# scheck-k/ste-gan

Measured on NVIDIA B200. Metric: GAN train samples/s, higher is better.
Workload: dtype bf16

## Files before the change

### include/stegan_b200.h

```cpp
#ifndef STEGAN_B200_H_
#define STEGAN_B200_H_

#include <stdint.h>

#ifdef __cplusplus
extern "C" {
#endif

typedef void* stg_stream_t;

enum { STG_F32 = 0, STG_BF16 = 1 };
enum { STG_ACT_NONE = 0, STG_ACT_RELU = 1, STG_ACT_LEAKY = 2, STG_ACT_TANH = 3 };
enum {
  STG_OK = 0,
  STG_EINVAL = -1,
  STG_ECUDA = -2,
  STG_EUNSUPPORTED = -3
};
enum { STG_ENGINE_AUTO = 0, STG_ENGINE_SIMT = 1, STG_ENGINE_TCGEN05 = 2, STG_ENGINE_MATVEC = 3  };

#define STG_MAX_TAPS 48

typedef struct StgConv {
  int32_t dtype;
  int32_t engine;
  int32_t n_samples;
  int32_t phases;
  int32_t t_src;
  int32_t t_dst;
  int32_t c_src;
  int32_t c_dst;
  int32_t groups;
  int32_t k, dilation, stride, pad;
  int32_t transposed;
  int32_t pair_sum;
  int32_t post_shift;
  int32_t mask_mode;
  int32_t act;
  int32_t dup_rows;
  int32_t out_f32;
  int32_t w_fwd_pack;
  const void* src;
  const void* w;
  const float* bias;
  const void* add_pre;
  const void* mask;
  const void* add_post;
  void* y_raw;
  void* y_act;
} StgConv;

int stg_conv(const StgConv* d, stg_stream_t stream);

int stg_conv_masked(const StgConv* d, const int32_t* valid_units, int32_t rows_per_unit, stg_stream_t stream);

typedef struct StgWgrad {
  int32_t dtype, engine;
  int32_t n_samples, phases, t_in, t_out, c_in, c_out, groups, k, dilation, stride, pad;
  const void* x;
  const void* dy;
  float* dw;
  float* dbias;
} StgWgrad;

int stg_conv_wgrad(const StgWgrad* d, stg_stream_t stream);
int stg_wgrad_layout(const StgWgrad* d, int* ld, int* span);

enum { STG_PACK_UNFOLD = 1 };
int stg_weightnorm_fold(const float* v, const float* g, int c_out, int cin_g, int k, int groups, int pack_groups,
                        int flags, int dtype, void* wf, void* wd, float* scale, stg_stream_t stream);
int stg_weightnorm_fold_bwd(const float* dw, int dw_ld, int dw_span, const float* v, const float* g, int c_out, int cin_g,
                            int k, int groups, float* dv, float* dg, int accumulate, stg_stream_t stream);

int stg_spectralnorm_fold(const float* w_orig, float* u, float* v, int c_out, int cin_g, int k, int groups,
                          int pack_groups, int flags, int training, int dtype, void* wf, void* wd, float* sigma_out,
                          float* scratch, float* u_used, float* v_used, stg_stream_t stream);
int stg_spectralnorm_fold_bwd(const float* dw, int dw_ld, int dw_span, const float* w_orig, const float* u, const float* v,
                              const float* sigma, int c_out, int cin_g, int k, int groups, float* dw_orig, int accumulate,
                              float* scratch, stg_stream_t stream);
typedef struct StgFoldItem {
  const float* v;
  const float* g;
  void* wf;
  void* wd;
  float* scale;
  const float* dw;
  float* dv;
  float* dg;
  int32_t c_out, cin_g, k, groups, pg, flags, dw_ld, dw_span;
  int32_t row0, tile0;
} StgFoldItem;
int stg_weightnorm_fold_multi(const StgFoldItem* items, int n_items, int total_rows, int total_tiles, int dtype,
                              stg_stream_t stream);
int stg_weightnorm_fold_bwd_multi(const StgFoldItem* items, int n_items, int total_rows, int accumulate,
                                  stg_stream_t stream);
int stg_weightnorm_fold_bwd_range(const StgFoldItem* items, int n_items, int row_base, int n_rows, int accumulate,
                                  stg_stream_t stream);

int stg_tc_pack_groups(int c_in, int c_out, int groups);

int stg_unfold(const void* src, int dtype, int B, int phases, int t_src, int t_dst, int C, int k, int dilation, int stride,
               int pad, void* out, stg_stream_t stream);
int stg_unfold_bwd(const void* dout, int dtype, int B, int phases, int t_src, int t_dst, int C, int k, int dilation,
                   int stride, int pad, float* dsrc, stg_stream_t stream);

int stg_period_first_layer(const float* x, const void* wf, const float* bias, int B, int T, int C, int period, int c_out,
                           int k, int stride, int pad, float slope, void* y, stg_stream_t stream);

int stg_embed_concat(const float* units, const float* emb, const int64_t* ids, int B, int T, int d_units, int d_emb,
                     int dtype, void* x0, stg_stream_t stream);
int stg_embed_concat_bwd(const void* dx0, const int64_t* ids, int B, int T, int d_units, int d_emb, int dtype,
                         float* demb, stg_stream_t stream);

int stg_reflect_pad_right(const float* x, int B, int T, int C, int T_pad, int dtype, void* out, stg_stream_t stream);
int stg_reflect_pad_right_bwd(const void* dout, int B, int T, int C, int T_pad, int dtype, float* dx, stg_stream_t stream);
int stg_avgpool4(const float* x, int B, int T, int C, float* out, stg_stream_t stream);
int stg_avgpool4_bwd(const float* dout, int B, int T, int C, float* dx, stg_stream_t stream);
int stg_cast(const void* src, int src_dtype, void* dst, int dst_dtype, int64_t n, stg_stream_t stream);
int stg_act_bwd(const float* dy, const float* y, int mode, int64_t n, int dtype, void* out, stg_stream_t stream);
int stg_relu_rows(const void* src, int dtype, int64_t rows, int C, int dup, void* out, stg_stream_t stream);
int stg_pair_sum_rows(const void* in, int64_t rows_out, int C, int dtype, void* out, stg_stream_t stream);
int stg_axpy_f32(float* y, const void* x, int x_dtype, float alpha, int64_t n, stg_stream_t stream);

int stg_td_loss(const float* x_real, const float* x_gen, int B, int T, int C, float* losses, const float* grad_scale,
                float* dx_gen, float* scratch, stg_stream_t stream);
int stg_td_loss_ex(const float* x_real, const float* x_gen, int B, int T, int C, int n_res, const int* wins,
                   const int* shifts, int pad_windows, int avg_window, float* losses, const float* grad_scale,
                   const float* grad_scale_dev, float* dx_gen, float* scratch, stg_stream_t stream);
int stg_td_features(const float* x, int B, int T, int C, int win, int shift, int pad_windows, int avg_window,
                    float* feats, float* scratch, stg_stream_t stream);
int stg_frame_stats(const float* x, int B, int T, int C, int win, int shift, int pad_windows, float* mean, float* power,
                    stg_stream_t stream);
int stg_window_signal(const float* x, int B, int T, int C, int win, int shift, int pad_windows, float* out,
                      stg_stream_t stream);
int stg_average_filter(const float* x, int64_t rows, int T, int window, int pad, float* out, stg_stream_t stream);

int stg_mse_const(const void* x, int dtype, int64_t n, float target, float* out_slot, float grad_scale, void* dx,
                  int dx_dtype, stg_stream_t stream);
int stg_l1_mean(const void* a, const void* b, int dtype, int64_t n, float* out_slot, float grad_scale, void* da,
                stg_stream_t stream);

#define STG_MAX_LOSS_ITEMS 32
typedef struct StgL1Item { const void* a; const void* b; void* da; int64_t n; } StgL1Item;
typedef struct StgMseItem { const void* x; void* dx; int64_t n; float target; int32_t slot; } StgMseItem;
int stg_l1_mean_multi(const StgL1Item* items, int n_items, int dtype, float* out_slot, float grad_scale, stg_stream_t stream);
int stg_mse_const_multi(const StgMseItem* items, int n_items, int x_dtype, int dx_dtype, float* slots, float grad_scale,
                        stg_stream_t stream);

int stg_layernorm_fwd(const void* x, int dtype, const float* gamma, const float* beta, int rows, int D, float eps, void* y,
                      float* stats, stg_stream_t stream);
int stg_layernorm_bwd(const void* dy, const void* x, int dtype, const float* stats, const float* gamma, int rows, int D,
                      void* dx, stg_stream_t stream);
int stg_relattn_fwd(const void* qkv, int dtype, const float* emb, int B, int L, int H, int d, int max_rel, float scale, void* o,
                    float* probs, stg_stream_t stream);
int stg_relattn_bwd(const void* qkv, int dtype, const float* emb, const float* probs, const void* dout, int B, int L, int H,
                    int d, int max_rel, float scale, void* dqkv, stg_stream_t stream);
int stg_relattn_dense_supported(int L, int d, int need_bwd);
int stg_relattn_band_fwd(const void* qkv, int dtype, const float* emb, int B, int L, int H, int d, int max_rel, float scale,
                         void* o, float* probs_band, stg_stream_t stream);
int stg_relattn_band_bwd(const void* qkv, int dtype, const float* emb, const float* probs_band, const void* dout, int B, int L,
                         int H, int d, int max_rel, float scale, void* dqkv, float* scratch, stg_stream_t stream);
int stg_relattn_fwd_masked(const void* qkv, int dtype, const float* emb, int B, int L, int H, int d, int max_rel, float scale,
                           void* o, float* probs, const int32_t* lengths, stg_stream_t stream);
int stg_relattn_band_fwd_masked(const void* qkv, int dtype, const float* emb, int B, int L, int H, int d, int max_rel, float scale,
                                void* o, float* probs_band, const int32_t* lengths, stg_stream_t stream);
int stg_encoder_losses(const float* unit_pred, const float* unit_target, const float* phoneme_logits,
                       const int64_t* phoneme_target, int N, int Du, int P, float* slots, float gs_units, float gs_phonemes,
                       void* d_units, void* d_logits, int grad_dtype, stg_stream_t stream);
int stg_encoder_scores(const float* unit_pred, const float* unit_target, const float* phoneme_logits,
                       const int64_t* phoneme_target, const int32_t* lengths, int B, int T, int Du, int P, int silence_index,
                       float* sums, int32_t* counts, stg_stream_t stream);

enum { STG_ADAMW_KEEP_STEP = 1 };
int stg_adamw(float* p, const float* g, float* m, float* v, int64_t n, float lr, const float* lr_dev, float beta1,
              float beta2, float eps, float weight_decay, int64_t* step_count, float grad_scale, int32_t* enable,
              int flags, stg_stream_t stream);

const char* stg_strerror(int code);
const char* stg_last_cuda_error(void);
int stg_version(void);
unsigned long long stg_launch_count(void);
void stg_set_sm_limit(int n_sms);
int stg_conv_tc_supported(const StgConv* d);
int stg_wgrad_tc_supported(const StgWgrad* d);
int stg_conv_route(const StgConv* d);
int stg_wgrad_route(const StgWgrad* d);
int stg_debug_set_trace(void* buf);
int stg_debug_rowshift(const void* x, const void* w, int rows_a, int shift, int base_off, float* out, stg_stream_t stream);
int stg_debug_group_mma(const void* x, const void* w, int cin_g, int cout_g, float* out, stg_stream_t stream);
int stg_debug_row_classes(int t_dst, int* out);
int stg_debug_tma_bw(const void* buf, long long n_rows, int box_rows, int n_iters, int mode, int stages, int grid, long long* clk,
                     stg_stream_t stream);
int stg_debug_conv_plan(const StgConv* d, int* out);
double stg_debug_ingest_bytes(int reset);

#ifdef __cplusplus
}
#endif
#endif
```

### ste_gan_b200/_lib.py

```python
from __future__ import annotations

import ctypes as C
import os

_HERE = os.path.dirname(os.path.abspath(__file__))
LIB_PATH = os.path.join(_HERE, "libstegan_b200.so")

F32, BF16 = 0, 1
ACT_NONE, ACT_RELU, ACT_LEAKY, ACT_TANH = 0, 1, 2, 3
ENGINE_AUTO, ENGINE_SIMT, ENGINE_TCGEN05 = 0, 1, 2
PACK_UNFOLD = 1
MAX_TAPS = 48


class StgConv(C.Structure):
    _fields_ = [(n, C.c_int32) for n in (
        "dtype", "engine", "n_samples", "phases", "t_src", "t_dst", "c_src", "c_dst", "groups", "k", "dilation",
        "stride", "pad", "transposed", "pair_sum", "post_shift", "mask_mode", "act", "dup_rows", "out_f32", "w_fwd_pack")] + [
        (n, C.c_void_p) for n in ("src", "w", "bias", "add_pre", "mask", "add_post", "y_raw", "y_act")]


class StgWgrad(C.Structure):
    _fields_ = [(n, C.c_int32) for n in (
        "dtype", "engine", "n_samples", "phases", "t_in", "t_out", "c_in", "c_out", "groups", "k", "dilation",
        "stride", "pad")] + [(n, C.c_void_p) for n in ("x", "dy", "dw", "dbias")]


class StgFoldItem(C.Structure):
    _fields_ = [(n, C.c_void_p) for n in ("v", "g", "wf", "wd", "scale", "dw", "dv", "dg")] + [
        (n, C.c_int32) for n in ("c_out", "cin_g", "k", "groups", "pg", "flags", "dw_ld", "dw_span", "row0", "tile0")]


class StgL1Item(C.Structure):
    _fields_ = [("a", C.c_void_p), ("b", C.c_void_p), ("da", C.c_void_p), ("n", C.c_int64)]


class StgMseItem(C.Structure):
    _fields_ = [("x", C.c_void_p), ("dx", C.c_void_p), ("n", C.c_int64), ("target", C.c_float), ("slot", C.c_int32)]


MAX_LOSS_ITEMS = 32
_P, _I, _L, _F = C.c_void_p, C.c_int, C.c_int64, C.c_float
_SIGS = {
    "stg_conv": [C.POINTER(StgConv), _P],
    "stg_conv_masked": [C.POINTER(StgConv), _P, C.c_int32, _P],
    "stg_conv_wgrad": [C.POINTER(StgWgrad), _P],
    "stg_conv_tc_supported": [C.POINTER(StgConv)],
    "stg_conv_route": [C.POINTER(StgConv)],
    "stg_wgrad_route": [C.POINTER(StgWgrad)],
    "stg_wgrad_tc_supported": [C.POINTER(StgWgrad)],
    "stg_weightnorm_fold": [_P, _P, _I, _I, _I, _I, _I, _I, _I, _P, _P, _P, _P],
    "stg_weightnorm_fold_bwd": [_P, _I, _I, _P, _P, _I, _I, _I, _I, _P, _P, _I, _P],
    "stg_wgrad_layout": [C.POINTER(StgWgrad), C.POINTER(C.c_int), C.POINTER(C.c_int)],
    "stg_spectralnorm_fold": [_P, _P, _P, _I, _I, _I, _I, _I, _I, _I, _I, _P, _P, _P, _P, _P, _P, _P],
    "stg_spectralnorm_fold_bwd": [_P, _I, _I, _P, _P, _P, _P, _I, _I, _I, _I, _P, _I, _P, _P],
    "stg_tc_pack_groups": [_I, _I, _I],
    "stg_l1_mean_multi": [_P, _I, _I, _P, _F, _P],
    "stg_mse_const_multi": [_P, _I, _I, _I, _P, _F, _P],
    "stg_weightnorm_fold_multi": [_P, _I, _I, _I, _I, _P],
    "stg_weightnorm_fold_bwd_multi": [_P, _I, _I, _I, _P],
    "stg_weightnorm_fold_bwd_range": [_P, _I, _I, _I, _I, _P],
    "stg_debug_set_trace": [_P],
    "stg_debug_rowshift": [_P, _P, _I, _I, _I, _P, _P],
    "stg_debug_row_classes": [_I, _P],
    "stg_debug_group_mma": [_P, _P, _I, _I, _P, _P],
    "stg_debug_conv_plan": [_P, _P],
    "stg_debug_tma_bw": [_P, C.c_longlong, _I, _I, _I, _I, _I, _P, _P],
    "stg_unfold": [_P, _I, _I, _I, _I, _I, _I, _I, _I, _I, _I, _P, _P],
    "stg_unfold_bwd": [_P, _I, _I, _I, _I, _I, _I, _I, _I, _I, _I, _P, _P],
    "stg_period_first_layer": [_P, _P, _P, _I, _I, _I, _I, _I, _I, _I, _I, C.c_float, _P, _P],
    "stg_embed_concat": [_P, _P, _P, _I, _I, _I, _I, _I, _P, _P],
    "stg_embed_concat_bwd": [_P, _P, _I, _I, _I, _I, _I, _P, _P],
    "stg_reflect_pad_right": [_P, _I, _I, _I, _I, _I, _P, _P],
    "stg_reflect_pad_right_bwd": [_P, _I, _I, _I, _I, _I, _P, _P],
    "stg_avgpool4": [_P, _I, _I, _I, _P, _P],
    "stg_avgpool4_bwd": [_P, _I, _I, _I, _P, _P],
    "stg_cast": [_P, _I, _P, _I, _L, _P],
    "stg_act_bwd": [_P, _P, _I, _L, _I, _P, _P],
    "stg_pair_sum_rows": [_P, _L, _I, _I, _P, _P],
    "stg_relu_rows": [_P, _I, _L, _I, _I, _P, _P],
    "stg_axpy_f32": [_P, _P, _I, _F, _L, _P],
    "stg_td_loss": [_P, _P, _I, _I, _I, _P, C.POINTER(C.c_float), _P, _P, _P],
    "stg_td_loss_ex": [_P, _P, _I, _I, _I, _I, C.POINTER(C.c_int), C.POINTER(C.c_int), _I, _I, _P, C.POINTER(C.c_float), _P, _P, _P, _P],
    "stg_td_features": [_P, _I, _I, _I, _I, _I, _I, _I, _P, _P, _P],
    "stg_frame_stats": [_P, _I, _I, _I, _I, _I, _I, _P, _P, _P],
    "stg_window_signal": [_P, _I, _I, _I, _I, _I, _I, _P, _P],
    "stg_average_filter": [_P, _L, _I, _I, _I, _P, _P],
    "stg_mse_const": [_P, _I, _L, _F, _P, _F, _P, _I, _P],
    "stg_l1_mean": [_P, _P, _I, _L, _P, _F, _P, _P],
    "stg_layernorm_fwd": [_P, _I, _P, _P, _I, _I, _F, _P, _P, _P],
    "stg_layernorm_bwd": [_P, _P, _I, _P, _P, _I, _I, _P, _P],
    "stg_relattn_fwd": [_P, _I, _P, _I, _I, _I, _I, _I, _F, _P, _P, _P],
    "stg_relattn_bwd": [_P, _I, _P, _P, _P, _I, _I, _I, _I, _I, _F, _P, _P],
    "stg_relattn_dense_supported": [_I, _I, _I],
    "stg_relattn_band_fwd": [_P, _I, _P, _I, _I, _I, _I, _I, _F, _P, _P, _P],
    "stg_relattn_band_bwd": [_P, _I, _P, _P, _P, _I, _I, _I, _I, _I, _F, _P, _P, _P],
    "stg_relattn_fwd_masked": [_P, _I, _P, _I, _I, _I, _I, _I, _F, _P, _P, _P, _P],
    "stg_relattn_band_fwd_masked": [_P, _I, _P, _I, _I, _I, _I, _I, _F, _P, _P, _P, _P],
    "stg_encoder_losses": [_P, _P, _P, _P, _I, _I, _I, _P, _F, _F, _P, _P, _I, _P],
    "stg_encoder_scores": [_P, _P, _P, _P, _P, _I, _I, _I, _I, _I, _P, _P, _P],
    "stg_adamw": [_P, _P, _P, _P, _L, _F, _P, _F, _F, _F, _F, _P, _F, _P, _I, _P],
}
EXPORTS = sorted(list(_SIGS) + ["stg_strerror", "stg_last_cuda_error", "stg_version", "stg_launch_count", "stg_set_sm_limit",
                                   "stg_debug_ingest_bytes"])

_lib = None


class StgError(RuntimeError):
    pass


def load(build_if_missing: bool = True):
    global _lib
    if _lib is not None:
        return _lib
    if not os.path.exists(LIB_PATH):
        if not build_if_missing:
            raise StgError(f"{LIB_PATH} is missing; run `python -m ste_gan_b200.build`")
        from . import build as _b
        _b.build()
    import torch
    lib = C.CDLL(LIB_PATH, mode=C.RTLD_GLOBAL)
    for name, argtypes in _SIGS.items():
        fn = getattr(lib, name)
        fn.argtypes = argtypes
        fn.restype = C.c_int
    lib.stg_strerror.argtypes = [C.c_int]
    lib.stg_strerror.restype = C.c_char_p
    lib.stg_last_cuda_error.argtypes = []
    lib.stg_last_cuda_error.restype = C.c_char_p
    lib.stg_version.argtypes = []
    lib.stg_version.restype = C.c_int
    lib.stg_set_sm_limit.argtypes = [C.c_int]
    lib.stg_set_sm_limit.restype = None
    lib.stg_debug_ingest_bytes.argtypes = [C.c_int]
    lib.stg_debug_ingest_bytes.restype = C.c_double
    lib.stg_launch_count.argtypes = []
    lib.stg_launch_count.restype = C.c_ulonglong
    _lib = lib
    return lib


def check(code: int, what: str = "") -> None:
    if code != 0:
        lib = load()
        msg = lib.stg_strerror(code).decode()
        if code == -2:
            msg += ": " + lib.stg_last_cuda_error().decode()
        raise StgError(f"{what}: {msg} (code {code})")
```

### ste_gan_b200/csrc/common.cuh

```cuda
#pragma once
#include <cuda_bf16.h>
#include <cuda_runtime.h>
#include <stdint.h>

#include "../../include/stegan_b200.h"

namespace stg {

void set_cuda_error(cudaError_t e, const char* where);

#define STG_CUDA_CHECK(expr)                                   \
  do {                                                         \
    cudaError_t _e = (expr);                                   \
    if (_e != cudaSuccess) {                                   \
      ::stg::set_cuda_error(_e, #expr);                        \
      return STG_ECUDA;                                        \
    }                                                          \
  } while (0)

extern unsigned long long g_launch_count;
extern double g_ingest_bytes;
extern int g_sm_limit;
#define STG_LAUNCH_CHECK()                 \
  do {                                     \
    ++::stg::g_launch_count;               \
    STG_CUDA_CHECK(cudaGetLastError());    \
  } while (0)

using bf16 = __nv_bfloat16;

__device__ __forceinline__ float to_f(float v) { return v; }
__device__ __forceinline__ float to_f(bf16 v) { return __bfloat162float(v); }
template <typename T> __device__ __forceinline__ T from_f(float v);
template <> __device__ __forceinline__ float from_f<float>(float v) { return v; }
template <> __device__ __forceinline__ bf16 from_f<bf16>(float v) { return __float2bfloat16_rn(v); }

__device__ __forceinline__ void ld4(const float* p, float (&o)[4]) {
  float4 v = *reinterpret_cast<const float4*>(p);
  o[0] = v.x; o[1] = v.y; o[2] = v.z; o[3] = v.w;
}
__device__ __forceinline__ void ld4(const bf16* p, float (&o)[4]) {
  uint2 v = *reinterpret_cast<const uint2*>(p);
  __nv_bfloat162 a = *reinterpret_cast<__nv_bfloat162*>(&v.x);
  __nv_bfloat162 b = *reinterpret_cast<__nv_bfloat162*>(&v.y);
  o[0] = __low2float(a); o[1] = __high2float(a); o[2] = __low2float(b); o[3] = __high2float(b);
}
__device__ __forceinline__ void st4(float* p, const float (&v)[4]) {
  *reinterpret_cast<float4*>(p) = make_float4(v[0], v[1], v[2], v[3]);
}
__device__ __forceinline__ void st4(bf16* p, const float (&v)[4]) {
  __nv_bfloat162 a = __floats2bfloat162_rn(v[0], v[1]);
  __nv_bfloat162 b = __floats2bfloat162_rn(v[2], v[3]);
  uint2 u;
  u.x = *reinterpret_cast<uint32_t*>(&a);
  u.y = *reinterpret_cast<uint32_t*>(&b);
  *reinterpret_cast<uint2*>(p) = u;
}

__device__ __forceinline__ float act_apply(int act, float v) {
  switch (act) {
    case STG_ACT_RELU: return v > 0.f ? v : 0.f;
    case STG_ACT_LEAKY: return v > 0.f ? v : 0.1f * v;
    case STG_ACT_TANH: return tanhf(v);
    default: return v;
  }
}
__device__ __forceinline__ float act_grad_from_output(int mode, float m) {
  switch (mode) {
    case STG_ACT_RELU: return m > 0.f ? 1.f : 0.f;
    case STG_ACT_LEAKY: return m > 0.f ? 1.f : 0.1f;
    case STG_ACT_TANH: return 1.f - m * m;
    default: return 1.f;
  }
}

__device__ __forceinline__ float warp_sum(float v) {
#pragma unroll
  for (int o = 16; o > 0; o >>= 1) v += __shfl_xor_sync(0xffffffffu, v, o);
  return v;
}
__device__ __forceinline__ float block_sum(float v, float* red) {
  const int lane = threadIdx.x & 31, warp = threadIdx.x >> 5, nw = (blockDim.x + 31) >> 5;
  v = warp_sum(v);
  __syncthreads();
  if (lane == 0) red[warp] = v;
  __syncthreads();
  float r = (lane < nw) ? red[lane] : 0.f;
  r = warp_sum(r);
  return r;
}

static inline int64_t ceil_div64(int64_t a, int64_t b) { return (a + b - 1) / b; }
static inline int ceil_div(int a, int b) { return (a + b - 1) / b; }

int conv_simt(const StgConv* d, cudaStream_t s, const int32_t* valid_units = nullptr, int rows_per_unit = 1);
int conv_tc(const StgConv* d, cudaStream_t s, const int32_t* valid_units = nullptr, int rows_per_unit = 1);
int conv_tc_plan(const StgConv* d, int* out);
bool conv_tc_supported(const StgConv* d);
int wgrad_simt(const StgWgrad* d, cudaStream_t s);
int wgrad_tc(const StgWgrad* d, cudaStream_t s);
bool wgrad_tc_supported(const StgWgrad* d);
int tc_pack_groups(int c_in, int c_out, int groups);
bool conv_c1_supported(const StgConv* d);
int conv_c1(const StgConv* d, cudaStream_t s);
bool wgrad_c1_supported(const StgWgrad* d);
int wgrad_c1(const StgWgrad* d, cudaStream_t s);
void conv_tc_set_trace(long long* buf);
void wgrad_tc_layout(const StgWgrad* d, int* ld, int* span);

}
```

### ste_gan_b200/csrc/misc.cu

```cuda
#include "common.cuh"

namespace stg {
namespace {

template <typename T>
__global__ void embed_concat_kernel(const float* __restrict__ units, const float* __restrict__ emb,
                                    const int64_t* __restrict__ ids, int T_, int du, int de, int64_t total,
                                    T* __restrict__ x0) {
  const int C = du + de;
  for (int64_t i = (int64_t)blockIdx.x * blockDim.x + threadIdx.x; i < total; i += (int64_t)gridDim.x * blockDim.x) {
    const int c = (int)(i % C);
    const int64_t bt = i / C;
    const int b = (int)(bt / T_);
    const float v = c < du ? units[bt * du + c] : emb[ids[b] * de + (c - du)];
    x0[i] = from_f<T>(v);
  }
}

template <typename T>
__global__ void embed_bwd_kernel(const T* __restrict__ dx0, const int64_t* __restrict__ ids, int T_, int du, int de,
                                 float* __restrict__ demb) {
  const int b = blockIdx.x, e = threadIdx.x;
  if (e >= de) return;
  const int C = du + de;
  float s = 0.f;
  for (int t = 0; t < T_; ++t) s += to_f(dx0[((int64_t)b * T_ + t) * C + du + e]);
  atomicAdd(demb + ids[b] * de + e, s);
}

__device__ __forceinline__ int reflect_right(int t, int T_) { return t < T_ ? t : 2 * (T_ - 1) - t; }

template <typename T>
__global__ void reflect_pad_kernel(const float* __restrict__ x, int T_, int C, int Tp, int64_t total, T* __restrict__ out) {
  for (int64_t i = (int64_t)blockIdx.x * blockDim.x + threadIdx.x; i < total; i += (int64_t)gridDim.x * blockDim.x) {
    const int c = (int)(i % C);
    const int64_t bt = i / C;
    const int t = (int)(bt % Tp), b = (int)(bt / Tp);
    out[i] = from_f<T>(x[((int64_t)b * T_ + reflect_right(t, T_)) * C + c]);
  }
}
template <typename T>
__global__ void reflect_pad_bwd_kernel(const T* __restrict__ dout, int T_, int C, int Tp, int64_t total_in,
                                       float* __restrict__ dx) {
  for (int64_t i = (int64_t)blockIdx.x * blockDim.x + threadIdx.x; i < total_in; i += (int64_t)gridDim.x * blockDim.x) {
    const int c = (int)(i % C);
    const int64_t bt = i / C;
    const int t = (int)(bt % T_), b = (int)(bt / T_);
    float g = to_f(dout[((int64_t)b * Tp + t) * C + c]);
    const int m = 2 * (T_ - 1) - t;
    if (m >= T_ && m < Tp) g += to_f(dout[((int64_t)b * Tp + m) * C + c]);
    atomicAdd(dx + i, g);
  }
}

__global__ void avgpool4_kernel(const float* __restrict__ x, int T_, int C, int To, int64_t total, float* __restrict__ out) {
  for (int64_t i = (int64_t)blockIdx.x * blockDim.x + threadIdx.x; i < total; i += (int64_t)gridDim.x * blockDim.x) {
    const int c = (int)(i % C);
    const int64_t bo = i / C;
    const int o = (int)(bo % To), b = (int)(bo / To);
    float s = 0.f;
#pragma unroll
    for (int j = -1; j <= 2; ++j) {
      const int t = 2 * o + j;
      if (t >= 0 && t < T_) s += x[((int64_t)b * T_ + t) * C + c];
    }
    out[i] = 0.25f * s;
  }
}
__global__ void avgpool4_bwd_kernel(const float* __restrict__ dout, int T_, int C, int To, int64_t total_in,
                                    float* __restrict__ dx) {
  for (int64_t i = (int64_t)blockIdx.x * blockDim.x + threadIdx.x; i < total_in; i += (int64_t)gridDim.x * blockDim.x) {
    const int c = (int)(i % C);
    const int64_t bt = i / C;
    const int t = (int)(bt % T_), b = (int)(bt / T_);
    float s = 0.f;
    const int lo = (t - 2 + 1) >> 1;
    for (int o = lo; o <= (t + 1) / 2; ++o)
      if (o >= 0 && o < To && 2 * o - 1 <= t && t <= 2 * o + 2) s += dout[((int64_t)b * To + o) * C + c];
    dx[i] += 0.25f * s;
  }
}

template <typename S, typename D>
__global__ void cast_kernel(const S* __restrict__ src, D* __restrict__ dst, int64_t n) {
  for (int64_t i = (int64_t)blockIdx.x * blockDim.x + threadIdx.x; i < n; i += (int64_t)gridDim.x * blockDim.x)
    dst[i] = from_f<D>(to_f(src[i]));
}

template <typename T>
__global__ void relu_rows_kernel(const T* __restrict__ src, int64_t rows, int C, int dup, T* __restrict__ out) {
  const int64_t total = rows * C;
  for (int64_t i = (int64_t)blockIdx.x * blockDim.x + threadIdx.x; i < total; i += (int64_t)gridDim.x * blockDim.x) {
    const int64_t r = i / C;
    const int c = (int)(i - r * C);
    const T v = from_f<T>(fmaxf(to_f(src[i]), 0.f));
    if (dup) { out[(2 * r) * C + c] = v; out[(2 * r + 1) * C + c] = v; }
    else out[i] = v;
  }
}

template <typename T>
__global__ void act_bwd_kernel(const float* __restrict__ dy, const float* __restrict__ y, int mode, int64_t n,
                               T* __restrict__ out) {
  for (int64_t i = (int64_t)blockIdx.x * blockDim.x + threadIdx.x; i < n; i += (int64_t)gridDim.x * blockDim.x)
    out[i] = from_f<T>(dy[i] * act_grad_from_output(mode, y[i]));
}

template <typename T>
__global__ void pair_sum_kernel(const T* __restrict__ in, int64_t rows_out, int C, T* __restrict__ out) {
  const int64_t total = rows_out * C;
  for (int64_t i = (int64_t)blockIdx.x * blockDim.x + threadIdx.x; i < total; i += (int64_t)gridDim.x * blockDim.x) {
    const int c = (int)(i % C);
    const int64_t r = i / C;
    out[i] = from_f<T>(to_f(in[(2 * r) * C + c]) + to_f(in[(2 * r + 1) * C + c]));
  }
}

template <typename T>
__global__ void axpy_kernel(float* __restrict__ y, const T* __restrict__ x, float alpha, int64_t n) {
  for (int64_t i = (int64_t)blockIdx.x * blockDim.x + threadIdx.x; i < n; i += (int64_t)gridDim.x * blockDim.x)
    y[i] = fmaf(alpha, to_f(x[i]), y[i]);
}

__global__ void step_inc_kernel(int64_t* step, const int32_t* __restrict__ enable) {
  if (enable == nullptr || *enable != 0) *step += 1;
}
__global__ void flag_clear_kernel(int32_t* flag) { *flag = 0; }

__global__ void __launch_bounds__(256) adamw_kernel(float* __restrict__ p, const float* __restrict__ g, float* __restrict__ m,
                                                    float* __restrict__ v, int64_t n, float lr_host,
                                                    const float* __restrict__ lr_dev, float b1, float b2, float eps,
                                                    float wd, const int64_t* __restrict__ step, float gscale,
                                                    const int32_t* __restrict__ enable) {
  if (enable != nullptr && *enable == 0) return;
  const float lr = lr_dev ? *lr_dev : lr_host;
  const float t = (float)(*step);
  const float bc1 = 1.f - powf(b1, t), bc2 = 1.f - powf(b2, t);
  const float step_size = lr / bc1, inv_sqrt_bc2 = rsqrtf(bc2), decay = 1.f - lr * wd;
  for (int64_t i = (int64_t)blockIdx.x * blockDim.x + threadIdx.x; i < n; i += (int64_t)gridDim.x * blockDim.x) {
    const float gi = g[i] * gscale;
    const float mi = b1 * m[i] + (1.f - b1) * gi;
    const float vi = b2 * v[i] + (1.f - b2) * gi * gi;
    m[i] = mi;
    v[i] = vi;
    const float denom = sqrtf(vi) * inv_sqrt_bc2 + eps;
    p[i] = p[i] * decay - step_size * (mi / denom);
  }
}

inline int grid_for(int64_t n) {
  int64_t b = ceil_div64(n, 256);
  const int64_t cap = 148 * 16;
  return (int)(b < 1 ? 1 : (b > cap ? cap : b));
}

template <typename T>
__global__ void unfold_kernel(const T* __restrict__ src, int phases, int t_src, int t_dst, int C, int k, int dil, int stride,
                              int pad, int Kp, int64_t total, T* __restrict__ out) {
  const int slots = Kp / C + ((Kp % C) ? 1 : 0);
  for (int64_t i = (int64_t)blockIdx.x * blockDim.x + threadIdx.x; i < total; i += (int64_t)gridDim.x * blockDim.x) {
    const int j = (int)(i % slots);
    const int64_t row = i / slots;
    const int ph = (int)(row % phases);
    const int64_t bt = row / phases;
    const int t = (int)(bt % t_dst);
    const int64_t b = bt / t_dst;
    const int ts = t * stride + j * dil - pad;
    const bool ok = j < k && ts >= 0 && ts < t_src;
    const T* s = src + ((b * t_src + ts) * phases + ph) * C;
    T* o = out + row * Kp + (int64_t)j * C;
    const int n = min(C, Kp - j * C);
    for (int c = 0; c < n; ++c) o[c] = ok ? s[c] : from_f<T>(0.f);
  }
}
template <typename T>
__global__ void unfold_bwd_kernel(const T* __restrict__ dout, int phases, int t_src, int t_dst, int C, int k, int dil,
                                  int stride, int pad, int Kp, int64_t total, float* __restrict__ dsrc) {
  for (int64_t i = (int64_t)blockIdx.x * blockDim.x + threadIdx.x; i < total; i += (int64_t)gridDim.x * blockDim.x) {
    const int c = (int)(i % C);
    const int64_t row = i / C;
    const int ph = (int)(row % phases);
    const int64_t bt = row / phases;
    const int ts = (int)(bt % t_src);
    const int64_t b = bt / t_src;
    float g = 0.f;
    for (int j = 0; j < k; ++j) {
      const int num = ts + pad - j * dil;
      if (num < 0) break;
      const int t = num / stride;
      if (t * stride == num && t < t_dst) g += to_f(dout[((b * t_dst + t) * phases + ph) * Kp + j * C + c]);
    }
    dsrc[i] += g;
  }
}

}
}

using namespace stg;
#define S_ static_cast<cudaStream_t>(stream)

extern "C" int stg_embed_concat(const float* units, const float* emb, const int64_t* ids, int B, int T, int d_units,
                                int d_emb, int dtype, void* x0, stg_stream_t stream) {
  if (!units || !x0 || (d_emb > 0 && (!emb || !ids))) return STG_EINVAL;
  const int64_t total = (int64_t)B * T * (d_units + d_emb);
  if (dtype == STG_F32) embed_concat_kernel<float><<<grid_for(total), 256, 0, S_>>>(units, emb, ids, T, d_units, d_emb, total, (float*)x0);
  else embed_concat_kernel<bf16><<<grid_for(total), 256, 0, S_>>>(units, emb, ids, T, d_units, d_emb, total, (bf16*)x0);
  STG_LAUNCH_CHECK();
  return STG_OK;
}

extern "C" int stg_embed_concat_bwd(const void* dx0, const int64_t* ids, int B, int T, int d_units, int d_emb, int dtype,
                                    float* demb, stg_stream_t stream) {
  if (!dx0 || !ids || !demb || d_emb > 1024) return STG_EINVAL;
  if (dtype == STG_F32) embed_bwd_kernel<float><<<B, d_emb, 0, S_>>>((const float*)dx0, ids, T, d_units, d_emb, demb);
  else embed_bwd_kernel<bf16><<<B, d_emb, 0, S_>>>((const bf16*)dx0, ids, T, d_units, d_emb, demb);
  STG_LAUNCH_CHECK();
  return STG_OK;
}

extern "C" int stg_reflect_pad_right(const float* x, int B, int T, int C, int T_pad, int dtype, void* out, stg_stream_t stream) {
  if (!x || !out || T_pad < T || T_pad - T > T - 1) return STG_EINVAL;
  const int64_t total = (int64_t)B * T_pad * C;
  if (dtype == STG_F32) reflect_pad_kernel<float><<<grid_for(total), 256, 0, S_>>>(x, T, C, T_pad, total, (float*)out);
  else reflect_pad_kernel<bf16><<<grid_for(total), 256, 0, S_>>>(x, T, C, T_pad, total, (bf16*)out);
  STG_LAUNCH_CHECK();
  return STG_OK;
}

extern "C" int stg_reflect_pad_right_bwd(const void* dout, int B, int T, int C, int T_pad, int dtype, float* dx, stg_stream_t stream) {
  if (!dout || !dx) return STG_EINVAL;
  const int64_t total = (int64_t)B * T * C;
  if (dtype == STG_F32) reflect_pad_bwd_kernel<float><<<grid_for(total), 256, 0, S_>>>((const float*)dout, T, C, T_pad, total, dx);
  else reflect_pad_bwd_kernel<bf16><<<grid_for(total), 256, 0, S_>>>((const bf16*)dout, T, C, T_pad, total, dx);
  STG_LAUNCH_CHECK();
  return STG_OK;
}

extern "C" int stg_avgpool4(const float* x, int B, int T, int C, float* out, stg_stream_t stream) {
  if (!x || !out) return STG_EINVAL;
  const int To = (T + 2 - 4) / 2 + 1;
  const int64_t total = (int64_t)B * To * C;
  avgpool4_kernel<<<grid_for(total), 256, 0, S_>>>(x, T, C, To, total, out);
  STG_LAUNCH_CHECK();
  return STG_OK;
}

extern "C" int stg_avgpool4_bwd(const float* dout, int B, int T, int C, float* dx, stg_stream_t stream) {
  if (!dout || !dx) return STG_EINVAL;
  const int To = (T + 2 - 4) / 2 + 1;
  const int64_t total = (int64_t)B * T * C;
  avgpool4_bwd_kernel<<<grid_for(total), 256, 0, S_>>>(dout, T, C, To, total, dx);
  STG_LAUNCH_CHECK();
  return STG_OK;
}

extern "C" int stg_cast(const void* src, int sd, void* dst, int dd, int64_t n, stg_stream_t stream) {
  if (!src || !dst) return STG_EINVAL;
  const int g = grid_for(n);
  if (sd == STG_F32 && dd == STG_BF16) cast_kernel<float, bf16><<<g, 256, 0, S_>>>((const float*)src, (bf16*)dst, n);
  else if (sd == STG_BF16 && dd == STG_F32) cast_kernel<bf16, float><<<g, 256, 0, S_>>>((const bf16*)src, (float*)dst, n);
  else if (sd == STG_F32 && dd == STG_F32) cast_kernel<float, float><<<g, 256, 0, S_>>>((const float*)src, (float*)dst, n);
  else if (sd == STG_BF16 && dd == STG_BF16) cast_kernel<bf16, bf16><<<g, 256, 0, S_>>>((const bf16*)src, (bf16*)dst, n);
  else return STG_EINVAL;
  STG_LAUNCH_CHECK();
  return STG_OK;
}

extern "C" int stg_relu_rows(const void* src, int dtype, int64_t rows, int C, int dup, void* out, stg_stream_t stream) {
  if (!src || !out || rows < 1 || C < 1) return STG_EINVAL;
  if (dtype == STG_F32) relu_rows_kernel<float><<<grid_for(rows * C), 256, 0, S_>>>((const float*)src, rows, C, dup, (float*)out);
  else if (dtype == STG_BF16) relu_rows_kernel<bf16><<<grid_for(rows * C), 256, 0, S_>>>((const bf16*)src, rows, C, dup, (bf16*)out);
  else return STG_EINVAL;
  STG_LAUNCH_CHECK();
  return STG_OK;
}

extern "C" int stg_act_bwd(const float* dy, const float* y, int mode, int64_t n, int dtype, void* out, stg_stream_t stream) {
  if (!dy || !y || !out) return STG_EINVAL;
  if (dtype == STG_F32) act_bwd_kernel<float><<<grid_for(n), 256, 0, S_>>>(dy, y, mode, n, (float*)out);
  else act_bwd_kernel<bf16><<<grid_for(n), 256, 0, S_>>>(dy, y, mode, n, (bf16*)out);
  STG_LAUNCH_CHECK();
  return STG_OK;
}

extern "C" int stg_pair_sum_rows(const void* in, int64_t rows_out, int C, int dtype, void* out, stg_stream_t stream) {
  if (!in || !out) return STG_EINVAL;
  const int g = grid_for(rows_out * C);
  if (dtype == STG_F32) pair_sum_kernel<float><<<g, 256, 0, S_>>>((const float*)in, rows_out, C, (float*)out);
  else pair_sum_kernel<bf16><<<g, 256, 0, S_>>>((const bf16*)in, rows_out, C, (bf16*)out);
  STG_LAUNCH_CHECK();
  return STG_OK;
}

extern "C" int stg_axpy_f32(float* y, const void* x, int x_dtype, float alpha, int64_t n, stg_stream_t stream) {
  if (!y || !x) return STG_EINVAL;
  if (x_dtype == STG_F32) axpy_kernel<float><<<grid_for(n), 256, 0, S_>>>(y, (const float*)x, alpha, n);
  else axpy_kernel<bf16><<<grid_for(n), 256, 0, S_>>>(y, (const bf16*)x, alpha, n);
  STG_LAUNCH_CHECK();
  return STG_OK;
}

extern "C" int stg_adamw(float* p, const float* g, float* m, float* v, int64_t n, float lr, const float* lr_dev, float beta1,
                         float beta2, float eps, float weight_decay, int64_t* step_count, float grad_scale, int32_t* enable,
                         int flags, stg_stream_t stream) {
  if (!p || !g || !m || !v || !step_count) return STG_EINVAL;
  if (!(flags & STG_ADAMW_KEEP_STEP)) {
    step_inc_kernel<<<1, 1, 0, S_>>>(step_count, enable);
    STG_LAUNCH_CHECK();
  }
  adamw_kernel<<<grid_for(n), 256, 0, S_>>>(p, g, m, v, n, lr, lr_dev, beta1, beta2, eps, weight_decay, step_count, grad_scale, enable);
  STG_LAUNCH_CHECK();
  if (enable) {
    flag_clear_kernel<<<1, 1, 0, S_>>>(enable);
    STG_LAUNCH_CHECK();
  }
  return STG_OK;
}

extern "C" int stg_unfold(const void* src, int dtype, int B, int phases, int t_src, int t_dst, int C, int k, int dilation,
                          int stride, int pad, void* out, stg_stream_t stream) {
  cudaStream_t s = static_cast<cudaStream_t>(stream);
  if (!src || !out || B < 1 || phases < 1 || C < 1 || k < 1 || stride < 1 || dilation < 1) return STG_EINVAL;
  const int Kp = (k * C + 7) / 8 * 8;
  const int slots = Kp / C + ((Kp % C) ? 1 : 0);
  const int64_t total = (int64_t)B * t_dst * phases * slots;
  const int64_t nb = ceil_div64(total, 256);
  const int blocks = (int)(nb < 148 * 16 ? nb : 148 * 16);
  if (dtype == STG_F32) unfold_kernel<float><<<blocks, 256, 0, s>>>(static_cast<const float*>(src), phases, t_src, t_dst, C, k, dilation, stride, pad, Kp, total, static_cast<float*>(out));
  else if (dtype == STG_BF16) unfold_kernel<bf16><<<blocks, 256, 0, s>>>(static_cast<const bf16*>(src), phases, t_src, t_dst, C, k, dilation, stride, pad, Kp, total, static_cast<bf16*>(out));
  else return STG_EINVAL;
  STG_LAUNCH_CHECK();
  return STG_OK;
}

extern "C" int stg_unfold_bwd(const void* dout, int dtype, int B, int phases, int t_src, int t_dst, int C, int k,
                              int dilation, int stride, int pad, float* dsrc, stg_stream_t stream) {
  cudaStream_t s = static_cast<cudaStream_t>(stream);
  if (!dout || !dsrc || B < 1 || phases < 1 || C < 1 || k < 1 || stride < 1 || dilation < 1) return STG_EINVAL;
  const int Kp = (k * C + 7) / 8 * 8;
  const int64_t total = (int64_t)B * t_src * phases * C;
  const int64_t nb = ceil_div64(total, 256);
  const int blocks = (int)(nb < 148 * 16 ? nb : 148 * 16);
  if (dtype == STG_F32) unfold_bwd_kernel<float><<<blocks, 256, 0, s>>>(static_cast<const float*>(dout), phases, t_src, t_dst, C, k, dilation, stride, pad, Kp, total, dsrc);
  else if (dtype == STG_BF16) unfold_bwd_kernel<bf16><<<blocks, 256, 0, s>>>(static_cast<const bf16*>(dout), phases, t_src, t_dst, C, k, dilation, stride, pad, Kp, total, dsrc);
  else return STG_EINVAL;
  STG_LAUNCH_CHECK();
  return STG_OK;
}
```

### ste_gan_b200/csrc/norm_fold.cu

```cuda
#include "common.cuh"

namespace stg {
namespace {

__global__ void __launch_bounds__(256) wn_scale_kernel(const float* __restrict__ v, const float* __restrict__ g, int n,
                                                       float* __restrict__ scale) {
  __shared__ float red[32];
  const int co = blockIdx.x;
  const float* row = v + (int64_t)co * n;
  float s = 0.f;
  for (int i = threadIdx.x; i < n; i += blockDim.x) { const float x = row[i]; s = fmaf(x, x, s); }
  s = block_sum(s, red);
  if (threadIdx.x == 0) scale[co] = g[co] / sqrtf(s);
}

template <typename T>
__global__ void __launch_bounds__(256) pack_fwd_kernel(const float* __restrict__ v, const float* __restrict__ scale,
                                                       int c_out, int cin_g, int k, int groups, int pg,
                                                       T* __restrict__ wf) {
  const int co = blockIdx.y;
  const int c_in = cin_g * groups, cin_gp = c_in / pg, cout_gp = c_out / pg, cout_g = c_out / groups;
  const int idx = blockIdx.x * 256 + threadIdx.x;
  if (idx >= cin_gp * k) return;
  const int j = idx / cin_gp, cip = idx - j * cin_gp;
// ... 24 lines not shown
    tile[r][tx] = w;
  }
  __syncthreads();
  for (int r = ty; r < 32; r += 8) {
    const int cip = ci0 + r, cop = co0 + tx;
    if (cip < cin_gp && cop < cout_gp)
      wd[((int64_t)j * c_in + gp * cin_gp + cip) * cout_gp + cop] = from_f<T>(tile[tx][r]);
  }
}

template <typename T>
__global__ void __launch_bounds__(256) pack_unfold_kernel(const float* __restrict__ v, const float* __restrict__ scale,
                                                          int c_out, int c_in, int k, int Kp, T* __restrict__ wf,
                                                          T* __restrict__ wd) {
  const int idx = blockIdx.x * 256 + threadIdx.x;
  if (idx >= c_out * Kp) return;
  const int co = idx / Kp, q = idx - co * Kp;
  float w = 0.f;
  if (q < k * c_in) {
    const int j = q / c_in, c = q - j * c_in;
    w = v[((int64_t)co * c_in + c) * k + j] * scale[co];
  }
  if (wf) wf[(int64_t)co * Kp + q] = from_f<T>(w);
  if (wd) wd[(int64_t)q * c_out + co] = from_f<T>(w);
}

__device__ __forceinline__ int span_goff(int co, int cin_g, int cout_g, int span) {
  if (span == cin_g || cout_g >= 128) return 0;
  return ((co / cout_g) % (128 / cout_g)) * cin_g;
}

__global__ void __launch_bounds__(256) wn_bwd_kernel(const float* __restrict__ dw, const float* __restrict__ v,
                                                     const float* __restrict__ g, int cin_g, int k, int dw_ld, int span,
                                                     int cout_g, float* __restrict__ dv, float* __restrict__ dg,
                                                     int accumulate) {
  __shared__ float red[32];
  const int co = blockIdx.x, n = cin_g * k;
  const float* vr = v + (int64_t)co * n;
  const float* dr = dw + (int64_t)co * dw_ld + span_goff(co, cin_g, cout_g, span);
  float ss = 0.f, dot = 0.f;
  for (int i = threadIdx.x; i < n; i += blockDim.x) {
    const int ci = i / k, j = i - ci * k;
    const float x = vr[i];
    ss = fmaf(x, x, ss);
    dot = fmaf(x, dr[j * span + ci], dot);
  }
  ss = block_sum(ss, red);
  dot = block_sum(dot, red);
  const float norm = sqrtf(ss), gg = g[co];
  const float a = gg / norm, bcoef = gg * dot / (norm * ss);
  for (int i = threadIdx.x; i < n; i += blockDim.x) {
    const int ci = i / k, j = i - ci * k;
    const float val = a * dr[j * span + ci] - bcoef * vr[i];
    float* o = dv + (int64_t)co * n + i;
    *o = accumulate ? (*o + val) : val;
  }
  if (threadIdx.x == 0) dg[co] = accumulate ? (dg[co] + dot / norm) : dot / norm;
}

__global__ void __launch_bounds__(256) sn_wt_u_kernel(const float* __restrict__ W, const float* __restrict__ u, int rows,
                                                      int n, float* __restrict__ out) {
  const int col = blockIdx.x * 256 + threadIdx.x;
  if (col >= n) return;
  const int r0 = blockIdx.y * 32, r1 = min(rows, r0 + 32);
  float s = 0.f;
  for (int r = r0; r < r1; ++r) s = fmaf(W[(int64_t)r * n + col], u[r], s);
  atomicAdd(out + col, s);
}
__global__ void __launch_bounds__(1024) sn_normalize_kernel(const float* __restrict__ raw, int n, float eps,
                                                            float* __restrict__ dst, float* __restrict__ sigma) {
  __shared__ float red[32];
  float s = 0.f;
  for (int i = threadIdx.x; i < n; i += blockDim.x) s = fmaf(raw[i], raw[i], s);
  s = block_sum(s, red);
  const float nrm = fmaxf(sqrtf(s), eps);
  for (int i = threadIdx.x; i < n; i += blockDim.x) dst[i] = raw[i] / nrm;
  if (sigma && threadIdx.x == 0) *sigma = s / nrm;
}
__global__ void __launch_bounds__(256) sn_w_v_kernel(const float* __restrict__ W, const float* __restrict__ v, int n,
                                                     float* __restrict__ out) {
  __shared__ float red[32];
  const int row = blockIdx.x;
  float s = 0.f;
  for (int i = threadIdx.x; i < n; i += blockDim.x) s = fmaf(W[(int64_t)row * n + i], v[i], s);
  s = block_sum(s, red);
  if (threadIdx.x == 0) out[row] = s;
}
__global__ void __launch_bounds__(256) sn_w_v_norm_kernel(const float* __restrict__ W, const float* __restrict__ raw_v, int n,
                                                          float eps, float* __restrict__ out, float* __restrict__ v_dst,
                                                          float* __restrict__ v_copy) {
  __shared__ float red[32];
  const int row = blockIdx.x;
  float ss = 0.f;
  for (int i = threadIdx.x; i < n; i += blockDim.x) ss = fmaf(raw_v[i], raw_v[i], ss);
  ss = block_sum(ss, red);
  const float nrm = fmaxf(sqrtf(ss), eps);
  __syncthreads();
  float s = 0.f;
  for (int i = threadIdx.x; i < n; i += blockDim.x) {
    const float vi = raw_v[i] / nrm;
    s = fmaf(W[(int64_t)row * n + i], vi, s);
    if (row == 0) { v_dst[i] = vi; if (v_copy) v_copy[i] = vi; }
  }
  s = block_sum(s, red);
  if (threadIdx.x == 0) out[row] = s;
}
__global__ void __launch_bounds__(1024) sn_finish_u_kernel(const float* __restrict__ raw, int n, float eps, float* __restrict__ u,
                                                           float* __restrict__ u_copy, float* __restrict__ sigma,
                                                           float* __restrict__ scale) {
  __shared__ float red[32];
  float s = 0.f;
  for (int i = threadIdx.x; i < n; i += blockDim.x) s = fmaf(raw[i], raw[i], s);
  s = block_sum(s, red);
  const float nrm = fmaxf(sqrtf(s), eps), sg = s / nrm;
  __syncthreads();
  for (int i = threadIdx.x; i < n; i += blockDim.x) {
    const float ui = raw[i] / nrm;
    u[i] = ui;
    if (u_copy) u_copy[i] = ui;
  }
  __syncthreads();
  for (int i = threadIdx.x; i < n; i += blockDim.x) scale[i] = 1.f / sg;
  if (threadIdx.x == 0) *sigma = sg;
}
__global__ void __launch_bounds__(1024) sn_dot_kernel(const float* __restrict__ a, const float* __restrict__ b, int n,
                                                      float* __restrict__ out) {
  __shared__ float red[32];
  float s = 0.f;
  for (int i = threadIdx.x; i < n; i += blockDim.x) s = fmaf(a[i], b[i], s);
  s = block_sum(s, red);
  if (threadIdx.x == 0) *out = s;
}
__global__ void sn_fill_scale_kernel(const float* __restrict__ sigma, int c_out, float* __restrict__ scale) {
  const int i = blockIdx.x * blockDim.x + threadIdx.x;
  if (i < c_out) scale[i] = 1.f / sigma[0];
}
__global__ void __launch_bounds__(256) sn_bwd_dot_kernel(const float* __restrict__ dw, const float* __restrict__ W,
                                                         int cin_g, int k, int dw_ld, int span, int cout_g,
                                                         float* __restrict__ acc) {
  __shared__ float red[32];
  const int co = blockIdx.x, n = cin_g * k;
  float s = 0.f;
  for (int i = threadIdx.x; i < n; i += blockDim.x) {
    const int ci = i / k, j = i - ci * k;
    s = fmaf(W[(int64_t)co * n + i], dw[(int64_t)co * dw_ld + span_goff(co, cin_g, cout_g, span) + j * span + ci], s);
  }
  s = block_sum(s, red);
  if (threadIdx.x == 0) atomicAdd(acc, s);
}
__global__ void __launch_bounds__(256) sn_bwd_kernel(const float* __restrict__ dw, const float* __restrict__ u,
                                                     const float* __restrict__ v, const float* __restrict__ sigma,
                                                     const float* __restrict__ dot, int cin_g, int k, int dw_ld,
                                                     int span, int cout_g, float* __restrict__ dW, int accumulate) {
  const int co = blockIdx.x, n = cin_g * k;
  const float sg = sigma[0], coef = dot[0] / (sg * sg) * u[co], inv = 1.f / sg;
  for (int i = threadIdx.x; i < n; i += blockDim.x) {
    const int ci = i / k, j = i - ci * k;
    const float val = dw[(int64_t)co * dw_ld + span_goff(co, cin_g, cout_g, span) + j * span + ci] * inv - coef * v[i];
    float* o = dW + (int64_t)co * n + i;
    if (accumulate) atomicAdd(o, val);
    else *o = val;
  }
}

__device__ __forceinline__ int find_item(const StgFoldItem* __restrict__ items, int n, int idx, bool by_tile) {
  int lo = 0, hi = n - 1;
  while (lo < hi) {
    const int mid = (lo + hi + 1) >> 1;
    const int first = by_tile ? items[mid].tile0 : items[mid].row0;
    if (first <= idx) lo = mid; else hi = mid - 1;
  }
  return lo;
}

__global__ void __launch_bounds__(256) wn_scale_multi_kernel(const StgFoldItem* __restrict__ items, int n) {
  __shared__ float red[32];
  const int it = find_item(items, n, blockIdx.x, false);
  const StgFoldItem d = items[it];
  const int co = blockIdx.x - d.row0, len = d.cin_g * d.k;
  const float* row = d.v + (int64_t)co * len;
  float s = 0.f;
  for (int i = threadIdx.x; i < len; i += blockDim.x) { const float x = row[i]; s = fmaf(x, x, s); }
  s = block_sum(s, red);
  if (threadIdx.x == 0) d.scale[co] = d.g[co] / sqrtf(s);
}

template <typename T>
__global__ void __launch_bounds__(256) pack_multi_kernel(const StgFoldItem* __restrict__ items, int n) {
  __shared__ float tile[32][33];
  const int it = find_item(items, n, blockIdx.x, true);
  const StgFoldItem d = items[it];
  int t = blockIdx.x - d.tile0;
  const int tx = threadIdx.x & 31, ty = threadIdx.x >> 5;
  T* wf = static_cast<T*>(d.wf);
  T* wd = static_cast<T*>(d.wd);
  if (d.flags & STG_PACK_UNFOLD) {
    const int Kp = (d.k * d.cin_g + 7) / 8 * 8, tq = (Kp + 31) / 32;
    const int co0 = (t / tq) * 32, q0 = (t % tq) * 32;
    for (int r = ty; r < 32; r += 8) {
      const int co = co0 + r, q = q0 + tx;
      float w = 0.f;
      if (co < d.c_out && q < d.k * d.cin_g) {
        const int j = q / d.cin_g, c = q - j * d.cin_g;
        w = d.v[((int64_t)co * d.cin_g + c) * d.k + j] * d.scale[co];
      }
      tile[r][tx] = w;
      if (wf && co < d.c_out && q < Kp) wf[(int64_t)co * Kp + q] = from_f<T>(w);
    }
    __syncthreads();
    if (wd) {
      for (int r = ty; r < 32; r += 8) {
        const int q = q0 + r, co = co0 + tx;
        if (q < Kp && co < d.c_out) wd[(int64_t)q * d.c_out + co] = from_f<T>(tile[tx][r]);
      }
    }
    return;
  }
  const int pg = d.pg, c_in = d.cin_g * d.groups, cin_gp = c_in / pg, cout_gp = d.c_out / pg, cout_g = d.c_out / d.groups;
  const int tco = (cout_gp + 31) / 32, tci = (cin_gp + 31) / 32;
  const int ci0 = (t % tci) * 32; t /= tci;
  const int co0 = (t % tco) * 32; t /= tco;
  const int j = t % d.k, gp = t / d.k;
  for (int r = ty; r < 32; r += 8) {
    const int cop = co0 + r, cip = ci0 + tx;
    float w = 0.f;
    if (cop < cout_gp && cip < cin_gp) {
      const int co = gp * cout_gp + cop, c = gp * cin_gp + cip;
      const int gc = c / d.cin_g;
      if (gc == co / cout_g) w = d.v[((int64_t)co * d.cin_g + (c - gc * d.cin_g)) * d.k + j] * d.scale[co];
      if (wf) wf[((int64_t)j * d.c_out + co) * cin_gp + cip] = from_f<T>(w);
    }
    tile[r][tx] = w;
  }
  __syncthreads();
  if (wd) {
    for (int r = ty; r < 32; r += 8) {
      const int cip = ci0 + r, cop = co0 + tx;
      if (cip < cin_gp && cop < cout_gp)
        wd[((int64_t)j * c_in + gp * cin_gp + cip) * cout_gp + cop] = from_f<T>(tile[tx][r]);
    }
  }
}

#ifndef STG_FOLD_RPW
#define STG_FOLD_RPW 1
#endif
constexpr int FOLD_RPW = STG_FOLD_RPW;
constexpr int FOLD_RPB = 8 * FOLD_RPW;
__device__ __forceinline__ bool al16(const void* p) { return (reinterpret_cast<uintptr_t>(p) & 15u) == 0; }
static inline bool al16_host(const void* p) { return (reinterpret_cast<uintptr_t>(p) & 15u) == 0; }

template <typename T> __device__ __forceinline__ void store4(T* dst, float a, float b, float c, float d);
template <> __device__ __forceinline__ void store4<float>(float* dst, float a, float b, float c, float d) {
  *reinterpret_cast<float4*>(dst) = make_float4(a, b, c, d);
}
template <> __device__ __forceinline__ void store4<bf16>(bf16* dst, float a, float b, float c, float d) {
  __nv_bfloat162 lo = __floats2bfloat162_rn(a, b), hi = __floats2bfloat162_rn(c, d);
  *reinterpret_cast<uint2*>(dst) = make_uint2(*reinterpret_cast<uint32_t*>(&lo), *reinterpret_cast<uint32_t*>(&hi));
}
__device__ __forceinline__ bool fold_fast(const StgFoldItem& d) {
  return d.flags == 0 && d.groups == 1 && d.pg == 1 && (d.k == 1 || d.k == 3 || d.k == 5) && (d.cin_g & 3) == 0 &&
         al16(d.v) && al16(d.wf);
}
__device__ __forceinline__ bool fold_bwd_fast(const StgFoldItem& d) {
  const int span = d.dw_span > 0 ? d.dw_span : d.cin_g, ld = d.dw_ld > 0 ? d.dw_ld : span * d.k;
  return d.flags == 0 && d.groups == 1 && (d.k == 1 || d.k == 3 || d.k == 5) && (d.cin_g & 3) == 0 && (span & 3) == 0 &&
         (ld & 3) == 0 && al16(d.v) && al16(d.dv) && al16(d.dw);
}

template <typename T, int K>
__device__ __forceinline__ void fold_row_warp(const StgFoldItem& d, int co, int lane) {
  const int cin = d.cin_g, ng = cin >> 2;
  const float4* v4 = reinterpret_cast<const float4*>(d.v + (int64_t)co * cin * K);
  float ss = 0.f;
  for (int g = lane; g < ng; g += 64) {
    float4 a[K], b[K];
    const bool two = g + 32 < ng;
#pragma unroll
    for (int q = 0; q < K; ++q) a[q] = v4[g * K + q];
#pragma unroll
    for (int q = 0; q < K; ++q) b[q] = two ? v4[(g + 32) * K + q] : make_float4(0.f, 0.f, 0.f, 0.f);
#pragma unroll
    for (int q = 0; q < K; ++q)
      ss += a[q].x * a[q].x + a[q].y * a[q].y + a[q].z * a[q].z + a[q].w * a[q].w +
            b[q].x * b[q].x + b[q].y * b[q].y + b[q].z * b[q].z + b[q].w * b[q].w;
  }
  ss = warp_sum(ss);
  const float sc = d.g[co] / sqrtf(ss);
  if (lane == 0) d.scale[co] = sc;
  T* wf = static_cast<T*>(d.wf);
  for (int g = lane; g < ng; g += 32) {
    float f[4 * K];
#pragma unroll
    for (int q = 0; q < K; ++q) {
      const float4 x = v4[g * K + q];
      f[4 * q] = x.x; f[4 * q + 1] = x.y; f[4 * q + 2] = x.z; f[4 * q + 3] = x.w;
    }
#pragma unroll
    for (int j = 0; j < K; ++j)
      store4<T>(wf + ((int64_t)j * d.c_out + co) * cin + 4 * g, f[j] * sc, f[K + j] * sc, f[2 * K + j] * sc, f[3 * K + j] * sc);
  }
}

template <int K>
__device__ __forceinline__ void fold_bwd_row_warp(const StgFoldItem& d, int co, int lane, int accumulate) {
  const int cin = d.cin_g, ng = cin >> 2;
  const int span = d.dw_span > 0 ? d.dw_span : cin, ld = d.dw_ld > 0 ? d.dw_ld : span * K;
  const float4* v4 = reinterpret_cast<const float4*>(d.v + (int64_t)co * cin * K);
  const float* dr = d.dw + (int64_t)co * ld;
  float4* o4 = reinterpret_cast<float4*>(d.dv + (int64_t)co * cin * K);
  float ss = 0.f, dot = 0.f;
  for (int g = lane; g < ng; g += 32) {
    float f[4 * K], w[K][4];
#pragma unroll
    for (int q = 0; q < K; ++q) {
      const float4 x = v4[g * K + q];
      f[4 * q] = x.x; f[4 * q + 1] = x.y; f[4 * q + 2] = x.z; f[4 * q + 3] = x.w;
    }
#pragma unroll
    for (int j = 0; j < K; ++j) {
      const float4 x = *reinterpret_cast<const float4*>(dr + j * span + 4 * g);
      w[j][0] = x.x; w[j][1] = x.y; w[j][2] = x.z; w[j][3] = x.w;
    }
#pragma unroll
    for (int c = 0; c < 4; ++c)
#pragma unroll
      for (int j = 0; j < K; ++j) { ss = fmaf(f[c * K + j], f[c * K + j], ss); dot = fmaf(f[c * K + j], w[j][c], dot); }
  }
  ss = warp_sum(ss);
  dot = warp_sum(dot);
  const float norm = sqrtf(ss), gg = d.g[co];
  const float a = gg / norm, bcoef = gg * dot / (norm * ss);
  for (int g = lane; g < ng; g += 32) {
    float f[4 * K], w[K][4], o[4 * K];
#pragma unroll
    for (int q = 0; q < K; ++q) {
      const float4 x = v4[g * K + q];
      f[4 * q] = x.x; f[4 * q + 1] = x.y; f[4 * q + 2] = x.z; f[4 * q + 3] = x.w;
    }
#pragma unroll
    for (int j = 0; j < K; ++j) {
      const float4 x = *reinterpret_cast<const float4*>(dr + j * span + 4 * g);
      w[j][0] = x.x; w[j][1] = x.y; w[j][2] = x.z; w[j][3] = x.w;
    }
#pragma unroll
    for (int c = 0; c < 4; ++c)
#pragma unroll
      for (int j = 0; j < K; ++j) o[c * K + j] = a * w[j][c] - bcoef * f[c * K + j];
#pragma unroll
    for (int q = 0; q < K; ++q) {
      float4 r = make_float4(o[4 * q], o[4 * q + 1], o[4 * q + 2], o[4 * q + 3]);
      if (accumulate) { const float4 p = o4[g * K + q]; r.x += p.x; r.y += p.y; r.z += p.z; r.w += p.w; }
      o4[g * K + q] = r;
    }
  }
  if (lane == 0) d.dg[co] = accumulate ? (d.dg[co] + dot / norm) : dot / norm;
}

template <typename T>
__device__ __forceinline__ void fold_row_warp_generic(const StgFoldItem& d, int co, int lane) {
  const int n = d.cin_g * d.k, k = d.k, cin_g = d.cin_g;
  const float* vr = d.v + (int64_t)co * n;
  float ss = 0.f;
  for (int i = lane; i < n; i += 32) { const float x = vr[i]; ss = fmaf(x, x, ss); }
  ss = warp_sum(ss);
  const float sc = d.g[co] / sqrtf(ss);
  if (lane == 0) d.scale[co] = sc;
  T* wf = static_cast<T*>(d.wf);
  if (d.flags & STG_PACK_UNFOLD) {
    const int Kp = (k * cin_g + 7) / 8 * 8;
    for (int q = lane; q < Kp; q += 32) {
      float w = 0.f;
      if (q < k * cin_g) { const int j = q / cin_g, c = q - j * cin_g; w = vr[c * k + j] * sc; }
      wf[(int64_t)co * Kp + q] = from_f<T>(w);
    }
    return;
  }
  const int pg = d.pg, c_in = cin_g * d.groups, cin_gp = c_in / pg, cout_gp = d.c_out / pg, cout_g = d.c_out / d.groups;
  const int off = ((co / cout_g) - (co / cout_gp) * (d.groups / pg)) * cin_g;
  for (int j = 0; j < k; ++j) {
    T* dst = wf + ((int64_t)j * d.c_out + co) * cin_gp;
    for (int cip = lane; cip < cin_gp; cip += 32) {
      const int c = cip - off;
      dst[cip] = from_f<T>((c >= 0 && c < cin_g) ? vr[c * k + j] * sc : 0.f);
    }
  }
}

template <typename T>
__global__ void __launch_bounds__(256) wd_from_wf_kernel(const StgFoldItem* __restrict__ items, int n_items) {
  __shared__ T slab[8192];
  const int it = find_item(items, n_items, blockIdx.x, true);
  const StgFoldItem d = items[it];
  const int local = blockIdx.x - d.tile0, j = local / d.pg, u = local - j * d.pg;
  const int c_in = d.cin_g * d.groups, cin_gp = c_in / d.pg, cout_gp = d.c_out / d.pg, n = cin_gp * cout_gp;
  const T* src = static_cast<const T*>(d.wf) + ((int64_t)j * d.c_out + (int64_t)u * cout_gp) * cin_gp;
  T* dst = static_cast<T*>(d.wd) + ((int64_t)j * c_in + (int64_t)u * cin_gp) * cout_gp;
  if (n <= 8192) {
    for (int i = threadIdx.x; i < n; i += 256) slab[i] = src[i];
    __syncthreads();
    for (int i = threadIdx.x; i < n; i += 256) { const int c = i / cout_gp, r = i - c * cout_gp; dst[i] = slab[r * cin_gp + c]; }
  } else {
    for (int i = threadIdx.x; i < n; i += 256) { const int c = i / cout_gp, r = i - c * cout_gp; dst[i] = src[(int64_t)r * cin_gp + c]; }
  }
}

template <typename T>
__global__ void __launch_bounds__(256, 4) wn_fold_rows_kernel(const StgFoldItem* __restrict__ items, int n_items, int total_rows) {
  const int warp = threadIdx.x >> 5, lane = threadIdx.x & 31;
  const int w_begin = blockIdx.x * FOLD_RPB + warp * FOLD_RPW, w_end = min(total_rows, w_begin + FOLD_RPW);
  if (w_begin >= w_end) return;
  int it = find_item(items, n_items, w_begin, false);
  StgFoldItem d = items[it];
  for (int r = w_begin; r < w_end; ++r) {
    while (r >= d.row0 + d.c_out) d = items[++it];
    const int co = r - d.row0;
    if (!fold_fast(d)) fold_row_warp_generic<T>(d, co, lane);
    else if (d.k == 3) fold_row_warp<T, 3>(d, co, lane);
    else if (d.k == 1) fold_row_warp<T, 1>(d, co, lane);
    else fold_row_warp<T, 5>(d, co, lane);
  }
}

__device__ __forceinline__ void fold_bwd_row_warp_generic(const StgFoldItem& d, int co, int lane, int accumulate) {
  const int n = d.cin_g * d.k, k = d.k, cin_g = d.cin_g;
  const int span = d.dw_span > 0 ? d.dw_span : cin_g, ld = d.dw_ld > 0 ? d.dw_ld : span * k;
  const float* vr = d.v + (int64_t)co * n;
  const float* dr = d.dw + (int64_t)co * ld + span_goff(co, cin_g, d.c_out / d.groups, span);
  float* orow = d.dv + (int64_t)co * n;
  float ss = 0.f, dot = 0.f;
  const int total = k * cin_g;
  for (int i = lane; i < total; i += 32) {
    const int j = i / cin_g, ci = i - j * cin_g;
    const float x = vr[ci * k + j];
    ss = fmaf(x, x, ss);
    dot = fmaf(x, dr[j * span + ci], dot);
  }
  ss = warp_sum(ss);
  dot = warp_sum(dot);
  const float norm = sqrtf(ss), gg = d.g[co];
  const float a = gg / norm, bcoef = gg * dot / (norm * ss);
  for (int i = lane; i < n; i += 32) {
    const int ci = i / k, j = i - ci * k;
    const float val = a * dr[j * span + ci] - bcoef * vr[i];
    orow[i] = accumulate ? (orow[i] + val) : val;
  }
  if (lane == 0) d.dg[co] = accumulate ? (d.dg[co] + dot / norm) : dot / norm;
}

__global__ void __launch_bounds__(256, 4) wn_bwd_multi_kernel(const StgFoldItem* __restrict__ items, int n_items, int row_base,
                                                           int total_rows, int accumulate) {
  const int warp = threadIdx.x >> 5, lane = threadIdx.x & 31;
  const int w_begin = row_base + blockIdx.x * FOLD_RPB + warp * FOLD_RPW, w_end = min(row_base + total_rows, w_begin + FOLD_RPW);
  if (w_begin >= w_end) return;
  int it = find_item(items, n_items, w_begin, false);
  StgFoldItem d = items[it];
  for (int r = w_begin; r < w_end; ++r) {
    while (r >= d.row0 + d.c_out) d = items[++it];
    const int co = r - d.row0;
    if (!fold_bwd_fast(d)) fold_bwd_row_warp_generic(d, co, lane, accumulate);
    else if (d.k == 3) fold_bwd_row_warp<3>(d, co, lane, accumulate);
    else if (d.k == 1) fold_bwd_row_warp<1>(d, co, lane, accumulate);
    else fold_bwd_row_warp<5>(d, co, lane, accumulate);
  }
}

template <typename T, int K>
__global__ void __launch_bounds__(256) pack_rows_kernel(const float* __restrict__ v, const float* __restrict__ scale, int c_out,
                                                        int cin, T* __restrict__ wf) {
  const int co = blockIdx.x * 8 + (threadIdx.x >> 5), lane = threadIdx.x & 31;
  if (co >= c_out) return;
  const float sc = scale[co];
  const float4* v4 = reinterpret_cast<const float4*>(v + (int64_t)co * cin * K);
  for (int g = lane; g < (cin >> 2); g += 32) {
    float f[4 * K];
#pragma unroll
    for (int q = 0; q < K; ++q) {
      const float4 x = v4[g * K + q];
      f[4 * q] = x.x; f[4 * q + 1] = x.y; f[4 * q + 2] = x.z; f[4 * q + 3] = x.w;
    }
#pragma unroll
    for (int j = 0; j < K; ++j)
      store4<T>(wf + ((int64_t)j * c_out + co) * cin + 4 * g, f[j] * sc, f[K + j] * sc, f[2 * K + j] * sc, f[3 * K + j] * sc);
  }
}

template <typename T>
__global__ void __launch_bounds__(256) wd_from_wf_direct_kernel(const T* __restrict__ wf, T* __restrict__ wd, int c_out, int c_in,
                                                                int pg) {
  __shared__ T slab[8192];
  const int j = blockIdx.x / pg, u = blockIdx.x - j * pg;
  const int cin_gp = c_in / pg, cout_gp = c_out / pg, n = cin_gp * cout_gp;
  const T* src = wf + ((int64_t)j * c_out + (int64_t)u * cout_gp) * cin_gp;
  T* dst = wd + ((int64_t)j * c_in + (int64_t)u * cin_gp) * cout_gp;
  if (n <= 8192) {
    for (int i = threadIdx.x; i < n; i += 256) slab[i] = src[i];
    __syncthreads();
    for (int i = threadIdx.x; i < n; i += 256) { const int c = i / cout_gp, r = i - c * cout_gp; dst[i] = slab[r * cin_gp + c]; }
  } else {
    for (int i = threadIdx.x; i < n; i += 256) { const int c = i / cout_gp, r = i - c * cout_gp; dst[i] = src[(int64_t)r * cin_gp + c]; }
  }
}

template <typename T>
int launch_packs(const float* v, const float* scale, int c_out, int cin_g, int k, int groups, int pg, int flags, T* wf,
                 T* wd, cudaStream_t s) {
  if (flags & STG_PACK_UNFOLD) {
    if (groups != 1) return STG_EINVAL;
    const int Kp = (k * cin_g + 7) / 8 * 8;
    pack_unfold_kernel<T><<<ceil_div(c_out * Kp, 256), 256, 0, s>>>(v, scale, c_out, cin_g, k, Kp, wf, wd);
    STG_LAUNCH_CHECK();
    return STG_OK;
  }
  if (pg <= 0) pg = groups;
  if (groups % pg) return STG_EINVAL;
  const int c_in = cin_g * groups, cin_gp = c_in / pg, cout_gp = c_out / pg;
  if (wf && groups == 1 && (k == 1 || k == 3 || k == 5) && (cin_g & 3) == 0 && al16_host(v) && al16_host(wf)) {
    const int nb = ceil_div(c_out, 8);
    if (k == 1) pack_rows_kernel<T, 1><<<nb, 256, 0, s>>>(v, scale, c_out, cin_g, wf);
    else if (k == 3) pack_rows_kernel<T, 3><<<nb, 256, 0, s>>>(v, scale, c_out, cin_g, wf);
    else pack_rows_kernel<T, 5><<<nb, 256, 0, s>>>(v, scale, c_out, cin_g, wf);
    STG_LAUNCH_CHECK();
  } else if (wf) {
    dim3 g1(ceil_div(cin_gp * k, 256), c_out);
    pack_fwd_kernel<T><<<g1, 256, 0, s>>>(v, scale, c_out, cin_g, k, groups, pg, wf);
    STG_LAUNCH_CHECK();
  }
  if (wd && wf && sizeof(T) == 2 && groups > 1) {
    wd_from_wf_direct_kernel<T><<<k * pg, 256, 0, s>>>(wf, wd, c_out, c_in, pg);
    STG_LAUNCH_CHECK();
  } else if (wd) {
    dim3 g2(ceil_div(cout_gp, 32), ceil_div(cin_gp, 32), k * pg);
    pack_dgrad_kernel<T><<<g2, 256, 0, s>>>(v, scale, c_out, cin_g, k, groups, pg, wd);
    STG_LAUNCH_CHECK();
  }
  return STG_OK;
}

}
}

using namespace stg;

extern "C" int stg_weightnorm_fold(const float* v, const float* g, int c_out, int cin_g, int k, int groups,
                                   int pack_groups, int flags, int dtype, void* wf, void* wd, float* scale,
                                   stg_stream_t stream) {
  cudaStream_t s = static_cast<cudaStream_t>(stream);
  if (!v || !g || !scale || c_out < 1 || cin_g < 1 || k < 1 || groups < 1 || c_out % groups) return STG_EINVAL;
  wn_scale_kernel<<<c_out, 256, 0, s>>>(v, g, cin_g * k, scale);
  STG_LAUNCH_CHECK();
  if (dtype == STG_F32) return launch_packs<float>(v, scale, c_out, cin_g, k, groups, pack_groups, flags, (float*)wf, (float*)wd, s);
  if (dtype == STG_BF16) return launch_packs<bf16>(v, scale, c_out, cin_g, k, groups, pack_groups, flags, (bf16*)wf, (bf16*)wd, s);
  return STG_EINVAL;
}

extern "C" int stg_weightnorm_fold_bwd(const float* dw, int dw_ld, int dw_span, const float* v, const float* g, int c_out,
                                       int cin_g, int k, int groups, float* dv, float* dg, int accumulate,
                                       stg_stream_t stream) {
  cudaStream_t s = static_cast<cudaStream_t>(stream);
  if (!dw || !v || !g || !dv || !dg || groups < 1) return STG_EINVAL;
  if (dw_span <= 0) dw_span = cin_g;
  if (dw_ld <= 0) dw_ld = dw_span * k;
  wn_bwd_kernel<<<c_out, 256, 0, s>>>(dw, v, g, cin_g, k, dw_ld, dw_span, c_out / groups, dv, dg, accumulate);
  STG_LAUNCH_CHECK();
  return STG_OK;
}

extern "C" int stg_spectralnorm_fold(const float* w_orig, float* u, float* v, int c_out, int cin_g, int k, int groups,
                                     int pack_groups, int flags, int training, int dtype, void* wf, void* wd,
                                     float* sigma_out, float* scratch, float* u_used, float* v_used, stg_stream_t stream) {
  cudaStream_t s = static_cast<cudaStream_t>(stream);
  if (!w_orig || !u || !v || !sigma_out || !scratch) return STG_EINVAL;
  const int n = cin_g * k;
  float* raw_u = scratch;
  float* raw_v = scratch + c_out;
  float* scale = raw_u;
  const float eps = 1e-12f;
  if (training) {
    STG_CUDA_CHECK(cudaMemsetAsync(raw_v, 0, sizeof(float) * n, s));
    dim3 g1(ceil_div(n, 256), ceil_div(c_out, 32));
    sn_wt_u_kernel<<<g1, 256, 0, s>>>(w_orig, u, c_out, n, raw_v);
    STG_LAUNCH_CHECK();
    sn_w_v_norm_kernel<<<c_out, 256, 0, s>>>(w_orig, raw_v, n, eps, raw_u, v, v_used);
    STG_LAUNCH_CHECK();
    sn_finish_u_kernel<<<1, 1024, 0, s>>>(raw_u, c_out, eps, u, u_used, sigma_out, scale);
    STG_LAUNCH_CHECK();
  } else {
    sn_w_v_kernel<<<c_out, 256, 0, s>>>(w_orig, v, n, raw_u);
    STG_LAUNCH_CHECK();
    sn_dot_kernel<<<1, 1024, 0, s>>>(u, raw_u, c_out, sigma_out);
    STG_LAUNCH_CHECK();
    sn_fill_scale_kernel<<<ceil_div(c_out, 256), 256, 0, s>>>(sigma_out, c_out, scale);
    STG_LAUNCH_CHECK();
    if (u_used) STG_CUDA_CHECK(cudaMemcpyAsync(u_used, u, sizeof(float) * c_out, cudaMemcpyDeviceToDevice, s));
    if (v_used) STG_CUDA_CHECK(cudaMemcpyAsync(v_used, v, sizeof(float) * n, cudaMemcpyDeviceToDevice, s));
  }
  if (dtype == STG_F32) return launch_packs<float>(w_orig, scale, c_out, cin_g, k, groups, pack_groups, flags, (float*)wf, (float*)wd, s);
  if (dtype == STG_BF16) return launch_packs<bf16>(w_orig, scale, c_out, cin_g, k, groups, pack_groups, flags, (bf16*)wf, (bf16*)wd, s);
  return STG_EINVAL;
}

extern "C" int stg_spectralnorm_fold_bwd(const float* dw, int dw_ld, int dw_span, const float* w_orig, const float* u,
                                         const float* v, const float* sigma, int c_out, int cin_g, int k, int groups,
                                         float* dw_orig, int accumulate, float* scratch, stg_stream_t stream) {
  cudaStream_t s = static_cast<cudaStream_t>(stream);
  if (!dw || !w_orig || !u || !v || !sigma || !dw_orig || !scratch || groups < 1) return STG_EINVAL;
  if (dw_span <= 0) dw_span = cin_g;
  if (dw_ld <= 0) dw_ld = dw_span * k;
  STG_CUDA_CHECK(cudaMemsetAsync(scratch, 0, sizeof(float), s));
  sn_bwd_dot_kernel<<<c_out, 256, 0, s>>>(dw, w_orig, cin_g, k, dw_ld, dw_span, c_out / groups, scratch);
  STG_LAUNCH_CHECK();
  sn_bwd_kernel<<<c_out, 256, 0, s>>>(dw, u, v, sigma, scratch, cin_g, k, dw_ld, dw_span, c_out / groups, dw_orig, accumulate);
  STG_LAUNCH_CHECK();
  return STG_OK;
}

extern "C" int stg_weightnorm_fold_multi(const StgFoldItem* items, int n_items, int total_rows, int total_tiles, int dtype,
                                         stg_stream_t stream) {
  cudaStream_t s = static_cast<cudaStream_t>(stream);
  if (!items || n_items < 1 || total_rows < 1) return STG_EINVAL;
  if (total_tiles <= 0) {
    if (dtype == STG_F32) wn_fold_rows_kernel<float><<<ceil_div(total_rows, FOLD_RPB), 256, 0, s>>>(items, n_items, total_rows);
    else if (dtype == STG_BF16) wn_fold_rows_kernel<bf16><<<ceil_div(total_rows, FOLD_RPB), 256, 0, s>>>(items, n_items, total_rows);
    else return STG_EINVAL;
    STG_LAUNCH_CHECK();
    if (total_tiles < 0) {
      if (dtype == STG_F32) return STG_EINVAL;
      wd_from_wf_kernel<bf16><<<-total_tiles, 256, 0, s>>>(items, n_items);
      STG_LAUNCH_CHECK();
    }
    return STG_OK;
  }
  wn_scale_multi_kernel<<<total_rows, 256, 0, s>>>(items, n_items);
  STG_LAUNCH_CHECK();
  if (dtype == STG_F32) pack_multi_kernel<float><<<total_tiles, 256, 0, s>>>(items, n_items);
  else if (dtype == STG_BF16) pack_multi_kernel<bf16><<<total_tiles, 256, 0, s>>>(items, n_items);
  else return STG_EINVAL;
  STG_LAUNCH_CHECK();
  return STG_OK;
}

extern "C" int stg_weightnorm_fold_bwd_multi(const StgFoldItem* items, int n_items, int total_rows, int accumulate,
                                             stg_stream_t stream) {
  cudaStream_t s = static_cast<cudaStream_t>(stream);
  if (!items || n_items < 1 || total_rows < 1) return STG_EINVAL;
  wn_bwd_multi_kernel<<<ceil_div(total_rows, FOLD_RPB), 256, 0, s>>>(items, n_items, 0, total_rows, accumulate);
  STG_LAUNCH_CHECK();
  return STG_OK;
}

extern "C" int stg_weightnorm_fold_bwd_range(const StgFoldItem* items, int n_items, int row_base, int n_rows, int accumulate,
                                             stg_stream_t stream) {
  cudaStream_t s = static_cast<cudaStream_t>(stream);
  if (!items || n_items < 1 || row_base < 0 || n_rows < 1) return STG_EINVAL;
  wn_bwd_multi_kernel<<<ceil_div(n_rows, FOLD_RPB), 256, 0, s>>>(items, n_items, row_base, n_rows, accumulate);
  STG_LAUNCH_CHECK();
  return STG_OK;
}
```

### ste_gan_b200/ops.py

```python
from __future__ import annotations

import ctypes as C
from typing import Optional, Tuple

import torch

from . import _lib
from ._lib import (ACT_LEAKY, ACT_NONE, ACT_RELU, ACT_TANH, BF16, ENGINE_AUTO, ENGINE_SIMT, ENGINE_TCGEN05, F32,
                   StgConv, StgWgrad, check)

Tensor = torch.Tensor
_engine_override: Optional[int] = None
profile = None
flop_log = None


def set_engine(engine: Optional[int]) -> None:
    global _engine_override
    _engine_override = engine


def code_of(dtype: torch.dtype) -> int:
    if dtype == torch.float32:
        return F32
    if dtype == torch.bfloat16:
        return BF16
    raise TypeError(f"unsupported dtype {dtype}")


def _ptr(t: Optional[Tensor]) -> Optional[int]:
    return None if t is None else t.data_ptr()


def _stream() -> int:
    return torch.cuda.current_stream().cuda_stream


def _need(t: Optional[Tensor], numel: int, dtype: Optional[torch.dtype], name: str) -> None:
    if t is None:
        return
    if not t.is_cuda:
        raise _lib.StgError(f"{name}: expected a CUDA tensor (there is no CPU fallback)")
    if not t.is_contiguous():
        raise _lib.StgError(f"{name}: expected a contiguous tensor")
    if dtype is not None and t.dtype != dtype:
        raise _lib.StgError(f"{name}: expected {dtype}, got {t.dtype}")
    if t.numel() < numel:
        raise _lib.StgError(f"{name}: buffer too small ({t.numel()} < {numel})")


def conv(src: Tensor, w: Tensor, *, n_samples: int, t_src: int, t_dst: int, c_src: int, c_dst: int, k: int,
         phases: int = 1, groups: int = 1, dilation: int = 1, stride: int = 1, pad: int = 0, transposed: bool = False,
         pair_sum: bool = False, post_shift: int = 0, mask: Optional[Tensor] = None, mask_mode: int = ACT_NONE,
         act: int = ACT_NONE, dup_rows: bool = False, bias: Optional[Tensor] = None, add_pre: Optional[Tensor] = None,
         add_post: Optional[Tensor] = None, y_raw: Optional[Tensor] = None, y_act: Optional[Tensor] = None,
         engine: int = ENGINE_AUTO, w_fwd_pack: bool = False, acct_groups: Optional[int] = None,
         valid_units: Optional[Tensor] = None, rows_per_unit: int = 1) -> None:
    dt = src.dtype
    nv = n_samples * phases
    t_out = t_dst // 2 if pair_sum else t_dst
    _need(src, nv * t_src * c_src, None, "src")
    _need(w, k * c_dst * (c_src // groups), dt, "w")
    _need(bias, c_dst, torch.float32, "bias")
    _need(add_pre, nv * t_out * c_dst, dt, "add_pre")
    _need(mask, nv * t_out * c_dst, dt, "mask")
    _need(add_post, nv * (t_out >> post_shift) * c_dst, dt, "add_post")
    outs = [t for t in (y_raw, y_act) if t is not None]
    out_f32 = dt != torch.float32 and len(outs) > 0 and all(t.dtype == torch.float32 for t in outs)
    odt = torch.float32 if out_f32 else dt
    _need(y_raw, nv * t_out * c_dst, odt, "y_raw")
    _need(y_act, nv * t_out * c_dst * (2 if dup_rows else 1), odt, "y_act")
    _need(valid_units, n_samples, torch.int32, "valid_units")
    d = StgConv(dtype=code_of(dt), engine=_engine_override if _engine_override is not None else engine,
                n_samples=n_samples, phases=phases, t_src=t_src, t_dst=t_dst, c_src=c_src, c_dst=c_dst, groups=groups,
                k=k, dilation=dilation, stride=stride, pad=pad, transposed=int(transposed), pair_sum=int(pair_sum),
                post_shift=post_shift, mask_mode=mask_mode, act=act, dup_rows=int(dup_rows), out_f32=int(out_f32),
                w_fwd_pack=int(w_fwd_pack), src=_ptr(src), w=_ptr(w), bias=_ptr(bias), add_pre=_ptr(add_pre), mask=_ptr(mask),
                add_post=_ptr(add_post), y_raw=_ptr(y_raw), y_act=_ptr(y_act))
    lib = _lib.load()

    def launch():
        if valid_units is None:
            check(lib.stg_conv(C.byref(d), _stream()), "stg_conv")
        else:
            check(lib.stg_conv_masked(C.byref(d), _ptr(valid_units), rows_per_unit, _stream()), "stg_conv_masked")

    if profile is None and flop_log is None:
        launch()
        return
    if valid_units is None:
        route = {1: "simt", 2: "tcgen05", 3: "matvec"}[lib.stg_conv_route(C.byref(d))]
    else:
        eng = d.engine if d.engine != ENGINE_AUTO else (ENGINE_TCGEN05 if lib.stg_conv_tc_supported(C.byref(d)) else ENGINE_SIMT)
        route = "tcgen05" if eng == ENGINE_TCGEN05 else "simt"
    ag = acct_groups if acct_groups is not None else groups
    flops = 2.0 * nv * t_src * c_src * k * (c_dst // ag) if transposed else 2.0 * nv * t_dst * c_dst * k * (c_src // ag)
    esz = 2 if dt == torch.bfloat16 else 4
    nbytes = esz * (nv * t_src * c_src + k * c_dst * (c_src // ag)) + sum(
        t.numel() * t.element_size() for t in (add_pre, mask, add_post, y_raw, y_act) if t is not None)
    rec = dict(kind=("dgrad" if transposed else "fwd"), engine=route, flops=flops, bytes=nbytes,
               shape=(n_samples, phases, t_src, t_dst, c_src, c_dst, k, dilation, stride, ag))
    if flop_log is not None:
        flop_log.append(rec)
    if profile is None:
        launch()
        return
    e0, e1 = torch.cuda.Event(enable_timing=True), torch.cuda.Event(enable_timing=True)
    e0.record()
    launch()
    e1.record()
    rec["ingest"] = _ingest(lib)
    fn, args = ("stg_conv", ()) if valid_units is None else ("stg_conv_masked", (_ptr(valid_units), rows_per_unit))
    profile.append(dict(rec, events=(e0, e1), desc=d, fn=fn, args=args,
                        keep=(src, w, bias, add_pre, mask, add_post, y_raw, y_act, valid_units)))


def _ingest(lib) -> float:
    return float(lib.stg_debug_ingest_bytes(1))


def conv_tc_supported(**kw) -> bool:
    d = StgConv(**kw)
    return bool(_lib.load().stg_conv_tc_supported(C.byref(d)))


def wgrad_layout(dtype: torch.dtype, *, c_in: int, c_out: int, k: int, groups: int = 1, stride: int = 1,
                 engine: int = ENGINE_AUTO) -> tuple:
    d = StgWgrad(dtype=code_of(dtype), engine=_engine_override if _engine_override is not None else engine, n_samples=1,
                 phases=1, t_in=1, t_out=1, c_in=c_in, c_out=c_out, groups=groups, k=k, dilation=1, stride=stride, pad=0)
    ld, span = C.c_int(0), C.c_int(0)
    check(_lib.load().stg_wgrad_layout(C.byref(d), C.byref(ld), C.byref(span)), "stg_wgrad_layout")
    return ld.value, span.value


def wgrad(x: Tensor, dy: Tensor, dw: Optional[Tensor], dbias: Optional[Tensor], *, n_samples: int, t_in: int,
          t_out: int, c_in: int, c_out: int, k: int, phases: int = 1, groups: int = 1, dilation: int = 1,
          stride: int = 1, pad: int = 0, engine: int = ENGINE_AUTO) -> None:
    nv = n_samples * phases
    _need(x, nv * t_in * c_in, None, "x")
    _need(dy, nv * t_out * c_out, x.dtype, "dy")
    if dw is not None:
        ld, _ = wgrad_layout(x.dtype, c_in=c_in, c_out=c_out, k=k, groups=groups, stride=stride, engine=engine)
        _need(dw, c_out * ld, torch.float32, "dw")
    _need(dbias, c_out, torch.float32, "dbias")
    d = StgWgrad(dtype=code_of(x.dtype), engine=_engine_override if _engine_override is not None else engine,
                 n_samples=n_samples, phases=phases, t_in=t_in, t_out=t_out, c_in=c_in, c_out=c_out, groups=groups,
                 k=k, dilation=dilation, stride=stride, pad=pad, x=_ptr(x), dy=_ptr(dy), dw=_ptr(dw), dbias=_ptr(dbias))
    lib = _lib.load()
    if profile is None and flop_log is None:
        check(lib.stg_conv_wgrad(C.byref(d), _stream()), "stg_conv_wgrad")
        return
    route = {1: "simt", 2: "tcgen05", 3: "matvec"}[lib.stg_wgrad_route(C.byref(d))]
    esz = 2 if x.dtype == torch.bfloat16 else 4
    rec = dict(kind="wgrad", engine=route, flops=2.0 * nv * t_out * c_out * k * (c_in // groups),
               bytes=esz * nv * (t_in * c_in + t_out * c_out) + 4 * c_out * k * (c_in // groups),
               shape=(n_samples, phases, t_in, t_out, c_in, c_out, k, dilation, stride, groups))
    if flop_log is not None:
        flop_log.append(rec)
    if profile is None:
        check(lib.stg_conv_wgrad(C.byref(d), _stream()), "stg_conv_wgrad")
        return
    e0, e1 = torch.cuda.Event(enable_timing=True), torch.cuda.Event(enable_timing=True)
    e0.record()
    check(lib.stg_conv_wgrad(C.byref(d), _stream()), "stg_conv_wgrad")
    e1.record()
    rec["ingest"] = _ingest(lib)
    profile.append(dict(rec, events=(e0, e1), desc=d, fn="stg_conv_wgrad", keep=(x, dy, dw, dbias)))


def tc_pack_groups(c_in: int, c_out: int, groups: int) -> int:
    return int(_lib.load().stg_tc_pack_groups(c_in, c_out, groups))


def round_up8(n: int) -> int:
    return (n + 7) // 8 * 8


def _pack_shapes(c_out: int, cin_g: int, k: int, groups: int, pack_groups: int, unfold: bool):
    if unfold:
        kp = round_up8(k * cin_g)
        return (c_out, kp), (kp, c_out)
    c_in = cin_g * groups
    return (k, c_out, c_in // pack_groups), (k, c_in, c_out // pack_groups)


def weightnorm_fold(v: Tensor, g: Tensor, groups: int, dtype: torch.dtype, want_dgrad: bool = True, out=None,
                    pack_groups: Optional[int] = None, unfold: bool = False):
    c_out, cin_g, k = v.shape[0], v.shape[1], v.shape[2]
    pg = groups if pack_groups is None else pack_groups
    sf, sd = _pack_shapes(c_out, cin_g, k, groups, pg, unfold)
    nf = sf[0] * sf[1] * (sf[2] if len(sf) > 2 else 1)
    _need(v, c_out * cin_g * k, torch.float32, "v"); _need(g, c_out, torch.float32, "g")
    if out is not None:
        wf, wd, scale = out
        _need(wf, nf, dtype, "wf"); _need(wd, nf, dtype, "wd"); _need(scale, c_out, torch.float32, "scale")
    else:
        wf = torch.empty(sf, device=v.device, dtype=dtype)
        wd = torch.empty(sd, device=v.device, dtype=dtype) if want_dgrad else None
        scale = torch.empty((c_out,), device=v.device, dtype=torch.float32)
    check(_lib.load().stg_weightnorm_fold(_ptr(v), _ptr(g), c_out, cin_g, k, groups, pg, _lib.PACK_UNFOLD if unfold else 0,
                                          code_of(dtype), _ptr(wf), _ptr(wd), _ptr(scale), _stream()), "stg_weightnorm_fold")
    return wf, wd, scale


def weightnorm_fold_bwd(dw: Tensor, v: Tensor, g: Tensor, dv: Tensor, dg: Tensor, accumulate: bool, dw_ld: int = 0,
                        dw_span: int = 0, groups: int = 1) -> None:
    c_out, cin_g, k = v.shape[0], v.shape[1], v.shape[2]
    _need(dw, c_out * max(dw_ld, max(dw_span, cin_g) * k), torch.float32, "dw"); _need(dv, c_out * cin_g * k, torch.float32, "dv")
    _need(dg, c_out, torch.float32, "dg")
    check(_lib.load().stg_weightnorm_fold_bwd(_ptr(dw), dw_ld, dw_span, _ptr(v), _ptr(g), c_out, cin_g, k, groups, _ptr(dv),
                                              _ptr(dg), int(accumulate), _stream()), "stg_weightnorm_fold_bwd")


def spectralnorm_fold(w_orig: Tensor, u: Tensor, v: Tensor, groups: int, training: bool, dtype: torch.dtype,
                      want_dgrad: bool = True, pack_groups: Optional[int] = None, unfold: bool = False, keep_uv: bool = False):
    c_out, cin_g, k = w_orig.shape[0], w_orig.shape[1], w_orig.shape[2]
    n = cin_g * k
    pg = groups if pack_groups is None else pack_groups
    sf, sd = _pack_shapes(c_out, cin_g, k, groups, pg, unfold)
    _need(w_orig, c_out * n, torch.float32, "w_orig"); _need(u, c_out, torch.float32, "u"); _need(v, n, torch.float32, "v")
    wf = torch.empty(sf, device=u.device, dtype=dtype)
    wd = torch.empty(sd, device=u.device, dtype=dtype) if want_dgrad else None
    sigma = torch.empty((1,), device=u.device, dtype=torch.float32)
    scratch = torch.empty((c_out + n + 8,), device=u.device, dtype=torch.float32)
    u_used = torch.empty_like(u) if keep_uv else None
    v_used = torch.empty_like(v) if keep_uv else None
    check(_lib.load().stg_spectralnorm_fold(_ptr(w_orig), _ptr(u), _ptr(v), c_out, cin_g, k, groups, pg,
                                            _lib.PACK_UNFOLD if unfold else 0, int(training), code_of(dtype), _ptr(wf),
                                            _ptr(wd), _ptr(sigma), _ptr(scratch), _ptr(u_used), _ptr(v_used), _stream()),
          "stg_spectralnorm_fold")
    if keep_uv:
        return wf, wd, sigma, u_used, v_used
    return wf, wd, sigma


def spectralnorm_fold_bwd(dw: Tensor, w_orig: Tensor, u: Tensor, v: Tensor, sigma: Tensor, dw_orig: Tensor,
                          accumulate: bool, dw_ld: int = 0, dw_span: int = 0, groups: int = 1) -> None:
    c_out, cin_g, k = w_orig.shape[0], w_orig.shape[1], w_orig.shape[2]
    _need(dw, c_out * max(dw_ld, max(dw_span, cin_g) * k), torch.float32, "dw"); _need(dw_orig, c_out * cin_g * k, torch.float32, "dw_orig")
    scratch = torch.empty((8,), device=u.device, dtype=torch.float32)
    check(_lib.load().stg_spectralnorm_fold_bwd(_ptr(dw), dw_ld, dw_span, _ptr(w_orig), _ptr(u), _ptr(v), _ptr(sigma), c_out,
                                                cin_g, k, groups, _ptr(dw_orig), int(accumulate), _ptr(scratch), _stream()),
          "stg_spectralnorm_fold_bwd")


def fold_table(items: list, device) -> Tensor:
    arr = (_lib.StgFoldItem * len(items))(*items)
    return torch.frombuffer(bytearray(bytes(arr)), dtype=torch.uint8).to(device)


def weightnorm_fold_multi(table: Tensor, n_items: int, total_rows: int, total_tiles: int, dtype: torch.dtype) -> None:
    check(_lib.load().stg_weightnorm_fold_multi(_ptr(table), n_items, total_rows, total_tiles, code_of(dtype), _stream()),
          "stg_weightnorm_fold_multi")


def weightnorm_fold_bwd_multi(table: Tensor, n_items: int, total_rows: int, accumulate: bool = True) -> None:
    check(_lib.load().stg_weightnorm_fold_bwd_multi(_ptr(table), n_items, total_rows, int(accumulate), _stream()),
          "stg_weightnorm_fold_bwd_multi")


def weightnorm_fold_bwd_range(table: Tensor, n_items: int, row_base: int, n_rows: int, accumulate: bool = True) -> None:
    check(_lib.load().stg_weightnorm_fold_bwd_range(_ptr(table), n_items, row_base, n_rows, int(accumulate), _stream()),
          "stg_weightnorm_fold_bwd_range")


def unfold(src: Tensor, *, n_samples: int, phases: int, t_src: int, t_dst: int, channels: int, k: int, dilation: int,
           stride: int, pad: int) -> Tensor:
    _need(src, n_samples * phases * t_src * channels, None, "src")
    out = torch.empty((n_samples, t_dst * phases, round_up8(k * channels)), device=src.device, dtype=src.dtype)
    check(_lib.load().stg_unfold(_ptr(src), code_of(src.dtype), n_samples, phases, t_src, t_dst, channels, k, dilation,
                                 stride, pad, _ptr(out), _stream()), "stg_unfold")
    return out


def unfold_bwd(dout: Tensor, dsrc: Tensor, *, n_samples: int, phases: int, t_src: int, t_dst: int, channels: int, k: int,
               dilation: int, stride: int, pad: int) -> None:
    _need(dout, n_samples * phases * t_dst * round_up8(k * channels), None, "dout")
    _need(dsrc, n_samples * phases * t_src * channels, torch.float32, "dsrc")
    check(_lib.load().stg_unfold_bwd(_ptr(dout), code_of(dout.dtype), n_samples, phases, t_src, t_dst, channels, k,
                                     dilation, stride, pad, _ptr(dsrc), _stream()), "stg_unfold_bwd")


def period_first_layer(x: Tensor, wf: Tensor, bias: Optional[Tensor], *, period: int, c_out: int, k: int, stride: int, pad: int,
                       slope: float = 0.1) -> Tuple[Tensor, int]:
    B, T, Cc = x.shape
    _need(x, B * T * Cc, torch.float32, "x")
    t_pad = T + (period - T % period)
    h_out = (t_pad // period + 2 * pad - (k - 1) - 1) // stride + 1
    _need(wf, c_out * round_up8(k * Cc), torch.bfloat16, "wf")
    y = torch.empty((B, h_out * period, c_out), device=x.device, dtype=torch.bfloat16)
    check(_lib.load().stg_period_first_layer(_ptr(x), _ptr(wf), _ptr(bias), B, T, Cc, period, c_out, k, stride, pad, float(slope),
                                             _ptr(y), _stream()), "stg_period_first_layer")
    return y, h_out


def embed_concat(units: Tensor, emb: Optional[Tensor], ids: Optional[Tensor], dtype: torch.dtype) -> Tensor:
    B, T, du = units.shape
    de = 0 if emb is None else emb.shape[1]
    _need(units, B * T * du, torch.float32, "units")
    if emb is not None:
        _need(emb, emb.shape[0] * de, torch.float32, "emb"); _need(ids, B, torch.int64, "ids")
    x0 = torch.empty((B, T, du + de), device=units.device, dtype=dtype)
    check(_lib.load().stg_embed_concat(_ptr(units), _ptr(emb), _ptr(ids), B, T, du, de, code_of(dtype), _ptr(x0),
                                       _stream()), "stg_embed_concat")
    return x0


def embed_concat_bwd(dx0: Tensor, ids: Tensor, d_units: int, demb: Tensor) -> None:
    B, T, Cc = dx0.shape
    de = Cc - d_units
    _need(ids, B, torch.int64, "ids"); _need(demb, de, torch.float32, "demb")
    check(_lib.load().stg_embed_concat_bwd(_ptr(dx0), _ptr(ids), B, T, d_units, de, code_of(dx0.dtype), _ptr(demb),
                                           _stream()), "stg_embed_concat_bwd")


def reflect_pad_right(x: Tensor, t_pad: int, dtype: torch.dtype) -> Tensor:
    B, T, Cc = x.shape
    _need(x, B * T * Cc, torch.float32, "x")
    out = torch.empty((B, t_pad, Cc), device=x.device, dtype=dtype)
    check(_lib.load().stg_reflect_pad_right(_ptr(x), B, T, Cc, t_pad, code_of(dtype), _ptr(out), _stream()),
          "stg_reflect_pad_right")
    return out


def reflect_pad_right_bwd(dout: Tensor, T: int, dx: Tensor) -> None:
    B, t_pad, Cc = dout.shape
    _need(dx, B * T * Cc, torch.float32, "dx"); _need(dout, B * t_pad * Cc, None, "dout")
    check(_lib.load().stg_reflect_pad_right_bwd(_ptr(dout), B, T, Cc, t_pad, code_of(dout.dtype), _ptr(dx), _stream()),
          "stg_reflect_pad_right_bwd")


def avgpool4(x: Tensor) -> Tensor:
    B, T, Cc = x.shape
    _need(x, B * T * Cc, torch.float32, "x")
    out = torch.empty((B, (T + 2 - 4) // 2 + 1, Cc), device=x.device, dtype=torch.float32)
    check(_lib.load().stg_avgpool4(_ptr(x), B, T, Cc, _ptr(out), _stream()), "stg_avgpool4")
    return out


def avgpool4_bwd(dout: Tensor, T: int, dx: Tensor) -> None:
    B, To, Cc = dout.shape
    _need(dout, B * To * Cc, torch.float32, "dout"); _need(dx, B * T * Cc, torch.float32, "dx")
    check(_lib.load().stg_avgpool4_bwd(_ptr(dout), B, T, Cc, _ptr(dx), _stream()), "stg_avgpool4_bwd")


def cast(src: Tensor, dtype: torch.dtype) -> Tensor:
    _need(src, src.numel(), None, "src")
    dst = torch.empty(src.shape, device=src.device, dtype=dtype)
    check(_lib.load().stg_cast(_ptr(src), code_of(src.dtype), _ptr(dst), code_of(dtype), src.numel(), _stream()), "stg_cast")
    return dst


def act_bwd(dy: Tensor, y: Tensor, mode: int, dtype: torch.dtype) -> Tensor:
    _need(dy, y.numel(), torch.float32, "dy"); _need(y, y.numel(), torch.float32, "y")
    out = torch.empty(y.shape, device=y.device, dtype=dtype)
    check(_lib.load().stg_act_bwd(_ptr(dy), _ptr(y), mode, y.numel(), code_of(dtype), _ptr(out), _stream()), "stg_act_bwd")
    return out


def average_filter(x: Tensor, window: int, pad: bool) -> Tensor:
    xc = x.contiguous().float()
    rows, T = xc.numel() // xc.shape[-1], xc.shape[-1]
    t_out = T if pad else T - window + 1
    out = torch.empty(xc.shape[:-1] + (t_out,), device=x.device, dtype=torch.float32)
    check(_lib.load().stg_average_filter(_ptr(xc), rows, T, window, int(pad), _ptr(out), _stream()), "stg_average_filter")
    return out


def relu_rows(x: Tensor, dup: bool) -> Tensor:
    B, T, Cc = x.shape
    _need(x, B * T * Cc, None, "x")
    out = torch.empty((B, T * (2 if dup else 1), Cc), device=x.device, dtype=x.dtype)
    check(_lib.load().stg_relu_rows(_ptr(x), code_of(x.dtype), B * T, Cc, int(dup), _ptr(out), _stream()), "stg_relu_rows")
    return out


def pair_sum_rows(x: Tensor, rows_out: int, Cc: int) -> Tensor:
    _need(x, 2 * rows_out * Cc, None, "x")
    out = torch.empty((rows_out, Cc), device=x.device, dtype=x.dtype)
    check(_lib.load().stg_pair_sum_rows(_ptr(x), rows_out, Cc, code_of(x.dtype), _ptr(out), _stream()), "stg_pair_sum_rows")
    return out


def axpy_f32(y: Tensor, x: Tensor, alpha: float) -> None:
    _need(y, x.numel(), torch.float32, "y"); _need(x, x.numel(), None, "x")
    check(_lib.load().stg_axpy_f32(_ptr(y), _ptr(x), code_of(x.dtype), float(alpha), x.numel(), _stream()), "stg_axpy_f32")


def td_loss(x_real: Tensor, x_gen: Tensor, losses: Tensor, grad_scale=None, dx_gen: Optional[Tensor] = None) -> None:
    B, T, Cc = x_gen.shape
    n = B * T * Cc
    _need(x_real, n, torch.float32, "x_real"); _need(x_gen, n, torch.float32, "x_gen")
    _need(losses, 3, torch.float32, "losses"); _need(dx_gen, n, torch.float32, "dx_gen")
    scratch = torch.empty((6 * n + 8,), device=x_gen.device, dtype=torch.float32)
    gs = (C.c_float * 3)(*([0.0] * 3 if grad_scale is None else [float(g) for g in grad_scale]))
    check(_lib.load().stg_td_loss(_ptr(x_real), _ptr(x_gen), B, T, Cc, _ptr(losses), gs, _ptr(dx_gen),
                                  _ptr(scratch), _stream()), "stg_td_loss")


def n_frames(T: int, win: int, shift: int, pad: bool) -> int:
    return ((T + 2 * (win // 2) if pad else T) - win) // shift + 1


def td_loss_ex(x_real: Tensor, x_gen: Tensor, resolutions, losses: Tensor, *, pad_windows: bool = True, avg_window: int = 9,
               grad_scale=None, dx_gen: Optional[Tensor] = None) -> None:
    B, T, Cc = x_gen.shape
    n, nr = B * T * Cc, len(resolutions)
    _need(x_real, n, torch.float32, "x_real"); _need(x_gen, n, torch.float32, "x_gen")
    _need(losses, nr, torch.float32, "losses"); _need(dx_gen, n, torch.float32, "dx_gen")
    scratch = torch.empty((6 * n + 8,), device=x_gen.device, dtype=torch.float32)
    wins = (C.c_int * nr)(*[int(w) for w, _ in resolutions]); shifts = (C.c_int * nr)(*[int(s_) for _, s_ in resolutions])
    gs_host, gs_dev = None, None
    if isinstance(grad_scale, torch.Tensor):
        _need(grad_scale, nr, torch.float32, "grad_scale")
        gs_dev = grad_scale
    elif grad_scale is not None:
        gs_host = (C.c_float * nr)(*[float(g) for g in grad_scale])
    check(_lib.load().stg_td_loss_ex(_ptr(x_real), _ptr(x_gen), B, T, Cc, nr, wins, shifts, int(pad_windows), int(avg_window),
                                     _ptr(losses), gs_host, _ptr(gs_dev), _ptr(dx_gen), _ptr(scratch), _stream()), "stg_td_loss_ex")


def td_features(x: Tensor, win: int, shift: int, pad_windows: bool = True, avg_window: int = 9) -> Tensor:
    x = x.contiguous().float()
    B, T, Cc = x.shape
    _need(x, B * T * Cc, torch.float32, "x")
    out = torch.empty((B, n_frames(T, win, shift, pad_windows), Cc, 4), device=x.device, dtype=torch.float32)
    scratch = torch.empty((2 * B * T * Cc,), device=x.device, dtype=torch.float32)
    check(_lib.load().stg_td_features(_ptr(x), B, T, Cc, win, shift, int(pad_windows), avg_window, _ptr(out), _ptr(scratch),
                                      _stream()), "stg_td_features")
    return out


def frame_stats(x: Tensor, win: int, shift: int, pad_windows: bool, want_mean: bool, want_power: bool):
    x = x.contiguous().float()
    B, T, Cc = x.shape
    _need(x, B * T * Cc, torch.float32, "x")
    F_ = n_frames(T, win, shift, pad_windows)
    mean = torch.empty((B, F_, Cc), device=x.device, dtype=torch.float32) if want_mean else None
    power = torch.empty((B, F_, Cc), device=x.device, dtype=torch.float32) if want_power else None
    check(_lib.load().stg_frame_stats(_ptr(x), B, T, Cc, win, shift, int(pad_windows), _ptr(mean), _ptr(power), _stream()),
          "stg_frame_stats")
    return mean, power


def window_signal(x: Tensor, win: int, shift: int, pad_windows: bool) -> Tensor:
    x = x.contiguous().float()
    B, T, Cc = x.shape
    _need(x, B * T * Cc, torch.float32, "x")
    out = torch.empty((B, n_frames(T, win, shift, pad_windows), Cc, win), device=x.device, dtype=torch.float32)
    check(_lib.load().stg_window_signal(_ptr(x), B, T, Cc, win, shift, int(pad_windows), _ptr(out), _stream()), "stg_window_signal")
    return out


def mse_const(x: Tensor, target: float, out_slot: Optional[Tensor], grad_scale: float = 0.0, dx: Optional[Tensor] = None) -> None:
    _need(x, x.numel(), None, "x"); _need(dx, x.numel(), None, "dx"); _need(out_slot, 1, torch.float32, "out_slot")
    check(_lib.load().stg_mse_const(_ptr(x), code_of(x.dtype), x.numel(), float(target), _ptr(out_slot), float(grad_scale),
                                    _ptr(dx), code_of(dx.dtype) if dx is not None else 0, _stream()), "stg_mse_const")


def l1_mean(a: Tensor, b: Tensor, out_slot: Optional[Tensor], grad_scale: float = 0.0, da: Optional[Tensor] = None) -> None:
    _need(a, a.numel(), None, "a"); _need(b, a.numel(), a.dtype, "b"); _need(da, a.numel(), a.dtype, "da")
    _need(out_slot, 1, torch.float32, "out_slot")
    check(_lib.load().stg_l1_mean(_ptr(a), _ptr(b), code_of(a.dtype), a.numel(), _ptr(out_slot), float(grad_scale), _ptr(da),
                                  _stream()), "stg_l1_mean")


def l1_mean_multi(pairs, out_slot: Tensor, grad_scale: float, want_grad: bool = True):
    _need(out_slot, 1, torch.float32, "out_slot")
    das = []
    lib = _lib.load()
    for lo in range(0, len(pairs), _lib.MAX_LOSS_ITEMS):
        chunk = pairs[lo:lo + _lib.MAX_LOSS_ITEMS]
        items = (_lib.StgL1Item * len(chunk))()
        for i, (a, b) in enumerate(chunk):
            _need(a, a.numel(), None, "a"); _need(b, a.numel(), a.dtype, "b")
            if a.dtype != chunk[0][0].dtype:
                raise _lib.StgError("l1_mean_multi: mixed dtypes")
            da = torch.empty_like(a) if want_grad else None
            das.append(da)
            items[i] = _lib.StgL1Item(_ptr(a), _ptr(b), _ptr(da), a.numel())
        check(lib.stg_l1_mean_multi(items, len(chunk), code_of(chunk[0][0].dtype), _ptr(out_slot), float(grad_scale), _stream()),
              "stg_l1_mean_multi")
    return das if want_grad else None


def mse_const_multi(xs, targets, slots: Tensor, slot_idx, grad_scale: float, dx_dtype: torch.dtype, outs=None):
    n = len(xs)
    if n > _lib.MAX_LOSS_ITEMS:
        raise _lib.StgError("mse_const_multi: too many tensors")
    items = (_lib.StgMseItem * n)()
    dxs = []
    for i, x in enumerate(xs):
        _need(x, x.numel(), xs[0].dtype, "x")
        if outs is not None and outs[i] is not None:
            dx = outs[i]
            _need(dx, x.numel(), dx_dtype, "out")
        else:
            dx = torch.empty(x.shape, device=x.device, dtype=dx_dtype)
        dxs.append(dx)
        items[i] = _lib.StgMseItem(_ptr(x), _ptr(dx), x.numel(), float(targets[i]), int(slot_idx[i]))
    check(_lib.load().stg_mse_const_multi(items, n, code_of(xs[0].dtype), code_of(dx_dtype), _ptr(slots), float(grad_scale),
                                          _stream()), "stg_mse_const_multi")
    return dxs


def adamw(p: Tensor, g: Tensor, m: Tensor, v: Tensor, step: Tensor, lr, beta1: float = 0.8, beta2: float = 0.99,
          eps: float = 1e-8, weight_decay: float = 0.01, grad_scale: float = 1.0, enable: Optional[Tensor] = None,
          keep_step: bool = False) -> None:
    _need(enable, 1, torch.int32, "enable")
    n = p.numel()
    lr_dev = None
    if isinstance(lr, torch.Tensor):
        _need(lr, 1, torch.float32, "lr")
        lr_dev, lr = lr, 0.0
    for t, nm in ((p, "p"), (g, "g"), (m, "m"), (v, "v")):
        _need(t, n, torch.float32, nm)
    _need(step, 1, torch.int64, "step")
    check(_lib.load().stg_adamw(_ptr(p), _ptr(g), _ptr(m), _ptr(v), n, float(lr), _ptr(lr_dev), beta1, beta2, eps, weight_decay,
                                _ptr(step), grad_scale, _ptr(enable), int(keep_step), _stream()), "stg_adamw")


def layernorm(x: Tensor, gamma: Tensor, beta: Tensor, eps: float = 1e-5) -> Tuple[Tensor, Tensor]:
    D = x.shape[-1]
    rows = x.numel() // D
    _need(x, rows * D, None, "x"); _need(gamma, D, torch.float32, "gamma"); _need(beta, D, torch.float32, "beta")
    y = torch.empty_like(x)
    stats = torch.empty((rows, 2), device=x.device, dtype=torch.float32)
    check(_lib.load().stg_layernorm_fwd(_ptr(x), code_of(x.dtype), _ptr(gamma), _ptr(beta), rows, D, float(eps), _ptr(y), _ptr(stats),
                                        _stream()), "stg_layernorm_fwd")
    return y, stats


def layernorm_bwd(dy: Tensor, x: Tensor, stats: Tensor, gamma: Tensor) -> Tensor:
    D = x.shape[-1]
    rows = x.numel() // D
    _need(dy, rows * D, x.dtype, "dy"); _need(x, rows * D, None, "x"); _need(stats, rows * 2, torch.float32, "stats")
    dx = torch.empty_like(x)
    check(_lib.load().stg_layernorm_bwd(_ptr(dy), _ptr(x), code_of(x.dtype), _ptr(stats), _ptr(gamma), rows, D, _ptr(dx), _stream()),
          "stg_layernorm_bwd")
    return dx


def relattn_fwd(qkv: Tensor, emb: Tensor, n_head: int, max_rel: int, lengths: Optional[Tensor] = None) -> Tuple[Tensor, Tensor]:
    B, L, C3 = qkv.shape
    d = C3 // (3 * n_head)
    _need(qkv, B * L * C3, None, "qkv"); _need(emb, n_head * (2 * max_rel - 1) * d, torch.float32, "emb")
    _need(lengths, B, torch.int32, "lengths")
    o = torch.empty((B, L, n_head * d), device=qkv.device, dtype=qkv.dtype)
    probs = torch.empty((B, n_head, L, L), device=qkv.device, dtype=torch.float32)
    args = (_ptr(qkv), code_of(qkv.dtype), _ptr(emb), B, L, n_head, d, max_rel, float(d) ** -0.5, _ptr(o), _ptr(probs))
    if lengths is None:
        check(_lib.load().stg_relattn_fwd(*args, _stream()), "stg_relattn_fwd")
    else:
        check(_lib.load().stg_relattn_fwd_masked(*args, _ptr(lengths), _stream()), "stg_relattn_fwd_masked")
    return o, probs


def relattn_bwd(qkv: Tensor, emb: Tensor, probs: Tensor, dout: Tensor, n_head: int, max_rel: int) -> Tensor:
# ... 72 lines not shown
```

### ste_gan_b200/passes.py

```python
from __future__ import annotations

from dataclasses import dataclass, field
from typing import Dict, List, Optional, Sequence, Tuple

import torch

from . import ops
from .ops import ACT_LEAKY, ACT_NONE, ACT_RELU, ACT_TANH

Tensor = torch.Tensor


@dataclass
class Folded:
    mod: torch.nn.Module
    wf: Tensor
    wd: Optional[Tensor]
    dtype: torch.dtype
    scale: Optional[Tensor] = None
    u: Optional[Tensor] = None
    v: Optional[Tensor] = None
    sigma: Optional[Tensor] = None
    pg: int = 1
    unfold: bool = False
# ... 142 lines not shown
            scale = self._scales[so:so + m.out_channels]; so += (m.out_channels + 3) // 4 * 4
            kp = ops.round_up8(m.kernel * m.in_channels) if unf else 0
            self.folds[id(m)] = Folded(m, wf, wd, dtype, scale=scale, pg=pg, unfold=unf, kp=kp)
        self._dw_off = {}
        for m in self.wn:
            n = dw_layout(self.folds[id(m)])[0]
            self._dw_off[id(m)] = (n_dw, n); n_dw += (n + 3) // 4 * 4
        self.arena = torch.zeros(n_dw, device=dev, dtype=torch.float32)
        items, row0, tile0 = [], 0, 0
        for m in self.wn:
            f = self.folds[id(m)]
            cin_g = m.in_channels // m.groups
            _, ld, span = dw_layout(f)
            off, n = self._dw_off[id(m)]
            gv, gg = _grad_of(m.weight_v), _grad_of(m.weight_g)
            items.append(_lib.StgFoldItem(
                v=m.weight_v.data.data_ptr(), g=m.weight_g.data.data_ptr(), wf=f.wf.data_ptr(), wd=f.wd.data_ptr() if f.wd is not None else None,
                scale=f.scale.data_ptr(), dw=self.arena[off:off + n].data_ptr(), dv=gv.data_ptr(), dg=gg.data_ptr(),
                c_out=m.out_channels, cin_g=cin_g, k=m.kernel, groups=m.groups, pg=f.pg,
                flags=_lib.PACK_UNFOLD if f.unfold else 0, dw_ld=ld, dw_span=span, row0=row0, tile0=tile0))
            row0 += m.out_channels
            if not self.need_wd:
                tile0 += m.kernel * f.pg if f.wd is not None else 0
            elif f.unfold:
                tile0 += -(-m.out_channels // 32) * -(-f.kp // 32)
            else:
                tile0 += m.kernel * f.pg * -(-(m.out_channels // f.pg) // 32) * -(-(m.in_channels // f.pg) // 32)
        self.n_items, self.total_rows, self.total_tiles = len(items), row0, (tile0 if self.need_wd else -tile0)
        self.item_row0 = [it.row0 for it in items] + [row0]
        self.table = ops.fold_table(items, dev)
        self._ptrs = [(p.data_ptr(), p.grad.data_ptr()) for m in self.wn for p in (m.weight_v, m.weight_g)]

    def _check_ptrs(self) -> None:
        cur = [(p.data_ptr(), p.grad.data_ptr() if p.grad is not None else 0) for m in self.wn for p in (m.weight_v, m.weight_g)]
        if cur != self._ptrs:
            raise RuntimeError("FoldPlan: parameter / gradient storage moved after the plan was built")

    def fold(self) -> Dict[int, Folded]:
        self._check_ptrs()
        ops.weightnorm_fold_multi(self.table, self.n_items, self.total_rows, self.total_tiles, self.dtype)
        return self.folds

    def zero(self) -> None:
        self.arena.zero_()

    def take(self, f: Folded) -> Tensor:
        ent = self._dw_off.get(id(f.mod))
        if ent is None:
            return torch.zeros(dw_layout(f)[0], device=self.device, dtype=torch.float32)
        return self.arena[ent[0]:ent[0] + ent[1]]

    def backward(self, accumulate: bool = True) -> None:
        self._check_ptrs()
        ops.weightnorm_fold_bwd_multi(self.table, self.n_items, self.total_rows, accumulate)


    def backward_range(self, item_lo: int, item_hi: int, accumulate: bool = True) -> None:
        self._check_ptrs()
        r0, r1 = self.item_row0[item_lo], self.item_row0[item_hi]
        if r1 > r0:
            ops.weightnorm_fold_bwd_range(self.table, self.n_items, r0, r1 - r0, accumulate)


def unfold_input(f: Folded, src: Tensor, B: int, t_src: int, phases: int = 1) -> Tensor:
    m = f.mod
    return ops.unfold(src, n_samples=B, phases=phases, t_src=t_src, t_dst=m.t_out(t_src), channels=m.in_channels,
                      k=m.kernel, dilation=m.dilation, stride=m.stride, pad=m.pad)


def _fwd(f: Folded, src: Tensor, B: int, t_src: int, *, phases: int = 1, act: int = ACT_NONE, want_raw: bool = False,
         want_act: bool = False, dup: bool = False, add_post: Optional[Tensor] = None, post_shift: int = 0,
         out_f32: bool = False, lengths: Optional[Tensor] = None, rate: int = 1) -> Tuple[Optional[Tensor], Optional[Tensor], int]:
    m = f.mod
    t_dst = m.t_out(t_src)
    odt = torch.float32 if out_f32 else f.dtype
    y_raw = torch.empty((B, t_dst * phases, m.out_channels), device=src.device, dtype=odt) if want_raw else None
    y_act = torch.empty((B, t_dst * phases * (2 if dup else 1), m.out_channels), device=src.device, dtype=odt) if want_act else None
    if f.unfold:
        ops.conv(src, f.wf, n_samples=B, phases=phases, t_src=t_dst, t_dst=t_dst, c_src=f.kp, c_dst=m.out_channels, k=1,
                 bias=m.bias.data, act=act, dup_rows=dup, add_post=add_post, post_shift=post_shift, y_raw=y_raw, y_act=y_act,
                 valid_units=lengths, rows_per_unit=rate)
    else:
        ops.conv(src, f.wf, n_samples=B, phases=phases, t_src=t_src, t_dst=t_dst, c_src=m.in_channels, c_dst=m.out_channels,
                 groups=f.pg, k=m.kernel, dilation=m.dilation, stride=m.stride, pad=m.pad, bias=m.bias.data, act=act,
                 dup_rows=dup, add_post=add_post, post_shift=post_shift, y_raw=y_raw, y_act=y_act, acct_groups=m.groups,
                 valid_units=lengths, rows_per_unit=rate)
    return y_raw, y_act, t_dst


def _dgrad(f: Folded, dy: Tensor, B: int, t_dy: int, t_x: int, *, phases: int = 1, mask: Optional[Tensor] = None,
           mask_mode: int = ACT_NONE, add_pre: Optional[Tensor] = None, add_post: Optional[Tensor] = None,
           pair_sum: bool = False, out_f32: bool = False) -> Tensor:
    m = f.mod
    if f.unfold:
        assert mask is None and add_pre is None and add_post is None and not pair_sum
        du = torch.empty((B, t_dy * phases, f.kp), device=dy.device, dtype=f.dtype)
        fwd_pack = f.dtype == torch.bfloat16
        ops.conv(dy, f.wf if fwd_pack else f.wd, n_samples=B, phases=phases, t_src=t_dy, t_dst=t_dy, c_src=m.out_channels,
                 c_dst=f.kp, k=1, transposed=True, y_raw=du, w_fwd_pack=fwd_pack)
        dx = torch.zeros((B, t_x * phases, m.in_channels), device=dy.device, dtype=torch.float32)
        ops.unfold_bwd(du, dx, n_samples=B, phases=phases, t_src=t_x, t_dst=t_dy, channels=m.in_channels, k=m.kernel,
                       dilation=m.dilation, stride=m.stride, pad=m.pad)
        return dx if out_f32 else ops.cast(dx, f.dtype)
    rows = t_x // 2 if pair_sum else t_x
    dx = torch.empty((B, rows * phases, m.in_channels), device=dy.device, dtype=torch.float32 if out_f32 else f.dtype)
    fwd_pack = f.dtype == torch.bfloat16 and not (m.groups > 1 and f.wd is not None)
    ops.conv(dy, f.wf if fwd_pack else f.wd, n_samples=B, phases=phases, t_src=t_dy, t_dst=t_x, c_src=m.out_channels,
             c_dst=m.in_channels, groups=f.pg, k=m.kernel, dilation=m.dilation, stride=m.stride, pad=m.pad, transposed=True,
             pair_sum=pair_sum, mask=mask, mask_mode=mask_mode, add_pre=add_pre, add_post=add_post, y_raw=dx,
             w_fwd_pack=fwd_pack, acct_groups=m.groups)
    return dx


def _wgrad(f: Folded, x: Tensor, dy: Tensor, B: int, t_x: int, t_dy: int, ws: _Workspace, phases: int = 1) -> None:
    m = f.mod
    side = ws.side_for_current() if getattr(ws, "wgrad_stream", None) is not None else None
    if side is not None:
        ev = torch.cuda.Event()
        ev.record(torch.cuda.current_stream())
        side.wait_event(ev)
        ws._keep.append((x, dy))
        with torch.cuda.stream(side):
            _wgrad_here(f, x, dy, B, t_x, t_dy, ws, phases)
        return
    _wgrad_here(f, x, dy, B, t_x, t_dy, ws, phases)


def _wgrad_here(f: Folded, x: Tensor, dy: Tensor, B: int, t_x: int, t_dy: int, ws, phases: int) -> None:
    m = f.mod
    dw = ws.take(f)
    if f.unfold:
        ops.wgrad(x, dy, dw, _grad_of(m.bias), n_samples=B, phases=phases, t_in=t_dy, t_out=t_dy, c_in=f.kp,
                  c_out=m.out_channels, k=1)
    else:
        ops.wgrad(x, dy, dw, _grad_of(m.bias), n_samples=B, phases=phases, t_in=t_x, t_out=t_dy, c_in=m.in_channels,
                  c_out=m.out_channels, groups=m.groups, k=m.kernel, dilation=m.dilation, stride=m.stride, pad=m.pad)
    if not (ws.deferred and m.norm == "weight_norm"):
        fold_backward(f, dw)


def generator_convs(model) -> List:
    convs = [model.gblocks[0]]
    for blk in list(model.gblocks)[1:]:
        c = blk.convs()
        convs += [c["c1"], c["c2"], c["res"], c["c3"], c["c4"]]
    convs.append(model.last_conv[1])
    return convs


def gblock_fwd(blk, folds: Dict[int, Folded], x_raw: Tensor, x_act: Tensor, B: int, t: int, *, want_raw: bool,
               want_act: bool, dup_next: bool, side=None, lengths: Optional[Tensor] = None, rate: int = 1):
    c = blk.convs()
    up = blk.upsample
    t_hi = t * up
    lo = dict(lengths=lengths, rate=rate)
    hi = dict(lengths=lengths, rate=rate * up)
    (r, _, _), (_, a1, _) = fork_join(
        side, lambda: _fwd(folds[id(c["res"])], x_raw, B, t, want_raw=True, **lo),
        lambda: _fwd(folds[id(c["c1"])], x_act, B, t_hi, act=ACT_RELU, want_act=True, **hi))
    h_raw, h_act, _ = _fwd(folds[id(c["c2"])], a1, B, t_hi, act=ACT_RELU, want_raw=True, want_act=True,
                           add_post=r, post_shift=1 if up > 1 else 0, **hi)
    _, a3, _ = _fwd(folds[id(c["c3"])], h_act, B, t_hi, act=ACT_RELU, want_act=True, **hi)
    y_raw, y_act, _ = _fwd(folds[id(c["c4"])], a3, B, t_hi, act=ACT_RELU, want_raw=want_raw, want_act=want_act,
                           add_post=h_raw, dup=dup_next, **hi)
    saved = dict(x_raw=x_raw, x_act=x_act, a1=a1, h_act=h_act, a3=a3, t_lo=t, t_hi=t_hi, up=up)
    return y_raw, y_act, saved


def gblock_bwd(blk, folds: Dict[int, Folded], s: dict, dy: Tensor, B: int, ws: _Workspace, out_f32: bool = False,
               side=None) -> Tensor:
    c = blk.convs()
    t_lo, t_hi, up = s["t_lo"], s["t_hi"], s["up"]
    f1, f2, fr, f3, f4 = (folds[id(c[k])] for k in ("c1", "c2", "res", "c3", "c4"))
    _wgrad(f4, s["a3"], dy, B, t_hi, t_hi, ws)
    da3 = _dgrad(f4, dy, B, t_hi, t_hi, mask=s["a3"], mask_mode=ACT_RELU)
    _wgrad(f3, s["h_act"], da3, B, t_hi, t_hi, ws)
    dh = _dgrad(f3, da3, B, t_hi, t_hi, mask=s["h_act"], mask_mode=ACT_RELU, add_post=dy)
    _wgrad(f2, s["a1"], dh, B, t_hi, t_hi, ws)

    def res_branch():
        dr = dh if up == 1 else ops.pair_sum_rows(dh, B * t_lo, fr.mod.out_channels).view(B, t_lo, -1)
        _wgrad(fr, s["x_raw"], dr, B, t_lo, t_lo, ws)
        return _dgrad(fr, dr, B, t_lo, t_lo), dr

    (dx_res, dr), da1 = fork_join(side, res_branch, lambda: _dgrad(f2, dh, B, t_hi, t_hi, mask=s["a1"], mask_mode=ACT_RELU))
    _wgrad(f1, s["x_act"], da1, B, t_hi, t_hi, ws)
    return _dgrad(f1, da1, B, t_hi, t_hi, pair_sum=up > 1, mask=s["x_raw"], mask_mode=ACT_RELU, add_post=dx_res,
                  out_f32=out_f32)


def fold_generator(model, dtype: torch.dtype, want_dgrad: bool = True, plan: Optional[FoldPlan] = None) -> Dict[int, Folded]:
    if plan is not None:
        return plan.fold()
    return {id(c): fold(c, dtype, want_dgrad=want_dgrad) for c in generator_convs(model)}


@dataclass
class GenCtx:
    B: int = 0
    T: int = 0
    dtype: torch.dtype = torch.float32
    folds: Dict[int, Folded] = field(default_factory=dict)
    x0: Optional[Tensor] = None
    ids: List[Optional[Tensor]] = field(default_factory=list)
    emb_dims: List[int] = field(default_factory=list)
    blocks: List[dict] = field(default_factory=list)
    y_last_act: Optional[Tensor] = None
    x_pred: Optional[Tensor] = None


def generator_forward(model, speech_units: Tensor, session_ids: Optional[Tensor], speaking_mode_ids: Optional[Tensor],
                      dtype: torch.dtype, need_ctx: bool, folds: Optional[Dict[int, Folded]] = None, side=None,
                      lengths: Optional[Tensor] = None):
    if need_ctx and lengths is not None:
        raise ValueError("generator_forward: length masks are forward-only (need_ctx=True with lengths)")
    su = speech_units.contiguous().float()
    B, T, du = su.shape
    if folds is None:
        folds = fold_generator(model, dtype, want_dgrad=need_ctx)
    tables, ids = [], []
    if model.use_session_embeddings:
        tables.append(model.session_embeddings.weight); ids.append(session_ids.to(torch.int64).contiguous())
    if model.use_speaking_mode_embedding:
        tables.append(model.speaking_mode_embeddings.weight); ids.append(speaking_mode_ids.to(torch.int64).contiguous())
    if len(tables) == 0:
        x0 = ops.cast(su, dtype)
    elif len(tables) == 1:
        x0 = ops.embed_concat(su, tables[0].data, ids[0], dtype)
    else:
        tmp = ops.embed_concat(su, tables[0].data, ids[0], torch.float32)
        x0 = ops.embed_concat(tmp, tables[1].data, ids[1], dtype)
    blocks = list(model.gblocks)[1:]
    ups = [b.upsample for b in blocks]
    for u in ups:
        if u not in (1, 2):
            raise ValueError("GBlock upsample must be 1 or 2 on this path")
    f0 = folds[id(model.gblocks[0])]
    if f0.unfold:
        x0 = unfold_input(f0, x0, B, T)
    x_raw, x_act, t = _fwd(f0, x0, B, T, act=ACT_RELU, want_raw=True, want_act=True, dup=ups[0] > 1, lengths=lengths)
    saved = []
    rate = 1
    for i, blk in enumerate(blocks):
        last = i + 1 == len(blocks)
        nxt_dup = (not last) and ups[i + 1] > 1
        y_raw, y_act, s = gblock_fwd(blk, folds, x_raw, x_act, B, t, want_raw=not last, want_act=True, dup_next=nxt_dup,
                                     side=side, lengths=lengths, rate=rate)
        if need_ctx:
            saved.append(s)
        x_raw, x_act, t = y_raw, y_act, s["t_hi"]
        rate *= s["up"]
    _, x_pred, _ = _fwd(folds[id(model.last_conv[1])], x_act, B, t, act=ACT_TANH, want_act=True, out_f32=True,
                        lengths=lengths, rate=rate)
    if not need_ctx:
        return x_pred, None
    ctx = GenCtx(B=B, T=T, dtype=dtype, folds=folds, x0=x0, ids=ids, emb_dims=[tb.shape[1] for tb in tables],
                 blocks=saved, y_last_act=x_act, x_pred=x_pred)
    ctx.tables = tables
    ctx.d_units = du
    ctx.t_out = t
    return x_pred, ctx


class GenBackward:

    def __init__(self, model, ctx: GenCtx, dx_pred: Tensor, plan: Optional[FoldPlan] = None, side=None, res_side=None,
                 overwrite_grads: bool = False):
        self.model, self.ctx, self.plan, self.side, self.res_side = model, ctx, plan, side, res_side
        self.accumulate = not overwrite_grads
        B, dtype, folds = ctx.B, ctx.dtype, ctx.folds
        if plan is not None:
            plan.zero()
            self.ws = plan
            if side is not None:
                plan.async_wgrads(side)
        else:
            self.ws = _Workspace([folds[id(c)] for c in generator_convs(model)], dx_pred.device)
        self.gblocks = list(model.gblocks)[1:]
        t = ctx.t_out
        dpre = ops.act_bwd(dx_pred.contiguous(), ctx.x_pred, ACT_TANH, dtype)
        f = folds[id(model.last_conv[1])]
        _wgrad(f, ctx.y_last_act, dpre, B, t, t, self.ws)
        self.dy = _dgrad(f, dpre, B, t, t, mask=ctx.y_last_act, mask_mode=ACT_RELU)

    def blocks(self, lo: int, hi: int) -> None:
        for i in reversed(range(lo, hi)):
            self.dy = gblock_bwd(self.gblocks[i], self.ctx.folds, self.ctx.blocks[i], self.dy, self.ctx.B, self.ws, side=self.res_side)

    def finish(self) -> None:
        model, ctx, dy, B = self.model, self.ctx, self.dy, self.ctx.B
        f0 = ctx.folds[id(model.gblocks[0])]
        _wgrad(f0, ctx.x0, dy, B, ctx.T, ctx.T, self.ws)
        if ctx.tables:
            dx0 = _dgrad(f0, dy, B, ctx.T, ctx.T)
            off = ctx.d_units
            if len(ctx.tables) == 1:
                ops.embed_concat_bwd(dx0, ctx.ids[0], off, _grad_of(ctx.tables[0]))
            else:
                d0, d1 = ctx.emb_dims
                ops.embed_concat_bwd(dx0[:, :, :off + d0].contiguous(), ctx.ids[0], off, _grad_of(ctx.tables[0]))
                ops.embed_concat_bwd(dx0, ctx.ids[1], off + d0, _grad_of(ctx.tables[1]))
        self.dy = None

    def bucket(self, item_lo: int, item_hi: int, last: bool = False) -> None:
        plan = self.plan
        if plan is None:
            return
        plan.join_wgrads()
        plan.backward_range(item_lo, item_hi, accumulate=self.accumulate)
        if not last and self.side is not None:
            plan.async_wgrads(self.side)


def generator_backward(model, ctx: GenCtx, dx_pred: Tensor, plan: Optional[FoldPlan] = None, side=None,
                       res_side=None, overwrite_grads: bool = False) -> None:
    gb = GenBackward(model, ctx, dx_pred, plan, side, res_side, overwrite_grads)
    gb.blocks(0, len(gb.gblocks))
    gb.finish()
    if plan is not None:
        plan.join_wgrads()
        plan.backward(accumulate=not overwrite_grads)


def fork_many(streams: Sequence["torch.cuda.Stream"], fns: Sequence) -> None:
    cur = torch.cuda.current_stream()
    ev = torch.cuda.Event()
    ev.record(cur)
    for st, fn in zip(streams, fns[1:]):
        st.wait_event(ev)
        with torch.cuda.stream(st):
            fn()
    fns[0]()
    for st in streams[:len(fns) - 1]:
        e2 = torch.cuda.Event()
        e2.record(st)
        cur.wait_event(e2)


def fork_join(side: Optional["torch.cuda.Stream"], fn_side, fn_main):
    if side is None:
        return fn_side(), fn_main()
    ev = torch.cuda.Event()
    ev.record(torch.cuda.current_stream())
    side.wait_event(ev)
    with torch.cuda.stream(side):
        ra = fn_side()
    rb = fn_main()
    ev2 = torch.cuda.Event()
    ev2.record(side)
    torch.cuda.current_stream().wait_event(ev2)
    return ra, rb


def disc_subnets(model) -> List[Tuple[str, object]]:
    return [("P", d) for d in model.multi_pooled_disc] + [("S", d) for d in model.multi_scale_disc]


def discriminator_convs(model) -> List:
    out = []
    for _, d in disc_subnets(model):
        out += list(d.layers) + [d.output]
    return out


def fold_discriminator(model, dtype: torch.dtype, training: bool = True, want_dgrad: bool = True,
                       reuse: Optional[Dict[int, Folded]] = None,
                       persist: Optional[Dict[int, Folded]] = None,
                       plan: Optional[FoldPlan] = None, refold: bool = True, sn_streams=None) -> Dict[int, Folded]:
    if plan is not None:
        sn = [c for c in discriminator_convs(model) if c.norm != "weight_norm"]
        if sn_streams and sn:
            cur = torch.cuda.current_stream()
            ev = torch.cuda.Event()
            ev.record(cur)
            out = dict(plan.fold() if refold else plan.folds)
            used = []
            for i, c in enumerate(sn):
                st = sn_streams[i % len(sn_streams)]
                if st not in used:
                    st.wait_event(ev)
                    used.append(st)
                with torch.cuda.stream(st):
                    out[id(c)] = fold(c, dtype, training=training, want_dgrad=want_dgrad)
            for st in used:
                e2 = torch.cuda.Event()
                e2.record(st)
                cur.wait_event(e2)
            return out
        out = dict(plan.fold() if refold else plan.folds)
        for c in sn:
            out[id(c)] = fold(c, dtype, training=training, want_dgrad=want_dgrad)
        return out
    out = {}
    for c in discriminator_convs(model):
        if reuse is not None and c.norm == "weight_norm" and id(c) in reuse:
            out[id(c)] = reuse[id(c)]
        else:
            out[id(c)] = fold(c, dtype, training=training, want_dgrad=want_dgrad, persist=persist)
    return out


@dataclass
class DiscCtx:
    B: int = 0
    T: int = 0
    C: int = 0
    dtype: torch.dtype = torch.float32
    folds: Dict[int, Folded] = field(default_factory=dict)
    subs: List[dict] = field(default_factory=list)


def _heavy_split(subs: Sequence) -> Tuple[List[int], List[int]]:
    heavy = [i for i, (kind, _) in enumerate(subs) if kind == "S"][:1]
    return heavy, [i for i in range(len(subs)) if i not in heavy]


def discriminator_forward(model, x: Tensor, dtype: torch.dtype, folds: Dict[int, Folded], side=None,
                          subset: Optional[Sequence[int]] = None, spread: Optional[Sequence] = None):
    x = x.contiguous().float()
    B, T, Cc = x.shape
    ctx = DiscCtx(B=B, T=T, C=Cc, dtype=dtype, folds=folds)
    subs = disc_subnets(model)
    wanted = set(range(len(subs)) if subset is None else subset)
    last_scale = max([i for i in wanted if subs[i][0] == "S"], default=-1)
    scale_in, xs = {}, x
    for i, (kind, d) in enumerate(subs):
        if kind == "S":
            scale_in[i] = xs
            if subset is None or i < last_scale:
                xs = ops.avgpool4(xs)
    results: List = [None] * len(subs)
    sub_ctx: List = [None] * len(subs)

    def run(idx: List[int]) -> None:
        for i in idx:
            kind, d = subs[i]
            fused0 = False
            if kind == "P":
                p = d.period
                t_pad = T + (p - T % p)
                phases, t = p, t_pad // p
                l0, f0_ = d.layers[0], folds[id(d.layers[0])]
                fused0 = (f0_.unfold and dtype == torch.bfloat16 and l0.groups == 1 and l0.dilation == 1 and
                          l0.out_channels % 8 == 0 and t_pad - T < T)
                src = None if fused0 else ops.reflect_pad_right(x, t_pad, dtype)
            else:
                src = ops.cast(scale_in[i], dtype)
                phases, t = 1, scale_in[i].shape[1]
            f0 = folds[id(d.layers[0])]
            if f0.unfold and not fused0:
                src = unfold_input(f0, src, B, t, phases)
            sub = dict(kind=kind, phases=phases, inputs=[src], ts=[t], t_in0=scale_in[i].shape[1] if kind == "S" else T, mod=d)
            fmaps = []
            h = src
            layers = list(d.layers)
            if fused0:
                l0 = layers[0]
                h, t = ops.period_first_layer(x, f0.wf, l0.bias.data, period=phases, c_out=l0.out_channels, k=l0.kernel,
                                              stride=l0.stride, pad=l0.pad, slope=0.1)
                fmaps.append(h); sub["inputs"].append(h); sub["ts"].append(t)
                sub["x0"] = x
                layers = layers[1:]
            for layer in layers:
                _, h, t = _fwd(folds[id(layer)], h, B, t, phases=phases, act=ACT_LEAKY, want_act=True)
                fmaps.append(h); sub["inputs"].append(h); sub["ts"].append(t)
            logits, _, t = _fwd(folds[id(d.output)], h, B, t, phases=phases, want_raw=True, out_f32=True)
            sub["ts"].append(t)
            fmaps.append(logits)
            if kind == "S":
                sub["x_scale"] = scale_in[i]
            results[i], sub_ctx[i] = fmaps, sub

    heavy, rest = _heavy_split(subs)
    heavy, rest = [i for i in heavy if i in wanted], [i for i in rest if i in wanted]
    if spread:
        todo = heavy + rest
        lanes = [todo[j::len(spread) + 1] for j in range(len(spread) + 1)]
        fork_many(list(spread), [(lambda idx=idx: run(idx)) for idx in lanes if idx])
    elif side is not None and heavy and rest:
        fork_join(side, lambda: run(heavy), lambda: run(rest))
    else:
        run(heavy + rest)
    ctx.subs = sub_ctx
    ctx.keep = (scale_in, xs)
    return results, ctx


def first_layer_input(sub: dict, f: Folded, B: int, dtype: torch.dtype) -> Tensor:
    x, p, t = sub["x0"], sub["phases"], sub["ts"][0]
    src = ops.reflect_pad_right(x, t * p, dtype)
    return unfold_input(f, src, B, t, p)


def split_disc_batch(results: List, ctx: DiscCtx, idx: Sequence[int], n_first: int):
    res_a: List = [None] * len(results)
    res_b: List = [None] * len(results)
    sub_a: List = [None] * len(results)
    for i in idx:
        res_a[i] = [fm[:n_first] for fm in results[i]]
        res_b[i] = [fm[n_first:] for fm in results[i]]
        sub = dict(ctx.subs[i])
        sub["inputs"] = [t[:n_first] if t is not None else None for t in sub["inputs"]]
        if "x0" in sub:
            sub["x0"] = sub["x0"][:n_first]
        if "x_scale" in sub:
            sub["x_scale"] = sub["x_scale"][:n_first]
        sub_a[i] = sub
    return res_a, res_b, sub_a


def discriminator_backward(model, ctx: DiscCtx, dlogits: Sequence[Optional[Tensor]],
                           dfmaps: Optional[Sequence[Sequence[Optional[Tensor]]]] = None, want_input_grad: bool = False,
                           want_weight_grad: bool = True, plan: Optional[FoldPlan] = None, side=None,
                           spread: Optional[Sequence] = None) -> Optional[Tensor]:
    B, T, Cc, dtype, folds = ctx.B, ctx.T, ctx.C, ctx.dtype, ctx.folds
    dev = next(sub for sub in ctx.subs if sub is not None)["inputs"][1].device
    if plan is not None and want_weight_grad:
        ws = plan
    else:
        ws = _Workspace([folds[id(c)] for c in discriminator_convs(model)], dev) if want_weight_grad else None
        if ws is not None:
            side = None
    dx = torch.zeros((B, T, Cc), device=dev, dtype=torch.float32) if want_input_grad else None
    n_sub = len(ctx.subs)
    scale_grad: List = [None] * n_sub

    def run(idx: List[int]) -> None:
        for di in idx:
            sub = ctx.subs[di]
            if sub is None:
                continue
            d, phases, inputs, ts = sub["mod"], sub["phases"], sub["inputs"], sub["ts"]
            convs = list(d.layers) + [d.output]
            g = dlogits[di]
            fm_g = dfmaps[di] if dfmaps is not None else None
            if g is None and (fm_g is None or all(t is None for t in fm_g)):
                continue
            if g is None:
                g = torch.zeros((B, ts[-1] * phases, 1), device=dev, dtype=dtype)
            dxin = None
            for j in reversed(range(len(convs))):
                f = folds[id(convs[j])]
                if want_weight_grad:
                    xin = inputs[j] if inputs[j] is not None else first_layer_input(sub, f, B, dtype)
                    _wgrad(f, xin, g, B, ts[j], ts[j + 1], ws, phases=phases)
                if j == 0:
                    if want_input_grad:
                        dxin = _dgrad(f, g, B, ts[1], ts[0], phases=phases, out_f32=True)
                    break
                g = _dgrad(f, g, B, ts[j + 1], ts[j], phases=phases, mask=inputs[j], mask_mode=ACT_LEAKY,
                           add_pre=fm_g[j - 1] if fm_g is not None else None)
            if want_input_grad:
                if sub["kind"] == "P":
                    ops.reflect_pad_right_bwd(dxin, T, dx)
                else:
                    scale_grad[di] = dxin

    heavy, rest = _heavy_split([(sub["kind"] if sub is not None else "-", None) for sub in ctx.subs])
    if spread and (plan is not None or not want_weight_grad):
        h_here = [i for i in heavy if ctx.subs[i] is not None] if side is not None else []
        todo = [i for i in range(n_sub) if ctx.subs[i] is not None and i not in h_here]
        lanes = [l for l in (todo[j::len(spread) + 1] for j in range(len(spread) + 1)) if l]
        fns = [(lambda idx=idx: run(idx)) for idx in lanes] or [lambda: None]
        streams = list(spread)[:len(fns) - 1]
        if h_here:
            fns.append(lambda: run(h_here)); streams.append(side)
        fork_many(streams, fns)
    elif side is not None and heavy and any(ctx.subs[i] is not None for i in rest):
        fork_join(side, lambda: run(heavy), lambda: run(rest))
    else:
        run(list(range(n_sub)))
    if want_input_grad:
        carry = None
        for di in reversed([i for i, sub in enumerate(ctx.subs) if sub is not None and sub["kind"] == "S"]):
            t_in, cur = ctx.subs[di]["t_in0"], scale_grad[di]
            if carry is not None:
                if cur is None:
                    cur = torch.zeros((B, t_in, Cc), device=dev, dtype=torch.float32)
                ops.avgpool4_bwd(carry, t_in, cur)
            carry = cur
        if carry is not None:
            ops.axpy_f32(dx, carry, 1.0)
    return dx


def to_reference_layout(fm: Tensor, kind: str, phases: int) -> Tensor:
    B, HP, Cc = fm.shape
    if kind == "P":
        return fm.view(B, HP // phases, phases, Cc).permute(0, 3, 1, 2)
    return fm.transpose(1, 2)


def single_conv_forward(mod, x: Tensor) -> Tensor:
    from .autograd import SingleConvFn
    return SingleConvFn.apply(mod, x, *[p for p in mod.parameters()])


def gblock_forward_torch_layout(blk, x: Tensor) -> Tensor:
    from .autograd import GBlockFn
    return GBlockFn.apply(blk, x, *[p for p in blk.parameters()])
```

### ste_gan_b200/trainer.py

```python
from __future__ import annotations

from typing import Dict, List, Optional

import torch
from . import ops, passes
from .dist import GradReducer

Tensor = torch.Tensor

W_TD_DEFAULT, W_FM_DEFAULT = 15.0, 7.0
LOSS_NAMES = ["loss_d", "loss_adv", "loss_fm", "loss_td_20_8", "loss_td_51_13", "loss_td_80_16", "loss_speech_unit", "loss_phoneme"]
W_SU_DEFAULT, W_PH_DEFAULT = 1.0, 1.0


class FlatParams:

    def __init__(self, module: torch.nn.Module):
        self.params = [p for p in module.parameters()]
        dev = self.params[0].device
        if dev.type != "cuda":
            raise RuntimeError("FlatParams: move the module to a CUDA device first")
        al = lambda k: (k + 3) // 4 * 4
        n = sum(al(p.numel()) for p in self.params)
        self.flat = torch.zeros(n, device=dev, dtype=torch.float32)
        self.grad = torch.zeros(n, device=dev, dtype=torch.float32)
        off = 0
        self.offsets: Dict[str, int] = {}
        names = [nm for nm, _ in module.named_parameters()]
        for nm, p in zip(names, self.params):
            k = p.numel()
            self.flat[off:off + k].copy_(p.data.reshape(-1))
            p.data = self.flat[off:off + k].view(p.shape)
            p.grad = self.grad[off:off + k].view(p.shape)
            self.offsets[nm] = off
            off += al(k)
        self.m = torch.zeros_like(self.flat)
        self.v = torch.zeros_like(self.flat)
        self.step = torch.zeros(1, device=dev, dtype=torch.int64)
        self.numel = n

    def zero_grad(self) -> None:
        self.grad.zero_()

    def adamw(self, lr, betas=(0.8, 0.99), eps: float = 1e-8, weight_decay: float = 1e-2,
              grad_scale: float = 1.0, enable: Optional[Tensor] = None, lo: int = 0, hi: Optional[int] = None,
              keep_step: bool = False) -> None:
        hi = self.numel if hi is None else hi
        ops.adamw(self.flat[lo:hi], self.grad[lo:hi], self.m[lo:hi], self.v[lo:hi], self.step, lr, betas[0], betas[1], eps,
                  weight_decay, grad_scale, enable, keep_step)


def generator_grad_buckets(offsets: Dict[str, int], numel: int, nblk: int) -> list:
    first = [offsets[next(nm for nm in offsets if nm.startswith(f"gblocks.{i + 1}."))] for i in range(nblk)]
    last = offsets[next(nm for nm in offsets if nm.startswith("last_conv."))]
    near = lambda frac, lo: min(range(lo, nblk), key=lambda i: abs(first[i] - frac * numel), default=nblk)
    k1 = near(1.0 / 3.0, 1)
    k2 = near(2.0 / 3.0, k1)
    n_conv = 5 * nblk + 2
    cut = lambda i: first[i] if i < nblk else last
    return [(k2, nblk, 1 + 5 * k2, n_conv, (cut(k2), numel)),
            (k1, k2, 1 + 5 * k1, 1 + 5 * k2, (cut(k1), cut(k2))),
            (0, k1, 0, 1 + 5 * k1, (0, cut(k1)))]


class GanTrainer:
    def __init__(self, net_g, net_d, precision: str = "bf16", lr: float = 2e-4, w_td: float = W_TD_DEFAULT,
                 w_fm: float = W_FM_DEFAULT, loss_adversarial: bool = True, loss_multi_td: bool = True,
                 loss_feat_match: bool = True, group=None, grad_buckets: Optional[int] = None, data_parallel: bool = True,
                 emg_encoder=None, loss_speech_unit: Optional[bool] = None, loss_phoneme: Optional[bool] = None,
                 w_su: float = W_SU_DEFAULT, w_ph: float = W_PH_DEFAULT):
        self.net_g, self.net_d = net_g, net_d
        self.dtype = torch.bfloat16 if precision == "bf16" else torch.float32
        self.w_td, self.w_fm = w_td, w_fm
        self.use_adv, self.use_td, self.use_fm = loss_adversarial, loss_multi_td, loss_feat_match
        self.emg_encoder = emg_encoder
        self.use_su = (emg_encoder is not None) if loss_speech_unit is None else bool(loss_speech_unit)
        self.use_ph = (emg_encoder is not None) if loss_phoneme is None else bool(loss_phoneme)
        if (self.use_su or self.use_ph) and emg_encoder is None:
            raise ValueError("loss_speech_unit / loss_phoneme need an emg_encoder")
        self.w_su, self.w_ph = w_su, w_ph
        self._enc_plan = None
        if emg_encoder is not None:
            if emg_encoder.training:
                raise ValueError("the EMG encoder of the perceptual losses is frozen: call emg_encoder.eval() (emg_encoder_loss.py:61)")
            self._enc_plan = emg_encoder.plan(self.dtype)
        self._cur_su = self._cur_ph = None
        self.G, self.D = FlatParams(net_g), FlatParams(net_d)
        self.g_plan = passes.FoldPlan(passes.generator_convs(net_g), self.dtype)
        self.d_plan = passes.FoldPlan(passes.discriminator_convs(net_d), self.dtype)
        self._d_folded = False
        self.reducer = GradReducer(group, enabled=data_parallel)
        self._inline = self.reducer.comm is not None
        dev = self.G.flat.device
        self.device = dev
        self.base_lr = float(lr)
        self._lr = float(lr)
        self.lr_dev = torch.full((1,), float(lr), device=dev, dtype=torch.float32)
        self.slots = torch.zeros(8, device=dev, dtype=torch.float32)
        self.d_folds: Optional[Dict[int, passes.Folded]] = None
        self._d_persist: Dict[int, passes.Folded] = {}
        self._graphs = None
        self._d_graphs = None
        self._pending_g = None
        self._static = None
        self.x_pred: Optional[Tensor] = None
        self._side = torch.cuda.Stream(device=dev)
        self._side2 = [torch.cuda.Stream(device=dev), torch.cuda.Stream(device=dev)]
        self._wg = [torch.cuda.Stream(device=dev) for _ in range(7)]
        self._ps = [torch.cuda.Stream(device=dev) for _ in range(2)]
        self._ss = [torch.cuda.Stream(device=dev)]
        self._sn = [torch.cuda.Stream(device=dev) for _ in range(4)]
        self._aux = torch.cuda.Stream(device=dev)
        self._enc = torch.cuda.Stream(device=dev)
        self._comm = torch.cuda.Stream(device=dev)
        self._pend = torch.zeros(1, device=dev, dtype=torch.int32)
        self._fused = None
        self._pending_host = False
        self._sm_reserve, self._n_sm = 0, torch.cuda.get_device_properties(dev).multi_processor_count
        self.concurrent_d = True
        import os
        self._d_slices = self._disc_grad_slices() if os.environ.get("STG_D_BUCKETS", "1") != "0" else None
        self.g_buckets = generator_grad_buckets(self.G.offsets, self.G.numel, len(list(net_g.gblocks)) - 1)
        if grad_buckets is None and os.environ.get("STG_G_BUCKETS"):
            grad_buckets = int(os.environ["STG_G_BUCKETS"])
        if (grad_buckets if grad_buckets is not None else (3 if self.reducer.enabled else 1)) == 1:
            nblk = len(list(net_g.gblocks)) - 1
            self.g_buckets = [(0, nblk, 0, 5 * nblk + 2, (0, self.G.numel))]

    @property
    def lr(self) -> float:
        return self._lr

    @lr.setter
    def lr(self, value: float) -> None:
        self.flush()
        self._lr = float(value)
        self.lr_dev.fill_(self._lr)

    def scheduler_step(self, gamma: float = 0.999) -> float:
        self.lr = self._lr * gamma
        return self._lr

    def _disc_grad_slices(self):
        subs = passes.disc_subnets(self.net_d)
        heavy, rest = passes._heavy_split(subs)
        if len(heavy) != 1 or any(i > heavy[0] for i in rest if subs[i][0] == "P") or any(i < heavy[0] for i in rest if subs[i][0] == "S"):
            return None
        wn = self.d_plan.wn
        def item_range(mods):
            ids = [k for k, m in enumerate(wn) if any(m is c for d_ in mods for c in list(d_.layers) + [d_.output])]
            return (ids[0], ids[-1] + 1) if ids and ids == list(range(ids[0], ids[-1] + 1)) else None
        def grad_range(prefixes):
            offs = [o for nm, o in self.D.offsets.items() if nm.startswith(tuple(prefixes))]
            nxt = [o for nm, o in self.D.offsets.items() if o > max(offs) and not nm.startswith(tuple(prefixes))]
            return min(offs), (min(nxt) if nxt else self.D.numel)
        p_mods = [subs[i][1] for i in rest if subs[i][0] == "P"]
        s_mods = [subs[i][1] for i in rest if subs[i][0] == "S"]
        h_mods = [subs[heavy[0]][1]]
        names = {id(m): nm for nm, m in self.net_d.named_modules()}
        pre = lambda mods: [names[id(m)] + "." for m in mods]
        out = dict(early=[], late=None)
        for mods in (p_mods, s_mods):
            if mods:
                ir = item_range(mods)
                if ir is None:
                    return None
                out["early"].append((ir, grad_range(pre(mods))))
        ir = item_range(h_mods)
        if ir is None:
            return None
        out["late"] = (ir, grad_range(pre(h_mods)))
        cover = sorted([g for _, g in out["early"]] + [out["late"][1]])
        if cover[0][0] != 0 or cover[-1][1] != self.D.numel or any(a[1] != b[0] for a, b in zip(cover, cover[1:])):
            return None
        return out

    def _s2(self, i: int):
        return self._side2[i] if self.concurrent_d else None

    def _fold_d(self, refold: bool):
        return passes.fold_discriminator(self.net_d, self.dtype, training=True, plan=self.d_plan, refold=refold,
                                         sn_streams=self._sn if self.concurrent_d else None)

    def _reduce(self, flat_slice: Tensor):
        if not self.reducer.enabled or flat_slice.numel() == 0:
            return None
        ev = torch.cuda.Event()
        ev.record(torch.cuda.current_stream())
        self._comm.wait_event(ev)
        self.reducer.all_reduce_on(flat_slice, self._comm)
        done = torch.cuda.Event()
        done.record(self._comm)
        return done

    @staticmethod
    def _wait_events(evs) -> None:
        for e in evs:
            if e is not None:
                torch.cuda.current_stream().wait_event(e)

    def _sm_scope(self, on: bool) -> None:
        if self._sm_reserve > 0:
            from . import _lib as _l
            _l.load().stg_set_sm_limit(self._n_sm - self._sm_reserve if on else 0)

    def _fork(self) -> None:
        ev = torch.cuda.Event()
        ev.record(torch.cuda.current_stream())
        self._side.wait_event(ev)

    def _join(self) -> None:
        ev = torch.cuda.Event()
        ev.record(self._side)
        torch.cuda.current_stream().wait_event(ev)

    def _d_folds(self) -> None:
        refold_d = not self._d_folded
        self._d_folded = True
        self._f1 = self._fold_d(refold_d)
        self._ev_f1 = torch.cuda.Event()
        self._ev_f1.record(torch.cuda.current_stream())
        self._f2 = self._fold_d(False)

    def _split_subs(self):
        subs = passes.disc_subnets(self.net_d)
        heavy, rest = passes._heavy_split(subs)
        return subs, heavy, [i for i in rest if subs[i][0] == "P"], [i for i in rest if subs[i][0] == "S"]

    def _d_real(self, x_real: Tensor) -> None:
        self._x_real = x_real
        if self.concurrent_d:
            _, heavy, _, _ = self._split_subs()
            self._real = passes.discriminator_forward(self.net_d, x_real, self.dtype, self._f2, subset=heavy) if heavy else (None, None)
        else:
            self._real = passes.discriminator_forward(self.net_d, x_real, self.dtype, self._f2)

    def _g_forward(self, su: Tensor, sess: Tensor, mode: Optional[Tensor], x_pred: Optional[Tensor] = None) -> None:
        self.slots.zero_()
        self.G.zero_grad(); self.D.zero_grad()
        self._gctx = None
        self._cur_su = su
        if x_pred is not None:
            self.x_pred = x_pred
            return
        self.x_pred, self._gctx = passes.generator_forward(self.net_g, su, sess, mode, self.dtype, True, folds=self.g_plan.fold(),
                                                           side=self._s2(1) if self.use_adv else None)

    def _d_fake(self) -> None:
        dt = self.dtype
        if not self.concurrent_d:
            self._fake = passes.discriminator_forward(self.net_d, self.x_pred, dt, self._f1)
            return
        _, heavy, p_idx, s_idx = self._split_subs()
        fwd = lambda x, idx: passes.discriminator_forward(self.net_d, x, dt, self._f1, subset=idx,
                                                          spread=self._ps if idx is p_idx else (self._ss if idx is s_idx else None)) if idx else (None, None)
        x_cat = torch.cat([self.x_pred, self._x_real], 0)
        ((rs, cs), (rp, cp)), (rh, ch) = passes.fork_join(
            self._s2(1), lambda: passes.fork_join(self._s2(0), lambda: fwd(x_cat, p_idx), lambda: fwd(x_cat, s_idx))[::-1],
            lambda: fwd(self.x_pred, heavy))
        self._fake = (rh, ch)
        self._batched = (rp, cp, rs, cs, x_cat)

    def _d_update(self) -> None:
        dt = self.dtype
        if not self.concurrent_d:
            (res_f, ctx_f), (res_r, ctx_r) = self._fake, self._real
            self._fake = self._real = None
            self._last_d_fmaps = (res_f, res_r, ctx_f)
            nd = len(res_f)
            dl = ops.mse_const_multi([fm[-1] for fm in res_f] + [fm[-1] for fm in res_r], [0.0] * nd + [1.0] * nd, self.slots,
                                     [0] * (2 * nd), 1.0, dt)
            self.d_plan.zero()
            passes.discriminator_backward(self.net_d, ctx_f, dl[:nd], None, want_input_grad=False, want_weight_grad=True, plan=self.d_plan)
            passes.discriminator_backward(self.net_d, ctx_r, dl[nd:], None, want_input_grad=False, want_weight_grad=True, plan=self.d_plan)
            self.d_plan.backward(accumulate=False)
            self._reduce_d()
            return
        subs, heavy, p_idx, s_idx = self._split_subs()
        (rh_f, ch_f), (rh_r, ch_r) = self._fake, self._real
        rp, cp, rs, cs, x_cat = self._batched
        self._fake = self._real = self._batched = None
        Bq, nd = self.x_pred.shape[0], len(subs)
        res_f, res_r = [None] * nd, [None] * nd
        for r_b, c_b, idx in ((rp, cp, p_idx), (rs, cs, s_idx)):
            if idx:
                a, b, _ = passes.split_disc_batch(r_b, c_b, idx, Bq)
                for i in idx:
                    res_f[i], res_r[i] = a[i], b[i]
        for i in heavy:
            res_f[i], res_r[i] = rh_f[i], rh_r[i]
        self._last_d_fmaps = (res_f, res_r, ch_f)
        dcat = {i: torch.empty((2 * Bq,) + tuple(res_f[i][-1].shape[1:]), device=self.device, dtype=dt) for i in p_idx + s_idx}
        outs = [dcat[i][:Bq] if i in dcat else None for i in range(nd)] + [dcat[i][Bq:] if i in dcat else None for i in range(nd)]
        dl = ops.mse_const_multi([fm[-1] for fm in res_f] + [fm[-1] for fm in res_r], [0.0] * nd + [1.0] * nd, self.slots,
                                 [0] * (2 * nd), 1.0, dt, outs=outs)
        dl_f, dl_r = dl[:nd], dl[nd:]
        dl_b = [dcat.get(i) for i in range(nd)]
        self.d_plan.zero()
        cur = torch.cuda.current_stream()
        self.d_plan.async_wgrads({st.cuda_stream: w for st, w in zip((cur, self._side, self._side2[0], self._side2[1], *self._ps, *self._ss), self._wg)})
        bwd = lambda ctx, dlog: passes.discriminator_backward(self.net_d, ctx, dlog, None, want_input_grad=False,
                                                              want_weight_grad=True, plan=self.d_plan,
                                                              spread=self._ps if ctx is cp else (self._ss if ctx is cs else None)) if ctx is not None else None
        only = lambda dlog, idx: [dlog[i] if i in idx else None for i in range(nd)]
        self._fork()
        with torch.cuda.stream(self._side):
            passes.fork_join(self._s2(0), lambda: bwd(ch_r, only(dl_r, heavy)), lambda: bwd(ch_f, only(dl_f, heavy)))
        passes.fork_join(self._s2(1), lambda: bwd(cs, only(dl_b, s_idx)), lambda: bwd(cp, only(dl_b, p_idx)))
        early = []
        if self._inline and heavy and self._d_slices is not None:
            self.d_plan.join_wgrads_of([cur, self._side2[1], *self._ps, *self._ss])
            for (i_lo, i_hi), (g_lo, g_hi) in self._d_slices["early"]:
                self.d_plan.backward_range(i_lo, i_hi, accumulate=False)
                early.append(self._reduce(self.D.grad[g_lo:g_hi]))
        self._join()
        self.d_plan.join_wgrads()
        if early:
            (i_lo, i_hi), (g_lo, g_hi) = self._d_slices["late"]
            self.d_plan.backward_range(i_lo, i_hi, accumulate=False)
            self._wait_events(early + [self._reduce(self.D.grad[g_lo:g_hi])])
            return
        self.d_plan.backward(accumulate=False)
        self._reduce_d()

    def _reduce_d(self) -> None:
        if self._inline:
            self._wait_events([self._reduce(self.D.grad)])

    def _phase_d(self, su: Tensor, sess: Tensor, mode: Optional[Tensor], x_real: Tensor, x_pred: Optional[Tensor] = None,
                 head=None) -> None:
        head = head or (lambda: None)
        if not self.use_adv:
            head()
            self._g_forward(su, sess, mode, x_pred)
            return
        if self.concurrent_d:
            cur = torch.cuda.current_stream()
            self._fork()
            self._sm_scope(True)
            with torch.cuda.stream(self._side):
                self._d_folds()
                self._d_real(x_real)
            head()
            self._sm_scope(False)
            self._g_forward(su, sess, mode, x_pred)
            cur.wait_event(self._ev_f1)
            self._d_fake()
            self._join()
        else:
            self._d_folds()
            head()
            self._g_forward(su, sess, mode, x_pred)
            self._d_fake()
            self._d_real(x_real)
        self._sm_scope(True)
        self._d_update()
        self._sm_scope(False)

    def _phase_g_head(self, x_real: Tensor, update_d: bool = True) -> None:
        dx_pred = self._g_losses(x_real, update_d)
        self._last_gctx = self._gctx
        self._gb = passes.GenBackward(self.net_g, self._gctx, dx_pred, plan=self.g_plan, side=self._s2(1), res_side=self._s2(0),
                                      overwrite_grads=True)
        self._g_bucket(0)

    def _g_losses(self, x_real: Tensor, update_d: bool = True) -> Tensor:
        dt = self.dtype
        x_pred = self.x_pred
        dx_pred = torch.zeros_like(x_pred)
        td_ev = None
        enc_ev, dx_enc = None, None
        if self.use_su or self.use_ph:
            from . import passes_encoder as pe
            if self._cur_ph is None:
                raise ValueError("the phoneme loss needs phoneme_targets ([B, frames] int64) in step() / step_graph()")
            ev = torch.cuda.Event()
            ev.record(torch.cuda.current_stream())
            self._enc.wait_event(ev)
            with torch.cuda.stream(self._enc if self.concurrent_d else torch.cuda.current_stream()):
                dx_enc, self._enc_units, self._enc_logits = pe.encoder_losses(
                    self._enc_plan, x_pred, self._cur_su, self._cur_ph, self.slots[6:8], self.w_su, self.w_ph, True,
                    self.use_su, self.use_ph)
                enc_ev = torch.cuda.Event()
                enc_ev.record(torch.cuda.current_stream())
        if self.use_td and self.use_adv and self.concurrent_d:
            ev = torch.cuda.Event()
            ev.record(torch.cuda.current_stream())
            self._aux.wait_event(ev)
            with torch.cuda.stream(self._aux):
                ops.td_loss(x_real, x_pred, self.slots[3:6], [self.w_td] * 3, dx_pred)
                td_ev = torch.cuda.Event()
                td_ev.record(self._aux)
        if self.use_adv:
            if update_d:
                self.D.adamw(self.lr_dev, grad_scale=self.reducer.grad_scale)
            refold_d = update_d or not self._d_folded
            self._d_folded = True
            if self.concurrent_d:
                subs = passes.disc_subnets(self.net_d)
                heavy, rest = passes._heavy_split(subs)
                p_idx = [i for i in rest if subs[i][0] == "P"]
                s_idx = [i for i in rest if subs[i][0] == "S"]
                Bq = x_pred.shape[0]
                f3 = self._fold_d(refold_d)
                x_cat = torch.cat([x_pred, x_real], 0)
                fwd = lambda x, f, idx: passes.discriminator_forward(self.net_d, x, dt, f, subset=idx,
                                                                     spread=self._ps if idx is p_idx else (self._ss if idx is s_idx else None)) if idx else (None, None)
                self._fork()
                with torch.cuda.stream(self._side):
                    (rs, cs), (rh_f, ch_f) = passes.fork_join(self._s2(0), lambda: fwd(x_cat, f3, s_idx), lambda: fwd(x_pred, f3, heavy))
                f4 = self._fold_d(False)
                (rh_r, _), (rp, cp) = passes.fork_join(self._s2(1), lambda: fwd(x_real, f4, heavy), lambda: fwd(x_cat, f3, p_idx))
                self._join()
                res_f, res_r, sub_f = [None] * len(subs), [None] * len(subs), [None] * len(subs)
                for r_b, c_b, idx in ((rp, cp, p_idx), (rs, cs, s_idx)):
                    if idx:
                        a, b, sa = passes.split_disc_batch(r_b, c_b, idx, Bq)
                        for i in idx:
                            res_f[i], res_r[i], sub_f[i] = a[i], b[i], sa[i]
                for i in heavy:
                    res_f[i], res_r[i], sub_f[i] = rh_f[i], rh_r[i], ch_f.subs[i]
                assert all(r is not None for r in res_f)
                ctx_f = passes.DiscCtx(B=Bq, T=x_pred.shape[1], C=x_pred.shape[2], dtype=dt, folds=f3, subs=sub_f)
                ctx_f.keep = (ch_f, cp, cs, x_cat)
            else:
                f3 = self._fold_d(refold_d)
                f4 = self._fold_d(False)
                res_f, ctx_f = passes.discriminator_forward(self.net_d, x_pred, dt, f3)
                res_r, _ = passes.discriminator_forward(self.net_d, x_real, dt, f4)
            self.d_folds = f4
            self._last_g_fmaps = (res_f, res_r)
            nd = len(res_f)
            dlog = ops.mse_const_multi([fm[-1] for fm in res_f], [1.0] * nd, self.slots, [1] * nd, 1.0, dt)
            if self.use_fm:
                pairs = [(a, b) for fm_f, fm_r in zip(res_f, res_r) for a, b in zip(fm_f[:-1], fm_r[:-1])]
                grads = ops.l1_mean_multi(pairs, self.slots[2:3], self.w_fm)
                dfm, i = [], 0
                for fm_f in res_f:
                    dfm.append(grads[i:i + len(fm_f) - 1]); i += len(fm_f) - 1
            else:
                dfm = [[None] * (len(fm_f) - 1) for fm_f in res_f]
            dx_d = passes.discriminator_backward(self.net_d, ctx_f, dlog, dfm, want_input_grad=True, want_weight_grad=False,
                                                 side=self._s2(0), spread=self._ps if self.concurrent_d else None)
            if td_ev is not None:
                torch.cuda.current_stream().wait_event(td_ev)
            ops.axpy_f32(dx_pred, dx_d, 1.0)
        if self.use_td and td_ev is None:
            ops.td_loss(x_real, x_pred, self.slots[3:6], [self.w_td] * 3, dx_pred)
        if dx_enc is not None:
            torch.cuda.current_stream().wait_event(enc_ev)
            ops.axpy_f32(dx_pred, dx_enc, 1.0)
        return dx_pred

    def _g_bucket(self, i: int) -> None:
        lo, hi, c_lo, c_hi, _ = self.g_buckets[i]
        gb = self._gb
        gb.blocks(lo, hi)
        if i == len(self.g_buckets) - 1:
            gb.finish()
        gb.bucket(c_lo, c_hi, last=i == len(self.g_buckets) - 1)
        if i == len(self.g_buckets) - 1:
            self._gb = self._gctx = None

    def _phase_g(self, x_real: Tensor, update_d: bool = True, reduce: bool = False, defer_last: bool = False) -> list:
        handles = []
        self._phase_g_head(x_real, update_d)
        n = len(self.g_buckets)
        for i in range(n):
            if i > 0:
                self._g_bucket(i)
            if reduce and not (defer_last and i == n - 1):
                handles += self._reduce_g_bucket(i)
        return handles

    def _reduce_g_bucket(self, i: int) -> list:
        lo, hi = self.g_buckets[i][4]
        if self._inline:
            return [self._reduce(self.G.grad[lo:hi])]
        return self.reducer.all_reduce_async(self.G.grad[lo:hi]) if hi > lo else []

    def _wait_handles(self, handles) -> None:
        if self._inline:
            self._wait_events(handles)
        else:
            self.reducer.wait(handles)

    def _phase_opt_g(self) -> None:
        self.G.adamw(self.lr_dev, grad_scale=self.reducer.grad_scale)

    def _opt_g_head(self) -> None:
        n = len(self.g_buckets)
        lo, hi = self.g_buckets[n - 1][4]
        if self._inline:
            self._wait_events(self._reduce_g_bucket(n - 1))
        self.G.adamw(self.lr_dev, grad_scale=self.reducer.grad_scale, enable=self._pend, lo=lo, hi=hi, keep_step=n > 1)

    def _fused_step(self, s: dict) -> None:
        self._phase_d(s["su"], s["sess"], s["mode"], s["x_real"], head=self._opt_g_head)
        self._phase_g_head(s["x_real"])
        n, evs = len(self.g_buckets), []
        for i in range(n - 1):
            if i > 0:
                self._g_bucket(i)
            lo, hi = self.g_buckets[i][4]
            ev = self._reduce(self.G.grad[lo:hi])
            self._sm_scope(True)
            if ev is None:
                ev = torch.cuda.Event()
                ev.record(torch.cuda.current_stream())
                self._comm.wait_event(ev)
            with torch.cuda.stream(self._comm):
                self.G.adamw(self.lr_dev, grad_scale=self.reducer.grad_scale, lo=lo, hi=hi, keep_step=i > 0)
                done = torch.cuda.Event()
                done.record(self._comm)
            evs.append(done)
        if n > 1:
            self._g_bucket(n - 1)
        self._sm_scope(False)
        self._wait_events(evs)
        self._pend.fill_(1)

    def step(self, speech_units: Tensor, session_ids: Tensor, x_real: Tensor,
             speaking_mode_ids: Optional[Tensor] = None, phoneme_targets: Optional[Tensor] = None) -> Tensor:
        self.flush()
        su = speech_units.contiguous().float()
        xr = x_real.contiguous().float()
        self._cur_ph = phoneme_targets
        self._phase_d(su, session_ids, speaking_mode_ids, xr)
        if not self._inline:
            self.reducer.all_reduce(self.D.grad)
        self._wait_handles(self._phase_g(xr, reduce=True))
        self._phase_opt_g()
        return self.slots

    def disc_losses_step(self, x_pred: Tensor, x_real: Tensor) -> Tensor:
        self._phase_d(None, None, None, x_real, x_pred=x_pred)
        return self._g_losses(x_real, update_d=True)

    def capture(self, batch: int, frames: int, unit_dim: int = 256, hop: int = 16, channels: int = 8,
                pipelined: Optional[bool] = None, fused: Optional[bool] = None) -> None:
        dev = self.device
        import os
        if fused is None:
            fused = pipelined is None and os.environ.get("STG_FUSED_GRAPH", "1") != "0"
        if pipelined is None:
            pipelined = self.concurrent_d and self.use_adv and os.environ.get("STG_PIPELINE", "1") != "0"
        self.flush()
        self._fused = None
        self._static = dict(
            su=torch.zeros(batch, frames, unit_dim, device=dev), sess=torch.zeros(batch, device=dev, dtype=torch.int64),
            x_real=torch.zeros(batch, frames * hop, channels, device=dev),
            mode=torch.zeros(batch, device=dev, dtype=torch.int64) if self.net_g.use_speaking_mode_embedding else None,
            ph=torch.zeros(batch, frames, device=dev, dtype=torch.int64) if (self.use_su or self.use_ph) else None)
        s = self._static
        self._cur_ph = s["ph"]
        snap = self._snapshot_state()
        side = torch.cuda.Stream()
        side.wait_stream(torch.cuda.current_stream())
        with torch.cuda.stream(side):
            for _ in range(2):
                self.step(s["su"], s["sess"], s["x_real"], s["mode"], s["ph"])
        torch.cuda.current_stream().wait_stream(side)
        torch.cuda.synchronize()
        self._restore_state(snap)
        torch.cuda.synchronize()
        pool = torch.cuda.graph_pool_handle()
        G = torch.cuda.CUDAGraph
        gkw = dict(capture_error_mode="thread_local") if self.reducer.enabled else {}
        if fused:
            from . import _lib as _l
            reserve = int(os.environ.get("STG_NCCL_SMS", "16")) if self.reducer.enabled else 0
            n_sm = torch.cuda.get_device_properties(dev).multi_processor_count
            step_g, flush_g = G(), G()
            self._pend.zero_()
            scoped = os.environ.get("STG_NCCL_SCOPE", "0") == "1"
            if reserve > 0:
                if scoped:
                    self._sm_reserve = reserve
                else:
                    _l.load().stg_set_sm_limit(n_sm - reserve)
            try:
                with torch.cuda.graph(step_g, pool=pool, **gkw):
                    self._fused_step(s)
            finally:
                self._sm_reserve = 0
                if reserve > 0:
                    _l.load().stg_set_sm_limit(0)
            with torch.cuda.graph(flush_g, pool=pool, **gkw):
                self._opt_g_head()
            self._pend.zero_()
            self._fused, self._graphs, self._d_graphs, self._pending_host = (step_g, flush_g), None, None, False
            return
        import contextlib, os
        from . import _lib
        reserve = int(os.environ.get("STG_NCCL_SMS", "0")) if self.reducer.enabled else 0
        n_sm = torch.cuda.get_device_properties(dev).multi_processor_count

        @contextlib.contextmanager
        def beside_allreduce():
            if reserve > 0:
                _lib.load().stg_set_sm_limit(n_sm - reserve)
            try:
                yield
            finally:
                if reserve > 0:
                    _lib.load().stg_set_sm_limit(0)
        if pipelined:
            pool_a = torch.cuda.graph_pool_handle()
            a1, a2, b1, b2, b3 = G(), G(), G(), G(), G()
            with beside_allreduce():
                with torch.cuda.graph(a1, pool=pool_a, **gkw):
                    self._d_folds()
                with torch.cuda.graph(a2, pool=pool_a, **gkw):
                    self._d_real(s["x_real"])
            with torch.cuda.graph(b1, pool=pool, **gkw):
                self._g_forward(s["su"], s["sess"], s["mode"])
            with torch.cuda.graph(b2, pool=pool, **gkw):
                self._d_fake()
            with torch.cuda.graph(b3, pool=pool, **gkw):
                self._d_update()
            self._d_graphs = (a1, a2, b1, b2, b3)
            self._pipe = torch.cuda.Stream(device=dev)
            self._pipe_ev = [torch.cuda.Event() for _ in range(3)]
            g1 = None
        else:
            self._d_graphs = None
            g1 = G()
            with torch.cuda.graph(g1, pool=pool, **gkw):
                self._phase_d(s["su"], s["sess"], s["mode"], s["x_real"])
        g2 = [G() for _ in self.g_buckets]
        with torch.cuda.graph(g2[0], pool=pool, **gkw):
            self._phase_g_head(s["x_real"])
        for i in range(1, len(g2)):
            with beside_allreduce(), torch.cuda.graph(g2[i], pool=pool, **gkw):
                self._g_bucket(i)
        g3 = G()
        with torch.cuda.graph(g3, pool=pool, **gkw):
            self._phase_opt_g()
        self._graphs = (g1, g2, g3)

    def _sn_buffers(self) -> list:
        return [b for c in passes.discriminator_convs(self.net_d) if c.norm != "weight_norm" for b in (c.weight_u, c.weight_v)]

    def _snapshot_state(self) -> dict:
        return dict(flat=[(fp, fp.flat.clone(), fp.m.clone(), fp.v.clone(), fp.step.clone()) for fp in (self.G, self.D)],
                    sn=[(b, b.clone()) for b in self._sn_buffers()], slots=self.slots.clone())

    def _restore_state(self, snap: dict) -> None:
        for fp, flat, m, v, step in snap["flat"]:
            fp.flat.copy_(flat); fp.m.copy_(m); fp.v.copy_(v); fp.step.copy_(step)
            fp.grad.zero_()
        for b, val in snap["sn"]:
            b.copy_(val)
        self.slots.copy_(snap["slots"])
        self._pend.zero_()
        self._pending_host = False
        self.refold()

    def refold(self) -> None:
        self.d_plan.fold()
        self._d_folded = True

    def flush(self) -> None:
        if self._pending_host and self._fused is not None:
            self._pending_host = False
            self._fused[1].replay()
        if self._pending_g is not None:
            self._wait_handles(self._pending_g)
            self._pending_g = None
            self._graphs[2].replay()

    def step_graph(self, speech_units: Tensor, session_ids: Tensor, x_real: Tensor,
                   speaking_mode_ids: Optional[Tensor] = None, phoneme_targets: Optional[Tensor] = None) -> Tensor:
        s = self._static
        s["su"].copy_(speech_units, non_blocking=True)
        s["sess"].copy_(session_ids, non_blocking=True)
        s["x_real"].copy_(x_real, non_blocking=True)
        if s["mode"] is not None:
            if speaking_mode_ids is None:
                raise ValueError("step_graph: this generator uses speaking-mode embeddings - pass speaking_mode_ids")
            s["mode"].copy_(speaking_mode_ids, non_blocking=True)
        if s["ph"] is not None:
            if phoneme_targets is None:
                raise ValueError("step_graph: the EMG-encoder losses are on - pass phoneme_targets")
            s["ph"].copy_(phoneme_targets, non_blocking=True)
        if self._fused is not None:
            self._fused[0].replay()
            self._pending_host = True
            return self.slots
        g1, g2, g3 = self._graphs
        def phase_g() -> list:
            handles = []
            for i, gr in enumerate(g2):
                gr.replay()
                handles += self._reduce_g_bucket(i)
            return handles
        if self._d_graphs is None:
            g1.replay()
            if not self._inline:
                self.reducer.all_reduce(self.D.grad)
            self._wait_handles(phase_g())
            g3.replay()
            return self.slots
        a1, a2, b1, b2, b3 = self._d_graphs
        ev0, ev_f, ev_r = self._pipe_ev
        cur = torch.cuda.current_stream()
        ev0.record(cur)
        self._pipe.wait_event(ev0)
        with torch.cuda.stream(self._pipe):
            a1.replay(); ev_f.record(self._pipe)
            a2.replay(); ev_r.record(self._pipe)
        self.flush()
        b1.replay()
        cur.wait_event(ev_f)
        b2.replay()
        cur.wait_event(ev_r)
        b3.replay()
        if not self._inline:
            self.reducer.all_reduce(self.D.grad)
        self._pending_g = phase_g()
        return self.slots

    def save_checkpoint(self, directory, steps: int, epoch: int, final: bool = False) -> None:
        from . import checkpoint
        checkpoint.save_checkpoint(self, directory, steps, epoch, final)

    def load_latest_checkpoint(self, directory):
        from . import checkpoint
        return checkpoint.load_latest_checkpoint(self, directory)

    def losses(self) -> Dict[str, float]:
        v = self.slots.tolist()
        out = dict(zip(LOSS_NAMES, v[:8]))
        out["loss_td"] = v[3] + v[4] + v[5]
        out["loss_g"] = v[1] + self.w_td * out["loss_td"] + self.w_fm * v[2] + \
            (self.w_su * v[6] if self.use_su else 0.0) + (self.w_ph * v[7] if self.use_ph else 0.0)
        return out
```

Before: 4034.

## Fuse weight-norm backward, AdamW update and refold into one row kernel

Adds a kernel that, per weight-norm conv row, computes the fold backward (dv/dg), applies AdamW directly to v, g and their moments, then refolds the effective weight. A second block range in the same launch updates the plain parameters in flat chunks. This replaces the separate fold-backward, full-flat AdamW and refold launches and skips their round trips through the dv/dg grad buffer. It applies only to the single-bucket, non-data-parallel bf16 path. Zeroing of grads is narrowed to the plain ranges, and a later forward reuses the already refolded weights. The cost is more complex bookkeeping of fold state, plus fused-path numerics that use explicit fma rounding.

```diff
diff --git a/include/stegan_b200.h b/include/stegan_b200.h
--- a/include/stegan_b200.h
+++ b/include/stegan_b200.h
@@ -97,6 +97,16 @@
 int stg_weightnorm_fold_bwd_range(const StgFoldItem* items, int n_items, int row_base, int n_rows, int accumulate,
                                   stg_stream_t stream);
 
+#define STG_UPDATE_CHUNK 2048
+typedef struct StgFlatRange {
+  int64_t lo, n;
+  int32_t blk0, pad;
+} StgFlatRange;
+int stg_weightnorm_update_multi(const StgFoldItem* items, int n_items, int total_rows, int wd_blocks, const StgFlatRange* ranges,
+                                int n_ranges, int range_blocks, int dtype, float* p, const float* g, float* m, float* v,
+                                float lr, const float* lr_dev, float beta1, float beta2, float eps, float weight_decay,
+                                int64_t* step_count, float grad_scale, int32_t* enable, stg_stream_t stream);
+
 int stg_tc_pack_groups(int c_in, int c_out, int groups);
 
 int stg_unfold(const void* src, int dtype, int B, int phases, int t_src, int t_dst, int C, int k, int dilation, int stride,
diff --git a/ste_gan_b200/_lib.py b/ste_gan_b200/_lib.py
--- a/ste_gan_b200/_lib.py
+++ b/ste_gan_b200/_lib.py
@@ -11,6 +11,7 @@
 ENGINE_AUTO, ENGINE_SIMT, ENGINE_TCGEN05 = 0, 1, 2
 PACK_UNFOLD = 1
 MAX_TAPS = 48
+UPDATE_CHUNK = 2048
 
 
 class StgConv(C.Structure):
@@ -29,6 +30,10 @@
 class StgFoldItem(C.Structure):
     _fields_ = [(n, C.c_void_p) for n in ("v", "g", "wf", "wd", "scale", "dw", "dv", "dg")] + [
         (n, C.c_int32) for n in ("c_out", "cin_g", "k", "groups", "pg", "flags", "dw_ld", "dw_span", "row0", "tile0")]
+
+
+class StgFlatRange(C.Structure):
+    _fields_ = [("lo", C.c_int64), ("n", C.c_int64), ("blk0", C.c_int32), ("pad", C.c_int32)]
 
 
 class StgL1Item(C.Structure):
@@ -60,6 +65,7 @@
     "stg_weightnorm_fold_multi": [_P, _I, _I, _I, _I, _P],
     "stg_weightnorm_fold_bwd_multi": [_P, _I, _I, _I, _P],
     "stg_weightnorm_fold_bwd_range": [_P, _I, _I, _I, _I, _P],
+    "stg_weightnorm_update_multi": [_P, _I, _I, _I, _P, _I, _I, _I, _P, _P, _P, _P, _F, _P, _F, _F, _F, _F, _P, _F, _P, _P],
     "stg_debug_set_trace": [_P],
     "stg_debug_rowshift": [_P, _P, _I, _I, _I, _P, _P],
     "stg_debug_row_classes": [_I, _P],
diff --git a/ste_gan_b200/csrc/common.cuh b/ste_gan_b200/csrc/common.cuh
--- a/ste_gan_b200/csrc/common.cuh
+++ b/ste_gan_b200/csrc/common.cuh
@@ -90,6 +90,26 @@
   return r;
 }
 
+struct AdamwCoef {
+  float b1, b2, eps, gscale, step_size, inv_sqrt_bc2, decay;
+};
+static __device__ __noinline__ AdamwCoef adamw_coef(float lr_host, const float* lr_dev, float b1, float b2, float eps, float wd,
+                                                    const int64_t* step, float gscale) {
+  const float lr = lr_dev ? *lr_dev : lr_host;
+  const float t = (float)(*step);
+  const float bc1 = 1.f - powf(b1, t), bc2 = 1.f - powf(b2, t);
+  return AdamwCoef{b1, b2, eps, gscale, lr / bc1, rsqrtf(bc2), 1.f - lr * wd};
+}
+__device__ __forceinline__ void adamw_elem(const AdamwCoef& c, float grad, float& p, float& m, float& v) {
+  const float gi = __fmul_rn(grad, c.gscale);
+  const float mi = __fmaf_rn(c.b1, m, __fmul_rn(1.f - c.b1, gi));
+  const float vi = __fmaf_rn(c.b2, v, __fmul_rn(__fmul_rn(1.f - c.b2, gi), gi));
+  m = mi;
+  v = vi;
+  const float denom = __fmaf_rn(sqrtf(vi), c.inv_sqrt_bc2, c.eps);
+  p = __fmaf_rn(-c.step_size, mi / denom, __fmul_rn(p, c.decay));
+}
+
 static inline int64_t ceil_div64(int64_t a, int64_t b) { return (a + b - 1) / b; }
 static inline int ceil_div(int a, int b) { return (a + b - 1) / b; }
 
@@ -106,6 +126,8 @@
 bool wgrad_c1_supported(const StgWgrad* d);
 int wgrad_c1(const StgWgrad* d, cudaStream_t s);
 void conv_tc_set_trace(long long* buf);
+int adamw_step_inc(int64_t* step, const int32_t* enable, cudaStream_t s);
+int adamw_flag_clear(int32_t* enable, cudaStream_t s);
 void wgrad_tc_layout(const StgWgrad* d, int* ld, int* span);
 
 }
diff --git a/ste_gan_b200/csrc/misc.cu b/ste_gan_b200/csrc/misc.cu
--- a/ste_gan_b200/csrc/misc.cu
+++ b/ste_gan_b200/csrc/misc.cu
@@ -133,18 +133,13 @@
                                                     float wd, const int64_t* __restrict__ step, float gscale,
                                                     const int32_t* __restrict__ enable) {
   if (enable != nullptr && *enable == 0) return;
-  const float lr = lr_dev ? *lr_dev : lr_host;
-  const float t = (float)(*step);
-  const float bc1 = 1.f - powf(b1, t), bc2 = 1.f - powf(b2, t);
-  const float step_size = lr / bc1, inv_sqrt_bc2 = rsqrtf(bc2), decay = 1.f - lr * wd;
+  const AdamwCoef c = adamw_coef(lr_host, lr_dev, b1, b2, eps, wd, step, gscale);
   for (int64_t i = (int64_t)blockIdx.x * blockDim.x + threadIdx.x; i < n; i += (int64_t)gridDim.x * blockDim.x) {
-    const float gi = g[i] * gscale;
-    const float mi = b1 * m[i] + (1.f - b1) * gi;
-    const float vi = b2 * v[i] + (1.f - b2) * gi * gi;
+    float pi = p[i], mi = m[i], vi = v[i];
+    adamw_elem(c, g[i], pi, mi, vi);
     m[i] = mi;
     v[i] = vi;
-    const float denom = sqrtf(vi) * inv_sqrt_bc2 + eps;
-    p[i] = p[i] * decay - step_size * (mi / denom);
+    p[i] = pi;
   }
 }
 
@@ -195,6 +190,18 @@
 }
 
 }
+
+int adamw_step_inc(int64_t* step, const int32_t* enable, cudaStream_t s) {
+  step_inc_kernel<<<1, 1, 0, s>>>(step, enable);
+  STG_LAUNCH_CHECK();
+  return STG_OK;
+}
+int adamw_flag_clear(int32_t* enable, cudaStream_t s) {
+  flag_clear_kernel<<<1, 1, 0, s>>>(enable);
+  STG_LAUNCH_CHECK();
+  return STG_OK;
+}
+
 }
 
 using namespace stg;
@@ -306,15 +313,12 @@
                          int flags, stg_stream_t stream) {
   if (!p || !g || !m || !v || !step_count) return STG_EINVAL;
   if (!(flags & STG_ADAMW_KEEP_STEP)) {
-    step_inc_kernel<<<1, 1, 0, S_>>>(step_count, enable);
-    STG_LAUNCH_CHECK();
+    const int rc = adamw_step_inc(step_count, enable, S_);
+    if (rc != STG_OK) return rc;
   }
   adamw_kernel<<<grid_for(n), 256, 0, S_>>>(p, g, m, v, n, lr, lr_dev, beta1, beta2, eps, weight_decay, step_count, grad_scale, enable);
   STG_LAUNCH_CHECK();
-  if (enable) {
-    flag_clear_kernel<<<1, 1, 0, S_>>>(enable);
-    STG_LAUNCH_CHECK();
-  }
+  if (enable) return adamw_flag_clear(enable, S_);
   return STG_OK;
 }
 
diff --git a/ste_gan_b200/csrc/norm_fold.cu b/ste_gan_b200/csrc/norm_fold.cu
--- a/ste_gan_b200/csrc/norm_fold.cu
+++ b/ste_gan_b200/csrc/norm_fold.cu
@@ -350,13 +350,61 @@
   }
 }
 
-template <int K>
-__device__ __forceinline__ void fold_bwd_row_warp(const StgFoldItem& d, int co, int lane, int accumulate) {
+struct GradOut {
+  int accumulate;
+  __device__ __forceinline__ void put4(const StgFoldItem& d, int co, int i, float4 r, float4) const {
+    float4* o = reinterpret_cast<float4*>(d.dv + (int64_t)co * d.cin_g * d.k + i);
+    if (accumulate) { const float4 p = *o; r.x += p.x; r.y += p.y; r.z += p.z; r.w += p.w; }
+    *o = r;
+  }
+  __device__ __forceinline__ void put(const StgFoldItem& d, int co, int i, float val, float) const {
+    float* o = d.dv + (int64_t)co * d.cin_g * d.k + i;
+    *o = accumulate ? (*o + val) : val;
+  }
+  __device__ __forceinline__ void put_g(const StgFoldItem& d, int co, float val, float) const {
+    d.dg[co] = accumulate ? (d.dg[co] + val) : val;
+  }
+};
+struct AdamwOut {
+  const float* p;
+  float* m;
+  float* s;
+  AdamwCoef c;
+  __device__ __forceinline__ void put4(const StgFoldItem& d, int co, int i, float4 r, float4 x) const {
+    const int64_t off = (d.v - p) + (int64_t)co * d.cin_g * d.k + i;
+    float4 mm = *reinterpret_cast<const float4*>(m + off), ss = *reinterpret_cast<const float4*>(s + off);
+    adamw_elem(c, r.x, x.x, mm.x, ss.x);
+    adamw_elem(c, r.y, x.y, mm.y, ss.y);
+    adamw_elem(c, r.z, x.z, mm.z, ss.z);
+    adamw_elem(c, r.w, x.w, mm.w, ss.w);
+    *reinterpret_cast<float4*>(m + off) = mm;
+    *reinterpret_cast<float4*>(s + off) = ss;
+    *reinterpret_cast<float4*>(const_cast<float*>(d.v) + (int64_t)co * d.cin_g * d.k + i) = x;
+  }
+  __device__ __forceinline__ void put(const StgFoldItem& d, int co, int i, float val, float x) const {
+    const int64_t off = (d.v - p) + (int64_t)co * d.cin_g * d.k + i;
+    float mm = m[off], ss = s[off];
+    adamw_elem(c, val, x, mm, ss);
+    m[off] = mm;
+    s[off] = ss;
+    const_cast<float*>(d.v)[(int64_t)co * d.cin_g * d.k + i] = x;
+  }
+  __device__ __forceinline__ void put_g(const StgFoldItem& d, int co, float val, float x) const {
+    const int64_t off = (d.g - p) + co;
+    float mm = m[off], ss = s[off];
+    adamw_elem(c, val, x, mm, ss);
+    m[off] = mm;
+    s[off] = ss;
+    const_cast<float*>(d.g)[co] = x;
+  }
+};
+
+template <int K, typename Out>
+__device__ __forceinline__ void fold_bwd_row_warp(const StgFoldItem& d, int co, int lane, const Out& out) {
   const int cin = d.cin_g, ng = cin >> 2;
   const int span = d.dw_span > 0 ? d.dw_span : cin, ld = d.dw_ld > 0 ? d.dw_ld : span * K;
   const float4* v4 = reinterpret_cast<const float4*>(d.v + (int64_t)co * cin * K);
   const float* dr = d.dw + (int64_t)co * ld;
-  float4* o4 = reinterpret_cast<float4*>(d.dv + (int64_t)co * cin * K);
   float ss = 0.f, dot = 0.f;
   for (int g = lane; g < ng; g += 32) {
     float f[4 * K], w[K][4];
@@ -380,29 +428,20 @@
   const float norm = sqrtf(ss), gg = d.g[co];
   const float a = gg / norm, bcoef = gg * dot / (norm * ss);
   for (int g = lane; g < ng; g += 32) {
-    float f[4 * K], w[K][4], o[4 * K];
 #pragma unroll
     for (int q = 0; q < K; ++q) {
       const float4 x = v4[g * K + q];
-      f[4 * q] = x.x; f[4 * q + 1] = x.y; f[4 * q + 2] = x.z; f[4 * q + 3] = x.w;
-    }
-#pragma unroll
-    for (int j = 0; j < K; ++j) {
-      const float4 x = *reinterpret_cast<const float4*>(dr + j * span + 4 * g);
-      w[j][0] = x.x; w[j][1] = x.y; w[j][2] = x.z; w[j][3] = x.w;
-    }
-#pragma unroll
-    for (int c = 0; c < 4; ++c)
-#pragma unroll
-      for (int j = 0; j < K; ++j) o[c * K + j] = a * w[j][c] - bcoef * f[c * K + j];
-#pragma unroll
-    for (int q = 0; q < K; ++q) {
-      float4 r = make_float4(o[4 * q], o[4 * q + 1], o[4 * q + 2], o[4 * q + 3]);
-      if (accumulate) { const float4 p = o4[g * K + q]; r.x += p.x; r.y += p.y; r.z += p.z; r.w += p.w; }
-      o4[g * K + q] = r;
-    }
-  }
-  if (lane == 0) d.dg[co] = accumulate ? (d.dg[co] + dot / norm) : dot / norm;
+      const float f[4] = {x.x, x.y, x.z, x.w};
+      float o[4];
+#pragma unroll
+      for (int e = 0; e < 4; ++e) {
+        const int j = (4 * q + e) % K, c = (4 * q + e) / K;
+        o[e] = __fmaf_rn(a, dr[j * span + 4 * g + c], -__fmul_rn(bcoef, f[e]));
+      }
+      out.put4(d, co, 4 * (g * K + q), make_float4(o[0], o[1], o[2], o[3]), x);
+    }
+  }
+  if (lane == 0) out.put_g(d, co, dot / norm, gg);
 }
 
 template <typename T>
@@ -470,12 +509,12 @@
   }
 }
 
-__device__ __forceinline__ void fold_bwd_row_warp_generic(const StgFoldItem& d, int co, int lane, int accumulate) {
+template <typename Out>
+__device__ __forceinline__ void fold_bwd_row_warp_generic(const StgFoldItem& d, int co, int lane, const Out& out) {
   const int n = d.cin_g * d.k, k = d.k, cin_g = d.cin_g;
   const int span = d.dw_span > 0 ? d.dw_span : cin_g, ld = d.dw_ld > 0 ? d.dw_ld : span * k;
   const float* vr = d.v + (int64_t)co * n;
   const float* dr = d.dw + (int64_t)co * ld + span_goff(co, cin_g, d.c_out / d.groups, span);
-  float* orow = d.dv + (int64_t)co * n;
   float ss = 0.f, dot = 0.f;
   const int total = k * cin_g;
   for (int i = lane; i < total; i += 32) {
@@ -490,10 +529,10 @@
   const float a = gg / norm, bcoef = gg * dot / (norm * ss);
   for (int i = lane; i < n; i += 32) {
     const int ci = i / k, j = i - ci * k;
-    const float val = a * dr[j * span + ci] - bcoef * vr[i];
-    orow[i] = accumulate ? (orow[i] + val) : val;
-  }
-  if (lane == 0) d.dg[co] = accumulate ? (d.dg[co] + dot / norm) : dot / norm;
+    const float x = vr[i];
+    out.put(d, co, i, __fmaf_rn(a, dr[j * span + ci], -__fmul_rn(bcoef, x)), x);
+  }
+  if (lane == 0) out.put_g(d, co, dot / norm, gg);
 }
 
 __global__ void __launch_bounds__(256, 4) wn_bwd_multi_kernel(const StgFoldItem* __restrict__ items, int n_items, int row_base,
@@ -506,10 +545,60 @@
   for (int r = w_begin; r < w_end; ++r) {
     while (r >= d.row0 + d.c_out) d = items[++it];
     const int co = r - d.row0;
-    if (!fold_bwd_fast(d)) fold_bwd_row_warp_generic(d, co, lane, accumulate);
-    else if (d.k == 3) fold_bwd_row_warp<3>(d, co, lane, accumulate);
-    else if (d.k == 1) fold_bwd_row_warp<1>(d, co, lane, accumulate);
-    else fold_bwd_row_warp<5>(d, co, lane, accumulate);
+    const GradOut out{accumulate};
+    if (!fold_bwd_fast(d)) fold_bwd_row_warp_generic(d, co, lane, out);
+    else if (d.k == 3) fold_bwd_row_warp<3>(d, co, lane, out);
+    else if (d.k == 1) fold_bwd_row_warp<1>(d, co, lane, out);
+    else fold_bwd_row_warp<5>(d, co, lane, out);
+  }
+}
+
+template <typename T>
+__global__ void __launch_bounds__(256, 4) wn_update_rows_kernel(const StgFoldItem* __restrict__ items, int n_items, int total_rows,
+                                                              const StgFlatRange* __restrict__ ranges, int n_ranges, float* p,
+                                                              const float* __restrict__ grad, float* m, float* s, float lr_host,
+                                                              const float* __restrict__ lr_dev, float b1, float b2, float eps,
+                                                              float wd, const int64_t* __restrict__ step, float gscale,
+                                                              const int32_t* __restrict__ enable) {
+  if (enable != nullptr && *enable == 0) return;
+  const AdamwOut out{p, m, s, adamw_coef(lr_host, lr_dev, b1, b2, eps, wd, step, gscale)};
+  const int row_blocks = (total_rows + FOLD_RPB - 1) / FOLD_RPB;
+  if ((int)blockIdx.x >= row_blocks) {
+    const int b = blockIdx.x - row_blocks;
+    int lo = 0, hi = n_ranges - 1;
+    while (lo < hi) {
+      const int mid = (lo + hi + 1) >> 1;
+      if (ranges[mid].blk0 <= b) lo = mid; else hi = mid - 1;
+    }
+    const StgFlatRange r = ranges[lo];
+    const int64_t i0 = r.lo + (int64_t)(b - r.blk0) * STG_UPDATE_CHUNK;
+    const int64_t i1 = min(r.lo + r.n, i0 + STG_UPDATE_CHUNK);
+    for (int64_t i = i0 + threadIdx.x; i < i1; i += 256) {
+      float pi = p[i], mi = m[i], si = s[i];
+      adamw_elem(out.c, grad[i], pi, mi, si);
+      m[i] = mi;
+      s[i] = si;
+      p[i] = pi;
+    }
+    return;
+  }
+  const int warp = threadIdx.x >> 5, lane = threadIdx.x & 31;
+  const int w_begin = blockIdx.x * FOLD_RPB + warp * FOLD_RPW, w_end = min(total_rows, w_begin + FOLD_RPW);
+  if (w_begin >= w_end) return;
+  int it = find_item(items, n_items, w_begin, false);
+  for (int r = w_begin; r < w_end; ++r) {
+    while (r >= items[it].row0 + items[it].c_out) ++it;
+    const StgFoldItem& d = items[it];
+    const int co = r - d.row0;
+    if (!fold_bwd_fast(d)) fold_bwd_row_warp_generic(d, co, lane, out);
+    else if (d.k == 3) fold_bwd_row_warp<3>(d, co, lane, out);
+    else if (d.k == 1) fold_bwd_row_warp<1>(d, co, lane, out);
+    else fold_bwd_row_warp<5>(d, co, lane, out);
+    __syncwarp();
+    if (!fold_fast(d)) fold_row_warp_generic<T>(d, co, lane);
+    else if (d.k == 3) fold_row_warp<T, 3>(d, co, lane);
+    else if (d.k == 1) fold_row_warp<T, 1>(d, co, lane);
+    else fold_row_warp<T, 5>(d, co, lane);
   }
 }
 
@@ -705,3 +794,32 @@
   STG_LAUNCH_CHECK();
   return STG_OK;
 }
+
+extern "C" int stg_weightnorm_update_multi(const StgFoldItem* items, int n_items, int total_rows, int wd_blocks,
+                                           const StgFlatRange* ranges, int n_ranges, int range_blocks, int dtype, float* p,
+                                           const float* g, float* m, float* v, float lr, const float* lr_dev, float beta1,
+                                           float beta2, float eps, float weight_decay, int64_t* step_count, float grad_scale,
+                                           int32_t* enable, stg_stream_t stream) {
+  cudaStream_t s = static_cast<cudaStream_t>(stream);
+  if (!items || n_items < 1 || total_rows < 1 || wd_blocks < 0 || n_ranges < 0 || range_blocks < 0 ||
+      (n_ranges > 0) != (range_blocks > 0) || (n_ranges > 0 && !ranges) || !p || !g || !m || !v || !step_count)
+    return STG_EINVAL;
+  if (dtype != STG_F32 && dtype != STG_BF16) return STG_EINVAL;
+  if (dtype == STG_F32 && wd_blocks > 0) return STG_EINVAL;
+  int rc = adamw_step_inc(step_count, enable, s);
+  if (rc != STG_OK) return rc;
+  const int blocks = ceil_div(total_rows, FOLD_RPB) + range_blocks;
+  if (dtype == STG_F32)
+    wn_update_rows_kernel<float><<<blocks, 256, 0, s>>>(items, n_items, total_rows, ranges, n_ranges, p, g, m, v, lr, lr_dev,
+                                                        beta1, beta2, eps, weight_decay, step_count, grad_scale, enable);
+  else
+    wn_update_rows_kernel<bf16><<<blocks, 256, 0, s>>>(items, n_items, total_rows, ranges, n_ranges, p, g, m, v, lr, lr_dev,
+                                                       beta1, beta2, eps, weight_decay, step_count, grad_scale, enable);
+  STG_LAUNCH_CHECK();
+  if (wd_blocks > 0) {
+    wd_from_wf_kernel<bf16><<<wd_blocks, 256, 0, s>>>(items, n_items);
+    STG_LAUNCH_CHECK();
+  }
+  if (enable) return adamw_flag_clear(enable, s);
+  return STG_OK;
+}
diff --git a/ste_gan_b200/ops.py b/ste_gan_b200/ops.py
--- a/ste_gan_b200/ops.py
+++ b/ste_gan_b200/ops.py
@@ -254,6 +254,33 @@
           "stg_weightnorm_fold_multi")
 
 
+def flat_range_table(ranges: list, device) -> Tuple[Tensor, int]:
+    items, blk = [], 0
+    for lo, hi in ranges:
+        items.append(_lib.StgFlatRange(lo=lo, n=hi - lo, blk0=blk, pad=0))
+        blk += -(-(hi - lo) // _lib.UPDATE_CHUNK)
+    arr = (_lib.StgFlatRange * max(1, len(items)))(*items)
+    return torch.frombuffer(bytearray(bytes(arr)), dtype=torch.uint8).to(device), blk
+
+
+def weightnorm_update_multi(table: Tensor, n_items: int, total_rows: int, total_tiles: int, ranges: Tensor, n_ranges: int,
+                            range_blocks: int, dtype: torch.dtype, p: Tensor, g: Tensor, m: Tensor, v: Tensor, step: Tensor,
+                            lr: Tensor, beta1: float = 0.8, beta2: float = 0.99, eps: float = 1e-8, weight_decay: float = 0.01,
+                            grad_scale: float = 1.0, enable: Optional[Tensor] = None) -> None:
+    if total_tiles > 0:
+        raise ValueError("weightnorm_update_multi: needs a row-form fold table (total_tiles <= 0)")
+    n = p.numel()
+    for t, nm in ((p, "p"), (g, "g"), (m, "m"), (v, "v")):
+        _need(t, n, torch.float32, nm)
+    _need(step, 1, torch.int64, "step")
+    _need(lr, 1, torch.float32, "lr")
+    _need(enable, 1, torch.int32, "enable")
+    check(_lib.load().stg_weightnorm_update_multi(_ptr(table), n_items, total_rows, -total_tiles, _ptr(ranges), n_ranges,
+                                                  range_blocks, code_of(dtype), _ptr(p), _ptr(g), _ptr(m), _ptr(v), 0.0,
+                                                  _ptr(lr), beta1, beta2, eps, weight_decay, _ptr(step), grad_scale,
+                                                  _ptr(enable), _stream()), "stg_weightnorm_update_multi")
+
+
 def weightnorm_fold_bwd_multi(table: Tensor, n_items: int, total_rows: int, accumulate: bool = True) -> None:
     check(_lib.load().stg_weightnorm_fold_bwd_multi(_ptr(table), n_items, total_rows, int(accumulate), _stream()),
           "stg_weightnorm_fold_bwd_multi")
diff --git a/ste_gan_b200/passes.py b/ste_gan_b200/passes.py
--- a/ste_gan_b200/passes.py
+++ b/ste_gan_b200/passes.py
@@ -468,12 +468,13 @@
                 ops.embed_concat_bwd(dx0, ctx.ids[1], off + d0, _grad_of(ctx.tables[1]))
         self.dy = None
 
-    def bucket(self, item_lo: int, item_hi: int, last: bool = False) -> None:
+    def bucket(self, item_lo: int, item_hi: int, last: bool = False, fold_bwd: bool = True) -> None:
         plan = self.plan
         if plan is None:
             return
         plan.join_wgrads()
-        plan.backward_range(item_lo, item_hi, accumulate=self.accumulate)
+        if fold_bwd:
+            plan.backward_range(item_lo, item_hi, accumulate=self.accumulate)
         if not last and self.side is not None:
             plan.async_wgrads(self.side)
 
diff --git a/ste_gan_b200/trainer.py b/ste_gan_b200/trainer.py
--- a/ste_gan_b200/trainer.py
+++ b/ste_gan_b200/trainer.py
@@ -20,27 +20,33 @@
         dev = self.params[0].device
         if dev.type != "cuda":
             raise RuntimeError("FlatParams: move the module to a CUDA device first")
-        al = lambda k: (k + 3) // 4 * 4
-        n = sum(al(p.numel()) for p in self.params)
+        self.offsets: Dict[str, int] = flat_offsets(module)
+        n = sum((p.numel() + 3) // 4 * 4 for p in self.params)
         self.flat = torch.zeros(n, device=dev, dtype=torch.float32)
         self.grad = torch.zeros(n, device=dev, dtype=torch.float32)
-        off = 0
-        self.offsets: Dict[str, int] = {}
-        names = [nm for nm, _ in module.named_parameters()]
-        for nm, p in zip(names, self.params):
+        for (nm, off), p in zip(self.offsets.items(), self.params):
             k = p.numel()
             self.flat[off:off + k].copy_(p.data.reshape(-1))
             p.data = self.flat[off:off + k].view(p.shape)
             p.grad = self.grad[off:off + k].view(p.shape)
-            self.offsets[nm] = off
-            off += al(k)
         self.m = torch.zeros_like(self.flat)
         self.v = torch.zeros_like(self.flat)
         self.step = torch.zeros(1, device=dev, dtype=torch.int64)
         self.numel = n
+        self._plan = self._plain = self._zero = None
+
+    def attach_plan(self, plan) -> None:
+        base = self.flat.data_ptr()
+        plain = plain_ranges(self.numel, [((p.data_ptr() - base) // 4, p.numel()) for m in plan.wn for p in (m.weight_v, m.weight_g)])
+        self._plan, self._plain = plan, plain
+        self._zero = [self.grad[lo:hi] for lo, hi in plain]
+        self._ranges, self._range_blocks = ops.flat_range_table(plain, self.flat.device)
 
     def zero_grad(self) -> None:
-        self.grad.zero_()
+        if self._zero is None:
+            self.grad.zero_()
+        elif self._zero:
+            torch._foreach_zero_(self._zero)
 
     def adamw(self, lr, betas=(0.8, 0.99), eps: float = 1e-8, weight_decay: float = 1e-2,
               grad_scale: float = 1.0, enable: Optional[Tensor] = None, lo: int = 0, hi: Optional[int] = None,
@@ -48,6 +54,34 @@
         hi = self.numel if hi is None else hi
         ops.adamw(self.flat[lo:hi], self.grad[lo:hi], self.m[lo:hi], self.v[lo:hi], self.step, lr, betas[0], betas[1], eps,
                   weight_decay, grad_scale, enable, keep_step)
+
+    def update_rows(self, lr: Tensor, betas=(0.8, 0.99), eps: float = 1e-8, weight_decay: float = 1e-2,
+                    grad_scale: float = 1.0, enable: Optional[Tensor] = None) -> None:
+        plan = self._plan
+        ops.weightnorm_update_multi(plan.table, plan.n_items, plan.total_rows, plan.total_tiles, self._ranges, len(self._plain),
+                                    self._range_blocks, plan.dtype, self.flat, self.grad, self.m, self.v, self.step, lr,
+                                    betas[0], betas[1], eps, weight_decay, grad_scale, enable)
+
+
+def flat_offsets(module: torch.nn.Module) -> Dict[str, int]:
+    out, off = {}, 0
+    for nm, p in module.named_parameters():
+        out[nm] = off
+        off += (p.numel() + 3) // 4 * 4
+    return out
+
+
+def plain_ranges(numel: int, spans) -> List:
+    plain, at = [], 0
+    for lo, n in sorted(spans):
+        if lo < at:
+            raise ValueError("plain_ranges: overlapping spans")
+        if lo > at:
+            plain.append((at, lo))
+        at = lo + n
+    if at < numel:
+        plain.append((at, numel))
+    return plain
 
 
 def generator_grad_buckets(offsets: Dict[str, int], numel: int, nblk: int) -> list:
@@ -88,7 +122,10 @@
         self.G, self.D = FlatParams(net_g), FlatParams(net_d)
         self.g_plan = passes.FoldPlan(passes.generator_convs(net_g), self.dtype)
         self.d_plan = passes.FoldPlan(passes.discriminator_convs(net_d), self.dtype)
+        self.G.attach_plan(self.g_plan)
+        self.D.attach_plan(self.d_plan)
         self._d_folded = False
+        self._g_folded = False
         self.reducer = GradReducer(group, enabled=data_parallel)
         self._inline = self.reducer.comm is not None
         dev = self.G.flat.device
@@ -126,6 +163,8 @@
         if (grad_buckets if grad_buckets is not None else (3 if self.reducer.enabled else 1)) == 1:
             nblk = len(list(net_g.gblocks)) - 1
             self.g_buckets = [(0, nblk, 0, 5 * nblk + 2, (0, self.G.numel))]
+        self._row_update = not self.reducer.enabled and self.dtype == torch.bfloat16 and len(self.g_buckets) == 1
+        self._rows = False
 
     @property
     def lr(self) -> float:
@@ -243,7 +282,9 @@
         if x_pred is not None:
             self.x_pred = x_pred
             return
-        self.x_pred, self._gctx = passes.generator_forward(self.net_g, su, sess, mode, self.dtype, True, folds=self.g_plan.fold(),
+        folds = self.g_plan.folds if self._rows and self._g_folded else self.g_plan.fold()
+        self._g_folded = True
+        self.x_pred, self._gctx = passes.generator_forward(self.net_g, su, sess, mode, self.dtype, True, folds=folds,
                                                            side=self._s2(1) if self.use_adv else None)
 
     def _d_fake(self) -> None:
@@ -273,7 +314,8 @@
             self.d_plan.zero()
             passes.discriminator_backward(self.net_d, ctx_f, dl[:nd], None, want_input_grad=False, want_weight_grad=True, plan=self.d_plan)
             passes.discriminator_backward(self.net_d, ctx_r, dl[nd:], None, want_input_grad=False, want_weight_grad=True, plan=self.d_plan)
-            self.d_plan.backward(accumulate=False)
+            if not self._rows:
+                self.d_plan.backward(accumulate=False)
             self._reduce_d()
             return
         subs, heavy, p_idx, s_idx = self._split_subs()
@@ -320,7 +362,8 @@
             self.d_plan.backward_range(i_lo, i_hi, accumulate=False)
             self._wait_events(early + [self._reduce(self.D.grad[g_lo:g_hi])])
             return
-        self.d_plan.backward(accumulate=False)
+        if not self._rows:
+            self.d_plan.backward(accumulate=False)
         self._reduce_d()
 
     def _reduce_d(self) -> None:
@@ -392,9 +435,11 @@
                 td_ev = torch.cuda.Event()
                 td_ev.record(self._aux)
         if self.use_adv:
-            if update_d:
+            if update_d and self._rows:
+                self.D.update_rows(self.lr_dev, grad_scale=self.reducer.grad_scale)
+            elif update_d:
                 self.D.adamw(self.lr_dev, grad_scale=self.reducer.grad_scale)
-            refold_d = update_d or not self._d_folded
+            refold_d = (update_d and not self._rows) or not self._d_folded
             self._d_folded = True
             if self.concurrent_d:
                 subs = passes.disc_subnets(self.net_d)
@@ -458,7 +503,7 @@
         gb.blocks(lo, hi)
         if i == len(self.g_buckets) - 1:
             gb.finish()
-        gb.bucket(c_lo, c_hi, last=i == len(self.g_buckets) - 1)
+        gb.bucket(c_lo, c_hi, last=i == len(self.g_buckets) - 1, fold_bwd=not self._rows)
         if i == len(self.g_buckets) - 1:
             self._gb = self._gctx = None
 
@@ -486,9 +531,17 @@
             self.reducer.wait(handles)
 
     def _phase_opt_g(self) -> None:
-        self.G.adamw(self.lr_dev, grad_scale=self.reducer.grad_scale)
+        if self._rows:
+            self.G.update_rows(self.lr_dev, grad_scale=self.reducer.grad_scale)
+        else:
+            self.G.adamw(self.lr_dev, grad_scale=self.reducer.grad_scale)
+        self._g_folded = self._rows
 
     def _opt_g_head(self) -> None:
+        self._g_folded = self._rows
+        if self._rows:
+            self.G.update_rows(self.lr_dev, grad_scale=self.reducer.grad_scale, enable=self._pend)
+            return
         n = len(self.g_buckets)
         lo, hi = self.g_buckets[n - 1][4]
         if self._inline:
@@ -526,11 +579,15 @@
         su = speech_units.contiguous().float()
         xr = x_real.contiguous().float()
         self._cur_ph = phoneme_targets
-        self._phase_d(su, session_ids, speaking_mode_ids, xr)
-        if not self._inline:
-            self.reducer.all_reduce(self.D.grad)
-        self._wait_handles(self._phase_g(xr, reduce=True))
-        self._phase_opt_g()
+        self._rows = self._row_update
+        try:
+            self._phase_d(su, session_ids, speaking_mode_ids, xr)
+            if not self._inline:
+                self.reducer.all_reduce(self.D.grad)
+            self._wait_handles(self._phase_g(xr, reduce=True))
+            self._phase_opt_g()
+        finally:
+            self._rows = False
         return self.slots
 
     def disc_losses_step(self, x_pred: Tensor, x_real: Tensor) -> Tensor:
@@ -579,6 +636,7 @@
                     self._sm_reserve = reserve
                 else:
                     _l.load().stg_set_sm_limit(n_sm - reserve)
+            self._rows = self._row_update
             try:
                 with torch.cuda.graph(step_g, pool=pool, **gkw):
                     self._fused_step(s)
@@ -586,8 +644,11 @@
                 self._sm_reserve = 0
                 if reserve > 0:
                     _l.load().stg_set_sm_limit(0)
-            with torch.cuda.graph(flush_g, pool=pool, **gkw):
-                self._opt_g_head()
+            try:
+                with torch.cuda.graph(flush_g, pool=pool, **gkw):
+                    self._opt_g_head()
+            finally:
+                self._rows = False
             self._pend.zero_()
             self._fused, self._graphs, self._d_graphs, self._pending_host = (step_g, flush_g), None, None, False
             return
@@ -660,6 +721,8 @@
     def refold(self) -> None:
         self.d_plan.fold()
         self._d_folded = True
+        self.g_plan.fold()
+        self._g_folded = True
 
     def flush(self) -> None:
         if self._pending_host and self._fused is not None:
@@ -689,6 +752,7 @@
             self._pending_host = True
             return self.slots
         g1, g2, g3 = self._graphs
+        self._g_folded = False
         def phase_g() -> list:
             handles = []
             for i, gr in enumerate(g2):
```

After: 4104 (median of 6 runs). 1.7% higher.
